# IVRL/NoiseDiff

Measured on AMD Instinct MI355X. Metric: sampled RAW patches/sec (256x256x4, 1000-step DDPM), higher is better.
Workload: dtype f32; 1 GPU; NoiseDiffNet dim=64, 256x256x4 patches, 1000-step DDPM (sigmoid2, pred_v), 16 patches per GPU; a step = one reverse-diffusion step (U-Net forward + fused posterior/noise update) over the per-GPU batch; patches/s = n_gpus*16/(1000*s_per_step); global_batch=16, launch=hipGraph replay, noise=device Philox4x32-10

## Files before the change

include/noisediff_hip.h:

```cpp
#ifndef NOISEDIFF_HIP_H
#define NOISEDIFF_HIP_H

#include <stdint.h>

#ifdef __cplusplus
extern "C" {
#endif

#define ND_E_BADARG   (-1)
#define ND_E_SHAPE    (-2)
#define ND_E_ALIGN    (-3)
#define ND_E_STATE    (-4)

int         nd_version(void);
const char* nd_last_error(void);
int         nd_device_arch(char* buf, int n);


enum nd_prologue {
    ND_PRO_NONE        = 0,
    ND_PRO_AFFINE_SILU = 1,
    ND_PRO_AFFINE_MAP_SILU = 2,
    ND_PRO_LAYERNORM   = 3,
    ND_PRO_SILU        = 4,
    ND_PRO_LEAKY       = 5,
    ND_PRO_LEAKY_SECOND = 6,
    ND_PRO_AFFINE_GENMAP_SILU = 7
};

typedef struct nd_src {
    const float* p0;
    const float* p1;
    int32_t c0, c1;
    int32_t ld0, ld1;
    int32_t mode;
    int32_t upsample;
    int32_t unshuffle;
    int32_t map_blocked;
    const float* mad;
    const float* map;
    const float* vec;
    const float* gamma;
    const float* beta;
    const float* rowstats;
} nd_src;

enum nd_act { ND_ACT_NONE = 0, ND_ACT_GELU = 1, ND_ACT_SILU = 2 };


typedef struct nd_conv3x3 {
    nd_src   src;
    const float* weight;
    const float* bias;
    float*   out;
    float*   stats;
    float*   slot_count;
    int32_t  B, H, W;
    int32_t  cin, cout, ldo;
} nd_conv3x3;

int nd_conv3x3_nhwc_f32(const nd_conv3x3* d, void* stream);
int nd_conv3x3_stat_slots(int H, int W, int cout, int B);
int nd_conv3x3_tiling_id(int B, int H, int W, int cout);
int64_t nd_pack_conv3x3_weight_floats(int cin, int cout);
int nd_pack_conv3x3_weight(const float* oihw, float* packed, int cin, int cout, void* stream);
int nd_pack_conv3x3_weight_dgrad(const float* oihw_fwd, float* packed, int cin, int cout, void* stream);

int nd_conv3x3_wino_nhwc_f32(const nd_conv3x3* d, void* stream);
int nd_conv3x3_wino2_nhwc_f32(const nd_conv3x3* d, void* stream);
int nd_conv3x3_wino_stat_slots(int H, int W);
int64_t nd_pack_conv3x3_wino_weight_floats(int cin, int cout);
int nd_pack_conv3x3_wino_weight(const float* oihw, float* packed, int cin, int cout, void* stream);
int nd_pack_conv3x3_wino_weight_dgrad(const float* oihw_fwd, float* packed, int cin, int cout, void* stream);

int nd_conv3x3_wino4_nhwc_f32(const nd_conv3x3* d, void* stream);
int nd_conv3x3_wino4_16_nhwc_f32(const nd_conv3x3* d, void* stream);
int nd_conv3x3_wino4_stat_slots(int H, int W);
int64_t nd_pack_conv3x3_wino4_weight_floats(int cin, int cout);
int nd_pack_conv3x3_wino4_weight(const float* oihw, float* packed, int cin, int cout, void* stream);
int nd_pack_conv3x3_wino4_weight_dgrad(const float* oihw_fwd, float* packed, int cin, int cout, void* stream);
typedef struct nd_pack_item {
    const float* w;
    float*       packed;
    int32_t      cin, cout, transposed, reserved;
} nd_pack_item;
int nd_pack_conv3x3_wino4_weights_batch(const nd_pack_item* items_dev, int n_items, void* stream);
int nd_conv3x3_wino4_splitk_plan(int B, int H, int W, int cin, int cout);
int64_t nd_conv3x3_wino4_splitk_workspace_floats(int B, int H, int W, int cout, int splits);
int nd_conv3x3_wino4_splitk_nhwc_f32(const nd_conv3x3* d, float* workspace, int splits, void* stream);
int nd_conv3x3_wino4_16_splitk_plan(int H, int W, int cin, int cout);
int nd_conv3x3_wino4_16_splitk_nhwc_f32(const nd_conv3x3* d, float* workspace, int splits, void* stream);


int64_t nd_conv3x3_wgrad_workspace_floats(int B, int H, int W, int cin, int cout);
int nd_conv3x3_wgrad_cat_nhwc_f32(const float* x0, int ldx0, int c0, const float* x1, int ldx1, int c1, const float* dy, int ldy, float* dw_oihw,
                                  float* dbias, float* workspace, int B, int H, int W, int cout, void* stream);
int nd_conv3x3_wgrad_form(int form);
int nd_conv3x3_wgrad_nhwc_f32(const float* x, int ldx, const float* dy, int ldy, float* dw_oihw, float* dbias, float* workspace,
                              int B, int H, int W, int cin, int cout, void* stream);
int nd_conv3x3_wgrad_leaky_nhwc_f32(const float* x, int ldx, const float* dy, int ldy, float* dw_oihw, float* dbias, float* workspace,
                                    int B, int H, int W, int cin, int cout, void* stream);
int64_t nd_conv3x3_wgrad_cat_workspace_floats(int B, int H, int W, int c0, int c1, int cout);
int nd_conv3x3_wgrad_cat_leaky_second_nhwc_f32(const float* x0, int ldx0, int c0, const float* x1, int ldx1, int c1, const float* dy, int ldy,
                                               float* dw_oihw, float* dbias, float* workspace, int B, int H, int W, int cout, void* stream);
int nd_leaky_grad_join_f32(const float* z, float* dz, const float* d_direct, int ld_direct, const float* d_pool, int B, int H, int W, int C,
                           void* stream);

int64_t nd_groupnorm_train_workspace_floats(int B, int HW, int C);
int nd_groupnorm_train_forward_f32(const float* x, int ldx, const float* gamma, const float* beta, float* y, int ldy, float* mean_rstd,
                                   float* workspace, int B, int HW, int C, int groups, float eps, void* stream);
int nd_groupnorm_train_backward_f32(const float* dy, int lddy, const float* x, int ldx, const float* gamma, const float* mean_rstd,
                                    float* dx, int lddx, float* dgamma, float* dbeta, float* workspace, int B, int HW, int C, int groups,
                                    void* stream);

int64_t nd_groupnorm_silu_train_workspace_floats(int B, int HW, int C);
int nd_groupnorm_silu_train_forward_f32(const float* x, int ldx, const float* gamma, const float* beta, const float* scale_shift, const float* res, int ldr,
                                        float* y, int ldy, float* mean_rstd, float* mad, float* workspace, int B, int HW, int C, int groups, float eps,
                                        void* stream);
int nd_groupnorm_silu_train_backward_f32(const float* dy, int lddy, const float* x, int ldx, const float* gamma, const float* beta,
                                         const float* scale_shift, const float* mean_rstd, const float* mad, float* dx, int lddx,
                                         float* dgamma, float* dbeta, float* dscale_shift, float* workspace, int B, int HW, int C, int groups,
                                         void* stream);

int nd_modulate_silu_forward_f32(const float* n, int ldn, const float* map, int ldm, float* y, int ldy, int64_t N, int C, void* stream);
int nd_modulate_silu_backward_f32(const float* dy, int lddy, const float* n, int ldn, const float* map, int ldm, float* dn, int lddn, float* dmap, int lddm,
                                  int64_t N, int C, void* stream);

int64_t nd_token_sum_workspace_floats(int B, int HW, int C);
int nd_token_sum_f32(const float* x, int ldx, float* out, float* workspace, int B, int HW, int C, void* stream);

int64_t nd_layernorm_train_workspace_floats(int64_t N, int C);
int nd_layernorm_train_forward_f32(const float* x, int ldx, const float* gamma, const float* beta, float* y, int ldy, float* stats,
                                   int64_t N, int C, float eps, void* stream);
int nd_layernorm_train_backward_f32(const float* dy, int lddy, const float* x, int ldx, const float* gamma, const float* stats,
                                    float* dx, int lddx, float* dgamma, float* dbeta, float* workspace, int64_t N, int C, void* stream);

int64_t nd_linear_wgrad_workspace_floats(int64_t N, int cin, int cout);
int nd_linear_wgrad_f32(const float* x, int ldx, const float* dy, int ldy, float* dw, float* dbias, float* workspace,
                        int64_t N, int cin, int cout, void* stream);
int nd_linear_wgrad_leaky_f32(const float* x, int ldx, const float* dy, int ldy, float* dw, float* dbias, float* workspace,
                              int64_t N, int cin, int cout, void* stream);
int64_t nd_convt2x2_wgrad_workspace_floats(int B, int h, int w, int cin, int cout);
int nd_convt2x2_wgrad_leaky_f32(const float* x, int ldx, const float* d_up, int ld_up, float* dw, float* workspace, int B, int h, int w,
                                int cin, int cout, int up_h, int up_w, void* stream);


typedef struct nd_pointwise {
    nd_src   src;
    const float* weight;
    const float* bias;
    float*   out;
    const float* res0; const float* res1;
    const float* vec;
    const float* gn_t;
    const float* gn_mad;
    int32_t  B, HW, W;
    int32_t  cin, cout, ldo, ldr0, ldr1, ldt;
    int32_t  act;
    int32_t  shuffle_c;
    int32_t  shuffle_h, shuffle_w;
} nd_pointwise;

int nd_pointwise_gemm_nhwc_f32(const nd_pointwise* d, void* stream);
int nd_pointwise_gemm_unshuffle_crop_nhwc_f32(const nd_pointwise* d, int src_h, int src_w, void* stream);

int64_t nd_image_quality_workspace_bytes(int B, int C, int H, int W);
int nd_image_quality_f32(const float* est, const float* target, const float* scale, double data_range, double* psnr, double* ssim,
                         double* mse, void* workspace, int B, int C, int H, int W, void* stream);
int64_t nd_illum_scale_workspace_bytes(int B, int C, int H, int W);
int nd_illum_scale_f32(const float* pred, const float* source, int source_batch, float* k32, double* k64, void* workspace,
                       int B, int C, int H, int W, void* stream);
int nd_illum_apply_f32(const float* pred, const float* k32, float* out, int B, int C, int H, int W, void* stream);
int64_t nd_pack_pointwise_weight_floats(int cin, int cout);
int nd_pack_pointwise_weight(const float* w, float* packed, int cin, int cout, int unshuffle_c, void* stream);
int nd_pack_pointwise_weight_t(const float* w_t, float* packed, int cin, int cout, void* stream);
int nd_pack_pointwise_weights_batch(const nd_pack_item* items_dev, int n_items, void* stream);

int nd_pointwise_gemm_split_nhwc_f32(const nd_pointwise* d, void* stream);
int nd_pointwise_gemm_split_takes(const nd_pointwise* d);
int64_t nd_pack_pointwise_weight_split_floats(int cin, int cout);
int nd_pack_pointwise_weight_split(const float* w, float* packed, int cin, int cout, void* stream);

enum nd_chain_res { ND_CHAIN_RES_NONE = 0, ND_CHAIN_RES_INPUT = 1 , ND_CHAIN_RES_INPUT_RAW = 2  };
typedef struct nd_chain_stage {
    const float* weight;
    const float* bias;
    int32_t  cin, cout;
    int32_t  act;
    int32_t  res;
} nd_chain_stage;
typedef struct nd_chain {
    nd_src   src;
    nd_chain_stage st[3];
    float*   out;
    int32_t  n_stages, B, HW, ldo;
} nd_chain;
int nd_pointwise_chain_nhwc_f32(const nd_chain* d, void* stream);
int nd_pointwise_chain_supported(int cin, int n1, int n2, int n3);
int64_t nd_pack_chain_weight_floats(int cin, int cout, int first_stage);
int nd_pack_chain_weight(const float* w, float* packed, int cin, int cout, int first_stage, void* stream);
int nd_pointwise_chain_split_nhwc_f32(const nd_chain* d, void* stream);
int64_t nd_pack_chain_weight_split_floats(int cin, int cout, int first_stage);
int nd_pack_chain_weight_split(const float* w, float* packed, int cin, int cout, int first_stage, void* stream);


int nd_groupnorm_finalize_f32(const float* stats, const float* slot_count, int slots,
                              const float* gamma, const float* beta,
                              const float* scale_shift, int ld_ss,
                              float* mad, int B, int C, int groups, float eps, void* stream);
int nd_groupnorm_finalize_train_f32(const float* stats, const float* slot_count, int slots, const float* gamma, const float* beta,
                                    const float* scale_shift, int ld_ss, float* mad, float* mean_rstd, int B, int C, int groups, float eps,
                                    void* stream);

int nd_layernorm_stats_f32(const float* x, int ldx, const float* vec, float* stats,
                           int B, int HW, int C, float eps, void* stream);

int nd_affine_silu_add_f32(const float* t, int ldt, const float* mad,
                           const float* res0, int ldr0, const float* res1, int ldr1,
                           float* out, int ldo, int B, int HW, int C, void* stream);


int nd_linear_rows_f32(const float* in, int ld_in, const float* W, const float* bias,
                       float* out, int ld_out, int B, int K, int N,
                       int act_in, int act_out, void* stream);
int nd_sinusoidal_time_emb_f32(const int64_t* time, const float* freqs, float* emb, int B, int half, void* stream);
int64_t nd_cond_step_lds_bytes(int B, int dim);
int nd_cond_step_f32(const int64_t* time, const float* freqs, const float* W1, const float* b1, const float* W2, const float* b2,
                     const float* Wp, const float* bp, float* out, int ld_out, int B, int dim, int J, void* stream);
int nd_cond_table_build_f32(const float* freqs, const float* W1, const float* b1, const float* W2, const float* b2, float* table, int rows, int dim,
                            void* stream);
int nd_cond_step_table_f32(const int64_t* time, const float* freqs, const float* W1, const float* b1, const float* W2, const float* b2,
                           const float* Wp, const float* bp, float* out, int ld_out, int B, int dim, int J, const float* table, int table_rows,
                           void* stream);
int nd_cond_step_ptable_f32(const int64_t* time, const float* freqs, const float* W1, const float* b1, const float* W2, const float* b2,
                            const float* Wp, const float* bp, float* out, int ld_out, int B, int dim, int J, const float* table, int table_rows,
                            const float* ptable, void* stream);
int nd_embedding_rows_f32(const int64_t* idx, const float* table, float* out, int B, int rows, int dim, void* stream);


int nd_conv7x7_c4_f32(const float* x, const float* wpacked, const float* bias, float* out, int ldo,
                      int B, int H, int W, int cout, void* stream);
int64_t nd_conv7x7_c4_wgrad_workspace_floats(int B, int H, int W, int cout);
int nd_conv7x7_c4_wgrad_f32(const float* x, const float* dy, int ldy, float* dw_oihw, float* dbias, float* workspace, int B, int H, int W, int cout,
                            void* stream);
int nd_pack_conv7x7_weight(const float* oihw, float* packed, int cout, void* stream);
int nd_conv7x7_c4_split_f32(const float* x, const float* wsplit, const float* bias, float* out, int ldo,
                            int B, int H, int W, int cout, void* stream);
int64_t nd_pack_conv7x7_weight_split_floats(int cout);
int nd_pack_conv7x7_weight_split(const float* oihw, float* packed, int cout, void* stream);
int nd_pos_enc_f32(const float* position_nchw, const float* w , const float* bias,
                   float* out, int B, int H, int W, int hid, void* stream);
int nd_maxpool2x2_nhwc_f32(const float* in, float* out, int B, int H, int W, int C, void* stream);
int nd_nchw_to_nhwc_f32(const float* in, float* out, int B, int C, int H, int W, void* stream);
int nd_nhwc_to_nchw_f32(const float* in, float* out, int B, int C, int H, int W, void* stream);
int nd_nchw_to_nhwc_pad_f32(const float* in, float* out, int B, int C, int H, int W, int Cpad, void* stream);


typedef struct nd_sampler_state {
    int32_t* step;
    const int32_t* t_cur;
    const int32_t* t_next;
    const float* coef;
    int64_t* time_out;
    const int64_t* rng;
    int32_t n_steps, B;
} nd_sampler_state;

int nd_sampler_begin_step(const nd_sampler_state* s, void* stream);
int nd_sampler_advance(const nd_sampler_state* s, void* stream);

int nd_sampler_step_ddpm_f32(float* x, const float* model_out, const float* noise, int64_t noise_step_stride,
                             const nd_sampler_state* s, int objective,
                             uint64_t seed, int64_t first_sample,
                             int B, int HW, int C, void* stream);
int nd_sampler_step_ddim_f32(float* x, const float* model_out, const float* noise, int64_t noise_step_stride,
                             const nd_sampler_state* s, int objective,
                             uint64_t seed, int64_t first_sample,
                             int B, int HW, int C, void* stream);
int nd_philox_normal_f32(float* out, uint64_t seed, int64_t first_sample, int32_t step,
                         int B, int HW, int C, void* stream);


int nd_attention_mfma_f32(const float* qkv, int ld_qkv, float* out, int ld_out,
                          int B, int N, int heads, int dh, void* stream);
int64_t nd_linear_attention_workspace_floats(int B, int N, int heads);
int nd_linear_attention_f32(const float* qkv, int ld_qkv, float* out, int ld_out, float* workspace,
                            int B, int N, int heads, int dh, void* stream);
int nd_rmsnorm_nhwc_f32(const float* x, int ldx, const float* g, float* out, int ldo,
                        int B, int HW, int C, void* stream);
int nd_rmsnorm_add_nhwc_f32(const float* x, int ldx, const float* g, const float* res, int ldr, float* out, int ldo, int B, int HW, int C, void* stream);

typedef struct nd_adam_item {
    float*       p;
    const float* g;
    float*       m;
    float*       v;
    int64_t      n;
    float        step_size, bias2_sqrt;
    int32_t      vec4, reserved;
    float*       step;
} nd_adam_item;
int nd_adam_chunk_elements(void);
int nd_adam_step_f32(const nd_adam_item* items_dev, int n_items, const int32_t* chunks_dev, int n_chunks, float beta1, float beta2, float eps,
                     float weight_decay, void* stream);
int nd_adam_step_capturable_f32(const nd_adam_item* items_dev, int n_items, const int32_t* chunks_dev, int n_chunks, float lr, float beta1, float beta2,
                                float eps, float weight_decay, void* stream);

int nd_stream_create(void** stream);
int nd_stream_destroy(void* stream);
int nd_stream_sync(void* stream);
int nd_graph_begin(void* stream);
int nd_graph_end(void* stream, void** graph_exec);
int nd_graph_launch(void* graph_exec, void* stream);
int nd_graph_destroy(void* graph_exec);
int nd_stream_device(void* stream);
int nd_event_create(void** ev);
int nd_event_record(void* ev, void* stream);
int nd_event_elapsed_ms(void* start, void* stop, float* ms);
int nd_event_destroy(void* ev);
int nd_event_create_untimed(void** ev);
int nd_stream_wait_event(void* stream, void* ev);

#ifdef __cplusplus
}
#endif
#endif
```

noisediff_amd/_lib.py:

```python
from __future__ import annotations

import ctypes as C
import os
from typing import Optional

HERE = os.path.dirname(os.path.abspath(__file__))
LIB_PATH = os.path.join(HERE, "libnoisediff_hip.so")

PRO_NONE, PRO_AFFINE_SILU, PRO_AFFINE_MAP_SILU, PRO_LAYERNORM, PRO_SILU, PRO_LEAKY, PRO_LEAKY_SECOND, PRO_AFFINE_GENMAP_SILU = 0, 1, 2, 3, 4, 5, 6, 7
ACT_NONE, ACT_GELU, ACT_SILU = 0, 1, 2
OBJECTIVES = {"pred_noise": 0, "pred_x0": 1, "pred_v": 2}

fptr = C.c_void_p


class HipError(RuntimeError):
    pass


class Src(C.Structure):
    _fields_ = [("p0", fptr), ("p1", fptr), ("c0", C.c_int32), ("c1", C.c_int32), ("ld0", C.c_int32), ("ld1", C.c_int32),
                ("mode", C.c_int32), ("upsample", C.c_int32), ("unshuffle", C.c_int32), ("map_blocked", C.c_int32),
                ("mad", fptr), ("map", fptr), ("vec", fptr), ("gamma", fptr), ("beta", fptr), ("rowstats", fptr)]


class AdamItem(C.Structure):
    _fields_ = [("p", fptr), ("g", fptr), ("m", fptr), ("v", fptr), ("n", C.c_int64), ("step_size", C.c_float), ("bias2_sqrt", C.c_float),
                ("vec4", C.c_int32), ("reserved", C.c_int32), ("step", fptr)]


class PackItem(C.Structure):
    _fields_ = [("w", fptr), ("packed", fptr), ("cin", C.c_int32), ("cout", C.c_int32), ("transposed", C.c_int32), ("reserved", C.c_int32)]


class Conv3x3(C.Structure):
    _fields_ = [("src", Src), ("weight", fptr), ("bias", fptr), ("out", fptr), ("stats", fptr), ("slot_count", fptr),
                ("B", C.c_int32), ("H", C.c_int32), ("W", C.c_int32), ("cin", C.c_int32), ("cout", C.c_int32), ("ldo", C.c_int32)]


class Pointwise(C.Structure):
    _fields_ = [("src", Src), ("weight", fptr), ("bias", fptr), ("out", fptr), ("res0", fptr), ("res1", fptr), ("vec", fptr),
                ("gn_t", fptr), ("gn_mad", fptr), ("B", C.c_int32), ("HW", C.c_int32), ("W", C.c_int32), ("cin", C.c_int32),
                ("cout", C.c_int32), ("ldo", C.c_int32), ("ldr0", C.c_int32), ("ldr1", C.c_int32), ("ldt", C.c_int32), ("act", C.c_int32),
                ("shuffle_c", C.c_int32), ("shuffle_h", C.c_int32), ("shuffle_w", C.c_int32)]


class ChainStage(C.Structure):
    _fields_ = [("weight", fptr), ("bias", fptr), ("cin", C.c_int32), ("cout", C.c_int32), ("act", C.c_int32), ("res", C.c_int32)]


class Chain(C.Structure):
    _fields_ = [("src", Src), ("st", ChainStage * 3), ("out", fptr), ("n_stages", C.c_int32), ("B", C.c_int32), ("HW", C.c_int32),
                ("ldo", C.c_int32)]


CHAIN_RES_NONE, CHAIN_RES_INPUT, CHAIN_RES_INPUT_RAW = 0, 1, 2


class SamplerState(C.Structure):
    _fields_ = [("step", fptr), ("t_cur", fptr), ("t_next", fptr), ("coef", fptr), ("time_out", fptr), ("rng", fptr),
                ("n_steps", C.c_int32), ("B", C.c_int32)]


i32, i64, u64, vp, f32, f64 = C.c_int, C.c_int64, C.c_uint64, C.c_void_p, C.c_float, C.c_double

SIGNATURES = {
    "nd_version": (i32, []),
    "nd_last_error": (C.c_char_p, []),
    "nd_device_arch": (i32, [C.c_char_p, i32]),
    "nd_conv3x3_nhwc_f32": (i32, [C.POINTER(Conv3x3), vp]),
    "nd_conv3x3_stat_slots": (i32, [i32, i32, i32, i32]),
    "nd_conv3x3_tiling_id": (i32, [i32, i32, i32, i32]),
    "nd_pack_conv3x3_weight_floats": (i64, [i32, i32]),
    "nd_pack_conv3x3_weight": (i32, [vp, vp, i32, i32, vp]),
    "nd_pack_conv3x3_weight_dgrad": (i32, [vp, vp, i32, i32, vp]),
    "nd_conv3x3_wino_nhwc_f32": (i32, [C.POINTER(Conv3x3), vp]),
    "nd_conv3x3_wino2_nhwc_f32": (i32, [C.POINTER(Conv3x3), vp]),
    "nd_conv3x3_wino_stat_slots": (i32, [i32, i32]),
    "nd_conv3x3_wino4_stat_slots": (i32, [i32, i32]),
    "nd_pack_conv3x3_wino_weight_floats": (i64, [i32, i32]),
    "nd_pack_conv3x3_wino_weight": (i32, [vp, vp, i32, i32, vp]),
    "nd_pack_conv3x3_wino_weight_dgrad": (i32, [vp, vp, i32, i32, vp]),
    "nd_conv3x3_wino4_nhwc_f32": (i32, [C.POINTER(Conv3x3), vp]),
    "nd_conv3x3_wino4_16_nhwc_f32": (i32, [C.POINTER(Conv3x3), vp]),
    "nd_pack_conv3x3_wino4_weight_floats": (i64, [i32, i32]),
    "nd_pack_conv3x3_wino4_weight": (i32, [vp, vp, i32, i32, vp]),
    "nd_pack_conv3x3_wino4_weight_dgrad": (i32, [vp, vp, i32, i32, vp]),
    "nd_conv3x3_wino4_splitk_plan": (i32, [i32, i32, i32, i32, i32]),
    "nd_conv3x3_wino4_splitk_workspace_floats": (i64, [i32, i32, i32, i32, i32]),
    "nd_conv3x3_wino4_splitk_nhwc_f32": (i32, [vp, vp, i32, vp]),
    "nd_conv3x3_wino4_16_splitk_plan": (i32, [i32, i32, i32, i32]),
    "nd_conv3x3_wino4_16_splitk_nhwc_f32": (i32, [vp, vp, i32, vp]),
    "nd_conv3x3_wgrad_workspace_floats": (i64, [i32, i32, i32, i32, i32]),
    "nd_conv3x3_wgrad_nhwc_f32": (i32, [vp, i32, vp, i32, vp, vp, vp, i32, i32, i32, i32, i32, vp]),
    "nd_groupnorm_train_workspace_floats": (i64, [i32, i32, i32]),
    "nd_linear_wgrad_workspace_floats": (i64, [i64, i32, i32]),
    "nd_groupnorm_silu_train_workspace_floats": (i64, [i32, i32, i32]),
    "nd_groupnorm_silu_train_forward_f32": (i32, [vp, i32, vp, vp, vp, vp, i32, vp, i32, vp, vp, vp, i32, i32, i32, i32, C.c_float, vp]),
    "nd_token_sum_workspace_floats": (i64, [i32, i32, i32]),
    "nd_token_sum_f32": (i32, [vp, i32, vp, vp, i32, i32, i32, vp]),
    "nd_modulate_silu_forward_f32": (i32, [vp, i32, vp, i32, vp, i32, i64, i32, vp]),
    "nd_modulate_silu_backward_f32": (i32, [vp, i32, vp, i32, vp, i32, vp, i32, vp, i32, i64, i32, vp]),
    "nd_groupnorm_silu_train_backward_f32": (i32, [vp, i32, vp, i32, vp, vp, vp, vp, vp, vp, i32, vp, vp, vp, vp, i32, i32, i32, i32, vp]),
    "nd_layernorm_train_workspace_floats": (i64, [i64, i32]),
    "nd_layernorm_train_forward_f32": (i32, [vp, i32, vp, vp, vp, i32, vp, i64, i32, C.c_float, vp]),
    "nd_layernorm_train_backward_f32": (i32, [vp, i32, vp, i32, vp, vp, vp, i32, vp, vp, vp, i64, i32, vp]),
    "nd_linear_wgrad_f32": (i32, [vp, i32, vp, i32, vp, vp, vp, i64, i32, i32, vp]),
    "nd_groupnorm_train_forward_f32": (i32, [vp, i32, vp, vp, vp, i32, vp, vp, i32, i32, i32, i32, C.c_float, vp]),
    "nd_groupnorm_train_backward_f32": (i32, [vp, i32, vp, i32, vp, vp, vp, i32, vp, vp, vp, i32, i32, i32, i32, vp]),
    "nd_pointwise_gemm_nhwc_f32": (i32, [C.POINTER(Pointwise), vp]),
    "nd_pointwise_chain_nhwc_f32": (i32, [C.POINTER(Chain), vp]),
    "nd_pointwise_chain_supported": (i32, [i32, i32, i32, i32]),
    "nd_pack_chain_weight_floats": (i64, [i32, i32, i32]),
    "nd_pack_chain_weight": (i32, [vp, vp, i32, i32, i32, vp]),
    "nd_pointwise_chain_split_nhwc_f32": (i32, [C.POINTER(Chain), vp]),
    "nd_pack_chain_weight_split_floats": (i64, [i32, i32, i32]),
    "nd_pack_chain_weight_split": (i32, [vp, vp, i32, i32, i32, vp]),
    "nd_pointwise_gemm_split_nhwc_f32": (i32, [C.POINTER(Pointwise), vp]),
    "nd_pointwise_gemm_split_takes": (i32, [C.POINTER(Pointwise)]),
    "nd_pack_pointwise_weight_split_floats": (i64, [i32, i32]),
    "nd_pack_pointwise_weight_split": (i32, [vp, vp, i32, i32, vp]),
    "nd_pack_pointwise_weight_floats": (i64, [i32, i32]),
    "nd_pack_pointwise_weight": (i32, [vp, vp, i32, i32, i32, vp]),
    "nd_pack_pointwise_weight_t": (i32, [vp, vp, i32, i32, vp]),
    "nd_pack_pointwise_weights_batch": (i32, [vp, i32, vp]),
    "nd_pack_conv3x3_wino4_weights_batch": (i32, [vp, i32, vp]),
    "nd_conv3x3_wgrad_cat_nhwc_f32": (i32, [vp, i32, i32, vp, i32, i32, vp, i32, vp, vp, vp, i32, i32, i32, i32, vp]),
    "nd_conv3x3_wgrad_form": (i32, [i32]),
    "nd_conv7x7_c4_wgrad_workspace_floats": (i64, [i32, i32, i32, i32]),
    "nd_conv7x7_c4_wgrad_f32": (i32, [vp, vp, i32, vp, vp, vp, i32, i32, i32, i32, vp]),
    "nd_adam_chunk_elements": (i32, []),
    "nd_adam_step_f32": (i32, [vp, i32, vp, i32, f32, f32, f32, f32, vp]),
    "nd_adam_step_capturable_f32": (i32, [vp, i32, vp, i32, f32, f32, f32, f32, f32, vp]),
    "nd_groupnorm_finalize_f32": (i32, [vp, vp, i32, vp, vp, vp, i32, vp, i32, i32, i32, f32, vp]),
    "nd_groupnorm_finalize_train_f32": (i32, [vp, vp, i32, vp, vp, vp, i32, vp, vp, i32, i32, i32, f32, vp]),
    "nd_layernorm_stats_f32": (i32, [vp, i32, vp, vp, i32, i32, i32, f32, vp]),
    "nd_affine_silu_add_f32": (i32, [vp, i32, vp, vp, i32, vp, i32, vp, i32, i32, i32, i32, vp]),
    "nd_linear_rows_f32": (i32, [vp, i32, vp, vp, vp, i32, i32, i32, i32, i32, i32, vp]),
    "nd_sinusoidal_time_emb_f32": (i32, [vp, vp, vp, i32, i32, vp]),
    "nd_cond_step_lds_bytes": (i64, [i32, i32]),
    "nd_cond_step_f32": (i32, [vp, vp, vp, vp, vp, vp, vp, vp, vp, i32, i32, i32, i32, vp]),
    "nd_cond_table_build_f32": (i32, [vp, vp, vp, vp, vp, vp, i32, i32, vp]),
    "nd_cond_step_table_f32": (i32, [vp, vp, vp, vp, vp, vp, vp, vp, vp, i32, i32, i32, i32, vp, i32, vp]),
    "nd_cond_step_ptable_f32": (i32, [vp, vp, vp, vp, vp, vp, vp, vp, vp, i32, i32, i32, i32, vp, i32, vp, vp]),
    "nd_embedding_rows_f32": (i32, [vp, vp, vp, i32, i32, i32, vp]),
    "nd_conv7x7_c4_f32": (i32, [vp, vp, vp, vp, i32, i32, i32, i32, i32, vp]),
    "nd_pack_conv7x7_weight": (i32, [vp, vp, i32, vp]),
    "nd_conv7x7_c4_split_f32": (i32, [vp, vp, vp, vp, i32, i32, i32, i32, i32, vp]),
    "nd_pack_conv7x7_weight_split_floats": (i64, [i32]),
    "nd_pack_conv7x7_weight_split": (i32, [vp, vp, i32, vp]),
    "nd_pos_enc_f32": (i32, [vp, vp, vp, vp, i32, i32, i32, i32, vp]),
    "nd_maxpool2x2_nhwc_f32": (i32, [vp, vp, i32, i32, i32, i32, vp]),
    "nd_nchw_to_nhwc_pad_f32": (i32, [vp, vp, i32, i32, i32, i32, i32, vp]),
    "nd_nchw_to_nhwc_f32": (i32, [vp, vp, i32, i32, i32, i32, vp]),
    "nd_nhwc_to_nchw_f32": (i32, [vp, vp, i32, i32, i32, i32, vp]),
    "nd_sampler_begin_step": (i32, [C.POINTER(SamplerState), vp]),
    "nd_sampler_advance": (i32, [C.POINTER(SamplerState), vp]),
    "nd_sampler_step_ddpm_f32": (i32, [vp, vp, vp, i64, C.POINTER(SamplerState), i32, u64, i64, i32, i32, i32, vp]),
    "nd_sampler_step_ddim_f32": (i32, [vp, vp, vp, i64, C.POINTER(SamplerState), i32, u64, i64, i32, i32, i32, vp]),
    "nd_philox_normal_f32": (i32, [vp, u64, i64, i32, i32, i32, i32, vp]),
    "nd_attention_mfma_f32": (i32, [vp, i32, vp, i32, i32, i32, i32, i32, vp]),
    "nd_linear_attention_workspace_floats": (i64, [i32, i32, i32]),
    "nd_linear_attention_f32": (i32, [vp, i32, vp, i32, vp, i32, i32, i32, i32, vp]),
    "nd_rmsnorm_nhwc_f32": (i32, [vp, i32, vp, vp, i32, i32, i32, i32, vp]),
    "nd_rmsnorm_add_nhwc_f32": (i32, [vp, i32, vp, vp, i32, vp, i32, i32, i32, i32, vp]),
    "nd_stream_create": (i32, [C.POINTER(vp)]),
    "nd_stream_destroy": (i32, [vp]),
    "nd_stream_sync": (i32, [vp]),
    "nd_graph_begin": (i32, [vp]),
    "nd_graph_end": (i32, [vp, C.POINTER(vp)]),
    "nd_graph_launch": (i32, [vp, vp]),
    "nd_graph_destroy": (i32, [vp]),
    "nd_event_create": (i32, [C.POINTER(vp)]),
    "nd_event_record": (i32, [vp, vp]),
    "nd_event_elapsed_ms": (i32, [vp, vp, C.POINTER(f32)]),
    "nd_event_destroy": (i32, [vp]),
    "nd_event_create_untimed": (i32, [C.POINTER(vp)]),
    "nd_stream_wait_event": (i32, [vp, vp]),
    "nd_stream_device": (i32, [vp]),
    "nd_conv3x3_wgrad_leaky_nhwc_f32": (i32, [vp, i32, vp, i32, vp, vp, vp, i32, i32, i32, i32, i32, vp]),
    "nd_conv3x3_wgrad_cat_workspace_floats": (i64, [i32, i32, i32, i32, i32, i32]),
    "nd_conv3x3_wgrad_cat_leaky_second_nhwc_f32": (i32, [vp, i32, i32, vp, i32, i32, vp, i32, vp, vp, vp, i32, i32, i32, i32, vp]),
    "nd_leaky_grad_join_f32": (i32, [vp, vp, vp, i32, vp, i32, i32, i32, i32, vp]),
    "nd_linear_wgrad_leaky_f32": (i32, [vp, i32, vp, i32, vp, vp, vp, i64, i32, i32, vp]),
    "nd_convt2x2_wgrad_workspace_floats": (i64, [i32, i32, i32, i32, i32]),
    "nd_convt2x2_wgrad_leaky_f32": (i32, [vp, i32, vp, i32, vp, vp, i32, i32, i32, i32, i32, i32, i32, vp]),
    "nd_pointwise_gemm_unshuffle_crop_nhwc_f32": (i32, [C.POINTER(Pointwise), i32, i32, vp]),
    "nd_image_quality_workspace_bytes": (i64, [i32, i32, i32, i32]),
    "nd_image_quality_f32": (i32, [vp, vp, vp, f64, vp, vp, vp, vp, i32, i32, i32, i32, vp]),
    "nd_illum_scale_workspace_bytes": (i64, [i32, i32, i32, i32]),
    "nd_illum_scale_f32": (i32, [vp, vp, i32, vp, vp, vp, i32, i32, i32, i32, vp]),
    "nd_illum_apply_f32": (i32, [vp, vp, vp, i32, i32, i32, i32, vp]),
}

_UNCHECKED = {"nd_version", "nd_last_error", "nd_stream_device", "nd_conv3x3_wgrad_form", "nd_adam_chunk_elements", "nd_conv7x7_c4_wgrad_workspace_floats", "nd_conv3x3_stat_slots", "nd_conv3x3_tiling_id", "nd_pack_conv3x3_weight_floats",
              "nd_pack_pointwise_weight_floats", "nd_linear_attention_workspace_floats", "nd_conv3x3_wino_stat_slots", "nd_conv3x3_wino4_stat_slots",
              "nd_pack_conv3x3_wino_weight_floats", "nd_pack_conv3x3_wino4_weight_floats", "nd_conv3x3_wino4_splitk_plan", "nd_conv3x3_wino4_16_splitk_plan", "nd_conv3x3_wino4_splitk_workspace_floats", "nd_token_sum_workspace_floats", "nd_cond_step_lds_bytes", "nd_conv3x3_wgrad_workspace_floats",
              "nd_groupnorm_train_workspace_floats", "nd_linear_wgrad_workspace_floats",
              "nd_layernorm_train_workspace_floats", "nd_groupnorm_silu_train_workspace_floats", "nd_conv3x3_wgrad_cat_workspace_floats",
              "nd_convt2x2_wgrad_workspace_floats", "nd_image_quality_workspace_bytes", "nd_illum_scale_workspace_bytes"}

_lib: Optional[C.CDLL] = None


def load(path: str = LIB_PATH) -> C.CDLL:
    global _lib
    if _lib is not None:
        return _lib
    import torch
    if not os.path.exists(path):
        raise HipError(f"{path} is missing: the HIP library is the product and there is no fallback. "
                       "Build it with `python -m noisediff_amd.build`.")
    lib = C.CDLL(path)
    for name, (res, args) in SIGNATURES.items():
        fn = getattr(lib, name)
        fn.restype, fn.argtypes = res, args
    _lib = lib
    return lib


def check(code: int, what: str = "") -> None:
    if code != 0:
        msg = load().nd_last_error().decode(errors="replace")
        raise HipError(f"{what or 'libnoisediff_hip'} failed with code {code}: {msg}")


def call(name: str, *args):
    r = getattr(load(), name)(*args)
    if name not in _UNCHECKED:
        check(r, name)
    return r


def ptr(t) -> Optional[int]:
    return None if t is None else t.data_ptr()
```

noisediff_amd/csrc/conv3x3_wino4.hip:

```cpp
#include <stdlib.h>
#include <type_traits>
#include "nd_common.h"

namespace {

typedef float f32x2 __attribute__((ext_vector_type(2)));
typedef unsigned u32x4_t __attribute__((ext_vector_type(4)));
typedef __attribute__((address_space(3))) void* lds_ptr;
typedef __attribute__((address_space(3))) short* lds_short_ptr;
typedef __attribute__((address_space(3))) unsigned* lds_u32_ptr;
typedef __attribute__((address_space(3))) unsigned short* lds_u16_ptr;
typedef __attribute__((address_space(3))) f32x4* lds_f32x4_ptr;

constexpr int KC4 = 16;
constexpr int NPOS = 36;
constexpr int VD_FLOATS = NPOS * 256;

constexpr int MAX_COUT = 2048;
template <int NTG, int NW = 4>
struct W4Geo {
    static constexpr int NT = 64 * NW;
    static constexpr int TGW = NTG * 4 / NW;
    static constexpr int REG_W = 16 * NTG, HALO_W = REG_W + 2;
    static constexpr int RAW_ROWP = NTG == 2 ? 40 : 24;
    static constexpr int RAW_ITEMS = 18 * HALO_W * 4, RAW_IT = (RAW_ITEMS + NT - 1) / NT;
    static constexpr int RAW_FLOATS = 18 * RAW_ROWP * 16;
    static constexpr bool RTAB = TGW == 2;
    static constexpr bool BIAS_LDS = TGW == 2;
    static constexpr int TAB_BYTES = (RAW_IT + (RTAB ? RAW_IT : 0)) * NT * 4 + (RAW_IT + 12) * NT * 2;
    static constexpr int BIAS_OFF_BYTES = RAW_FLOATS * 4 + NTG * VD_FLOATS * 4 + TAB_BYTES;
    static constexpr int LDS_BYTES = BIAS_OFF_BYTES + (BIAS_LDS ? MAX_COUT * 4 : 0);
    static constexpr int WG_PER_CU = NTG == 2 ? 1 : 2;
    static constexpr int ACC_AGPR = TGW == 2 ? 64 : 32;
    static_assert(NW == 4 || (NW == 8 && NTG == 2), "four waves, or eight on the 16 x 32 region");
    static_assert(LDS_BYTES * WG_PER_CU <= 160 * 1024, "LDS map");
};

#ifndef W4_UR
#define W4_UR 18
#endif
#ifndef W4_UR_AFF
#define W4_UR_AFF 18
#endif
#ifndef W4_UR_MAP
#define W4_UR_MAP 6
#endif
#ifndef W4_UR_GEN
#define W4_UR_GEN 6
#endif
#ifndef W4_UR_EPI
#define W4_UR_EPI 6
#endif
#ifndef W4_VR
#define W4_VR 3
#endif
#ifndef W4_COMMIT_AT
#define W4_COMMIT_AT 8
#endif
#ifndef W4_XF_AT
#define W4_XF_AT 10
#endif
#ifndef W4_U_AUX
#define W4_U_AUX 0
#endif
#ifndef W4_STORE_AUX
#define W4_STORE_AUX 19
#endif
#ifndef W4_STAGGER
#define W4_STAGGER 12
#endif
#ifndef W4_XF_SPLIT
#define W4_XF_SPLIT 1
#endif
#ifndef W4_UR1
#define W4_UR1 9
#endif
#ifndef W4_UR1_AFF
#define W4_UR1_AFF 6
#endif
#ifndef W4_UR1_EPI
#define W4_UR1_EPI 0
#endif
#ifndef W4_UR1_XF
#define W4_UR1_XF 6
#endif
#ifndef W4_PAIR_SKEW
#define W4_PAIR_SKEW 2
#endif
#ifndef W4_PRIO
#define W4_PRIO 0
#endif
#ifndef W4_ABLATE
#define W4_ABLATE 0
#endif

struct Wino4Args {
    nd_conv3x3 d;
    int tiles_x, tiles_y, regions_x, n_tiles, n_cg, n_c8, slots, total_wg;
    int splits, chunks_per_split;
};

#ifndef W4_NOP
#define W4_NOP ""
#endif
#define W4_MFMA_A(acc, uv, vv)  asm volatile(W4_NOP "v_mfma_f32_16x16x4_f32 %0, %2, %1, %0" : "+a"(acc) : "v"(uv), "v"(vv))
#define W4_MFMA_V(acc, uv, vv)  asm volatile(W4_NOP "v_mfma_f32_16x16x4_f32 %0, %2, %1, %0" : "+v"(acc) : "v"(uv), "v"(vv))
#define W4_MFMA_AZ(acc, uv, vv) asm volatile(W4_NOP "v_mfma_f32_16x16x4_f32 %0, %2, %1, 0" : "=&a"(acc) : "v"(uv), "v"(vv))
#define W4_MFMA_VZ(acc, uv, vv) asm volatile(W4_NOP "v_mfma_f32_16x16x4_f32 %0, %2, %1, 0" : "=&v"(acc) : "v"(uv), "v"(vv))
#define W4_MFMA_DRAIN() asm volatile("s_nop 15\n\ts_nop 15" ::: "memory")

__device__ __forceinline__ void w4_bt(const f32x2 (&d)[6], f32x2 (&t)[6]) {
    const f32x2 c4 = {4.0f, 4.0f}, cm4 = {-4.0f, -4.0f}, cm5 = {-5.0f, -5.0f}, c2 = {2.0f, 2.0f}, cm2 = {-2.0f, -2.0f};
    const f32x2 p = __builtin_elementwise_fma(cm4, d[2], d[4]), q = __builtin_elementwise_fma(cm4, d[1], d[3]);
    const f32x2 r = d[4] - d[2], s = d[3] - d[1];
    t[0] = __builtin_elementwise_fma(c4, d[0], __builtin_elementwise_fma(cm5, d[2], d[4]));
    t[1] = p + q;
    t[2] = p - q;
    t[3] = __builtin_elementwise_fma(c2, s, r);
    t[4] = __builtin_elementwise_fma(cm2, s, r);
    t[5] = __builtin_elementwise_fma(c4, d[1], __builtin_elementwise_fma(cm5, d[3], d[5]));
}

template <int HALF>
__device__ __forceinline__ void w4_bt_half(const f32x2 (&d)[6], f32x2 (&t)[3]) {
    const f32x2 c4 = {4.0f, 4.0f}, cm4 = {-4.0f, -4.0f}, cm5 = {-5.0f, -5.0f}, c2 = {2.0f, 2.0f}, cm2 = {-2.0f, -2.0f};
    if (HALF == 0) {
        const f32x2 p = __builtin_elementwise_fma(cm4, d[2], d[4]), q = __builtin_elementwise_fma(cm4, d[1], d[3]);
        t[0] = __builtin_elementwise_fma(c4, d[0], __builtin_elementwise_fma(cm5, d[2], d[4]));
        t[1] = p + q;
        t[2] = p - q;
    } else {
        const f32x2 r = d[4] - d[2], s = d[3] - d[1];
        t[0] = __builtin_elementwise_fma(c2, s, r);
        t[1] = __builtin_elementwise_fma(cm2, s, r);
        t[2] = __builtin_elementwise_fma(c4, d[1], __builtin_elementwise_fma(cm5, d[3], d[5]));
    }
}

template <int MODE, bool STREAM, bool SPLIT = false, int NTG = 2, int NW = 4>
__global__ __launch_bounds__((64 * NW), (W4Geo<NTG, NW>::WG_PER_CU)) void wino4_kernel(const Wino4Args a) {
    using Geo = W4Geo<NTG, NW>;
    constexpr int NT = Geo::NT, TGW = Geo::TGW;
    constexpr int RAW_FLOATS = Geo::RAW_FLOATS, BIAS_OFF_BYTES = Geo::BIAS_OFF_BYTES, ACC_AGPR = Geo::ACC_AGPR, REG_W = Geo::REG_W, HALO_W = Geo::HALO_W;
    constexpr bool MAP = MODE == ND_PRO_AFFINE_MAP_SILU;
    constexpr bool GEN = MODE == ND_PRO_AFFINE_GENMAP_SILU;
    constexpr bool MAPX = MAP || GEN;
    constexpr bool AFF = MODE == ND_PRO_AFFINE_SILU || MAPX;
    constexpr bool LEAKY = MODE == ND_PRO_LEAKY || MODE == ND_PRO_LEAKY_SECOND;
    constexpr int UR = TGW == 1 ? (AFF ? W4_UR1_AFF : W4_UR1) : MAP ? W4_UR_MAP : GEN ? W4_UR_GEN : AFF ? W4_UR_AFF : W4_UR, UR_EPI = TGW == 1 ? W4_UR1_EPI : W4_UR_EPI;
    static_assert(TGW == 2 || !MAPX, "the map prologues (20 more staging registers per halo item in flight) stay on the 512-register form");
    extern __shared__ __attribute__((aligned(16))) float lds_[];
    float* const Vd = lds_ + RAW_FLOATS;

    const int tid = threadIdx.x, lane = tid & 63;
    const int wave = __builtin_amdgcn_readfirstlane(tid >> 6);
    const int mtg = NW == 8 ? wave >> 2 : 0;
    const int tg = TGW == 2 ? wave >> 1 : mtg, rh = (wave >> 1) & 1, ch2 = wave & 1;
    const int tile = lane & 15, kq = lane >> 4;

    const int wgid = nd_xcd_remap(blockIdx.x, gridDim.x);
    const int t_begin = (int)((long)wgid * a.total_wg / gridDim.x), t_end = (int)((long)(wgid + 1) * a.total_wg / gridDim.x);
    if (t_begin >= t_end) return;

#ifdef W4_STAMP
    const unsigned long long stamp_c0 = __builtin_amdgcn_s_memtime(), stamp_r0 = __builtin_amdgcn_s_memrealtime();
    unsigned long long stamp_epi = 0, stamp_xf = 0, stamp_wait = 0, stamp_t = 0, stamp_drain = 0, stamp_first = 0, stamp_last = 0, stamp_second = 0, stamp_third = 0, stamp_pro = 0, stamp_top = 0, stamp_tile = 0;
#define W4_T0() (stamp_t = __builtin_amdgcn_s_memtime())
#define W4_ACC(x) (x += __builtin_amdgcn_s_memtime() - stamp_t)
#else
#define W4_T0()
#define W4_ACC(x)
#endif
#if W4_STAGGER
    if (a.total_wg >= 4 * (int)gridDim.x)
        for (int k = (int)(blockIdx.x >> 3) & 15; k > 0; --k) __builtin_amdgcn_s_sleep(W4_STAGGER);
#endif
#if W4_PAIR_SKEW
    if (NTG == 1 && 2 * blockIdx.x >= gridDim.x)
        for (int k = 0; k < W4_PAIR_SKEW; ++k) __builtin_amdgcn_s_sleep(32);
#endif
    const nd_src& s = a.d.src;
    const int H = a.d.H, W = a.d.W, Cin = a.d.cin, Cout = a.d.cout;
    const int up = s.upsample ? 1 : 0;
    const int sH = H >> up, sW = W >> up;
    const int Ctot = s.c0 + s.c1;
    const int n_chunks = SPLIT ? a.chunks_per_split : (Cin + KC4 - 1) / KC4;

    auto decode = [&](int t, int& b_, int& ty_, int& rx_, int& nt_, int& sp_) {
        int lid = t;
        nt_ = lid % a.n_tiles;  lid /= a.n_tiles;
        rx_ = lid % a.regions_x;  lid /= a.regions_x;
        ty_ = lid % a.tiles_y;
        b_ = lid / a.tiles_y;
        sp_ = 0;
        if (SPLIT) { sp_ = b_ / a.d.B;  b_ -= sp_ * a.d.B; }
    };

    constexpr int RAW_ROWP = Geo::RAW_ROWP, RAW_IT = Geo::RAW_IT;
    const long npx = (long)a.d.B * sH * sW;
    const unsigned PX_MARK = (unsigned)(npx + sW + 2);
    auto src_rsrc = [&](const float* p, long px_stride_floats) {
        return __builtin_amdgcn_make_buffer_rsrc(const_cast<float*>(p) - (long)(sW + 1) * px_stride_floats, 0,
                                                 (int)((npx + sW + 1) * px_stride_floats * 4), 0x00020000);
    };
    const __amdgpu_buffer_rsrc_t rsrc0 = src_rsrc(s.p0, s.ld0);
    const __amdgpu_buffer_rsrc_t rsrc1 = s.p1 ? src_rsrc(s.p1, s.ld1) : rsrc0;
    const __amdgpu_buffer_rsrc_t rsrcm = MAP ? src_rsrc(s.map, 2 * Ctot) : GEN ? src_rsrc(s.map, 8) : rsrc0;
    const int map_shift = s.map_blocked ? 64 : Ctot * 4;
    float* const vd_tg = Vd + tg * VD_FLOATS;
    char* const rawbuf = reinterpret_cast<char*>(lds_);
    lds_u32_ptr const ptab = (lds_u32_ptr)(Vd + NTG * VD_FLOATS) + tid;
    auto cperm = [](int c) { return ((c >> 2) & 3) | ((c & 3) << 2) | (c & 48); };
    auto swz = [](int r, int c) { return (2 * ((r >> 2) & 3)) ^ (4 * ((c >> 3) & 1)); };
    auto pixl_of = [](int t) { return GEN ? 16 * (t >> 6) + (t & 15) : t >> 2; };
    const int sq = GEN ? (tid >> 4) & 3 : tid & 3;
    lds_u32_ptr const rtab = ptab + RAW_IT * NT;
    lds_u16_ptr const dtab = (lds_u16_ptr)(ptab - tid + (Geo::RTAB ? 2 : 1) * RAW_IT * NT) + tid;
    lds_u16_ptr const ttab = dtab + RAW_IT * NT;
    float* const bias_lds = reinterpret_cast<float*>(reinterpret_cast<char*>(lds_) + BIAS_OFF_BYTES);
    auto item_rc = [&](int k, int tid_) {
        const int pix = pixl_of(tid_) + (NT / 4) * k, r = pix / HALO_W, c = pix - HALO_W * r;
        const int dy = up ? (r + 1) >> 1 : r, dx = up ? (c + 1) >> 1 : c;
        return (unsigned)(dy * sW + dx) | ((unsigned)r << 16) | ((unsigned)c << 24);
    };
#pragma unroll
    for (int k = 0; k < RAW_IT; ++k) {
        const int pix = pixl_of(tid) + (NT / 4) * k, r = pix / HALO_W, c = pix - HALO_W * r;
        dtab[k * NT] = (unsigned short)((r * RAW_ROWP + cperm(c)) * 64 + (((2 * sq) ^ swz(r, c)) * 8));
        if (Geo::RTAB) rtab[k * NT] = item_rc(k, tid);
    }
    const int t_tile = ((lane >> 1) & 7) | ((lane >> 4) & 1) << 3, t_kq = (lane & 1) | ((lane >> 5) << 1);
#pragma unroll
    for (int h = 0; h < 2; ++h)
#pragma unroll
        for (int bx = 0; bx < 6; ++bx) {
            const int r0 = 4 * (t_tile >> 2) + 4 * h, c = 16 * tg + 4 * (t_tile & 3) + bx;
            ttab[(h * 6 + bx) * NT] = (unsigned short)((4 * (t_tile >> 2) * RAW_ROWP + cperm(c)) * 64 + (((4 * ch2 + t_kq) ^ swz(r0, c)) * 8));
        }
    const unsigned t_lds = (unsigned)(ch2 * 1024 + (t_kq >> 1) * 512 + t_tile * 32 + (t_kq & 1) * 16);
    if (Geo::BIAS_LDS)
        for (int i = tid; i < a.n_tiles * 64; i += NT) bias_lds[i] = (a.d.bias && i < Cout) ? a.d.bias[i] : 0.0f;
    const __amdgpu_buffer_rsrc_t brsrc = __builtin_amdgcn_make_buffer_rsrc(const_cast<float*>(a.d.bias ? a.d.bias : a.d.weight), 0, a.d.bias ? Cout * 4 : 0, 0x00020000);
    float bias_r = 0.0f;

    const unsigned OOB = 0x7FFFFFF0u;
    int sb_ = 0;
    unsigned spx_ = 0;
    bool tab_clean = false;
    f32x4 tA4 = {1, 1, 1, 1}, tD4 = {0, 0, 0, 0};
    auto stage_tile = [&](int b_, int ty_, int rx_) {
        sb_ = b_;
        spx_ = (unsigned)((b_ * sH + ((ty_ * 16) >> up)) * sW + ((rx_ * REG_W) >> up));
        const int r_lo = ty_ == 0 ? 1 : 0, r_n = min(17, H - ty_ * 16) - r_lo;
        const int c_lo = rx_ == 0 ? 1 : 0, c_n = min(HALO_W - 1, W - rx_ * REG_W) - c_lo;
        const bool interior = r_lo == 0 && r_n == 17 && c_lo == 0 && c_n == HALO_W - 1;
        if (!(interior && tab_clean)) {
            int tid_ = tid;
            if (!Geo::RTAB) asm volatile("" : "+v"(tid_));
#pragma unroll
            for (int k = 0; k < RAW_IT; ++k) {
                const unsigned rc = Geo::RTAB ? rtab[k * NT] : item_rc(k, tid_);
                const unsigned r = (rc >> 16) & 255u, c = rc >> 24;
                const bool ok = r - (unsigned)r_lo <= (unsigned)r_n && c - (unsigned)c_lo <= (unsigned)c_n;
                ptab[k * NT] = ok ? (rc & 0xFFFFu) : PX_MARK;
            }
        }
        tab_clean = interior;
    };
    f32x4 raw[RAW_IT];
    constexpr int GEN_H = RAW_IT / 2;
    f32x4 msc[MAP ? RAW_IT : GEN ? GEN_H : 1], msh[MAP ? RAW_IT : GEN ? GEN_H : 1];
    float ev0[GEN ? RAW_IT : 1], ev1[GEN ? RAW_IT : 1];
    float gw_sc0 = 0, gw_sc1 = 0, gw_sh0 = 0, gw_sh1 = 0;
    f32x4 gb_sc = {0, 0, 0, 0}, gb_sh = {0, 0, 0, 0};
    int i_eoff = 0;
    bool i_second = false;
    __amdgpu_buffer_rsrc_t i_rs = rsrc0;
    int i_soff = 0, i_mapoff = 0;
    unsigned i_ld4 = 0, i_bias = 0;
    auto stage_issue_begin = [&](int cb_) {
        const bool sec = cb_ >= s.c0;
        i_second = sec;
        i_mapoff = (int)(cb_ * (s.map_blocked ? 8u : 4u) + spx_ * (unsigned)(2 * Ctot * 4));
        i_rs = sec ? rsrc1 : rsrc0;
        i_ld4 = (unsigned)(sec ? s.ld1 : s.ld0) * 4u;
        i_soff = (int)((sec ? cb_ - s.c0 : cb_) * 4u + spx_ * i_ld4);
        i_bias = cb_ + 4 * sq < Cin ? 16u * sq : OOB;
        if (GEN) {
            i_eoff = (int)(spx_ * 32u);
            const float* wr = s.gamma + (size_t)(cb_ + (lane & 15)) * 8 + sq;
            gw_sc0 = wr[0];  gw_sc1 = wr[4];  gw_sh0 = wr[(size_t)Ctot * 8];  gw_sh1 = wr[(size_t)Ctot * 8 + 4];
            gb_sc = nd_ld4(s.beta + cb_ + 4 * sq);  gb_sh = nd_ld4(s.beta + Ctot + cb_ + 4 * sq);
        }
        if (AFF) {
            const int c = cb_ + 4 * sq;
            const float* m = s.mad + (size_t)sb_ * 3 * Ctot + (c < Cin ? c : 0);
            const f32x4 M = nd_ld4(m), A = nd_ld4(m + Ctot), D = nd_ld4(m + 2 * Ctot);
            tA4 = A;
            tD4 = D - M * A;
        }
    };
    auto stage_issue_one = [&](int k, unsigned px, auto tile_first_c) {
#if !(W4_ABLATE & 1)
        const unsigned voff = __umul24(px, i_ld4) + i_bias;
        raw[k] = __builtin_bit_cast(f32x4, __builtin_amdgcn_raw_buffer_load_b128(i_rs, voff, i_soff, 0));
        if (GEN && decltype(tile_first_c)::value) {
            const unsigned eo = __umul24(px, 32u) + 4u * sq;
            ev0[k] = __builtin_bit_cast(float, __builtin_amdgcn_raw_buffer_load_b32(rsrcm, eo, i_eoff, 0));
            ev1[k] = __builtin_bit_cast(float, __builtin_amdgcn_raw_buffer_load_b32(rsrcm, eo, i_eoff + 16, 0));
        }
        if (MAP) {
            const unsigned mo = __umul24(px, (unsigned)(2 * Ctot * 4)) + i_bias;
            msc[k] = __builtin_bit_cast(f32x4, __builtin_amdgcn_raw_buffer_load_b128(rsrcm, mo, i_mapoff, 0));
            msh[k] = __builtin_bit_cast(f32x4, __builtin_amdgcn_raw_buffer_load_b128(rsrcm, mo, i_mapoff + map_shift, 0));
        }
#else
        raw[k] = f32x4{(float)k, 1.0f, 0.5f, 0.25f};
#endif
    };
    auto gen_maps = [&](int k0) {
#pragma unroll
        for (int k = 0; k < GEN_H; ++k) asm volatile("v_mfma_f32_16x16x4_f32 %0, %1, %2, %3" : "=&v"(msc[GEN ? k : 0]) : "v"(gw_sc0), "v"(ev0[GEN ? k0 + k : 0]), "v"(gb_sc));
#pragma unroll
        for (int k = 0; k < GEN_H; ++k) asm volatile("v_mfma_f32_16x16x4_f32 %0, %1, %2, %3" : "=&v"(msh[GEN ? k : 0]) : "v"(gw_sh0), "v"(ev0[GEN ? k0 + k : 0]), "v"(gb_sh));
#pragma unroll
        for (int k = 0; k < GEN_H; ++k) asm volatile("v_mfma_f32_16x16x4_f32 %0, %1, %2, %0" : "+v"(msc[GEN ? k : 0]) : "v"(gw_sc1), "v"(ev1[GEN ? k0 + k : 0]));
#pragma unroll
        for (int k = 0; k < GEN_H; ++k) asm volatile("v_mfma_f32_16x16x4_f32 %0, %1, %2, %0" : "+v"(msh[GEN ? k : 0]) : "v"(gw_sh1), "v"(ev1[GEN ? k0 + k : 0]));
        W4_MFMA_DRAIN();
    };
    auto stage_commit_one = [&](int k, unsigned daddr, unsigned pxk) {
        if (k == RAW_IT - 1 && pixl_of(tid) + (NT / 4) * k >= 18 * HALO_W) return;
        f32x4 v = raw[k];
        if (AFF) {
            f32x4 x = v * tA4 + tD4;
            if (MAPX) x = x * (msc[MAP ? k : GEN ? k % GEN_H : 0] + 1.0f) + msh[MAP ? k : GEN ? k % GEN_H : 0];
            const f32x4 t = x * -1.44269504088896340736f;
            f32x4 e;
            e.x = __builtin_amdgcn_exp2f(t.x); e.y = __builtin_amdgcn_exp2f(t.y); e.z = __builtin_amdgcn_exp2f(t.z); e.w = __builtin_amdgcn_exp2f(t.w);
            e = e + 1.0f;
            f32x4 r;
            r.x = __builtin_amdgcn_rcpf(e.x); r.y = __builtin_amdgcn_rcpf(e.y); r.z = __builtin_amdgcn_rcpf(e.z); r.w = __builtin_amdgcn_rcpf(e.w);
            const bool inside = pxk != PX_MARK && i_bias != OOB;
            const f32x4 zero = {0, 0, 0, 0};
            v = inside ? x * r : zero;
        }
        if (MODE == ND_PRO_LEAKY || (MODE == ND_PRO_LEAKY_SECOND && i_second)) v = nd_leaky4(v);
        *reinterpret_cast<lds_f32x4_ptr>(daddr) = v;
    };

    const unsigned d_lds = (unsigned)((kq >> 1) * 512 + tile * 32 + (kq & 1) * 16);

    auto xf_addr = [&](unsigned (&t_addr)[12]) {
#pragma unroll
        for (int i = 0; i < 12; ++i) t_addr[i] = ttab[i * NT];
    };
    auto xf_read = [&](f32x2 (&T)[6][6], const unsigned (&t_addr)[12], int ay) {
#if !(W4_ABLATE & 4)
#pragma unroll
        for (int bx = 0; bx < 6; ++bx)
            T[ay][bx] = *reinterpret_cast<const f32x2*>(rawbuf + t_addr[(ay >> 2) * 6 + bx] + ay * (RAW_ROWP * 64));
#endif
    };
    auto xf_finish = [&](f32x2 (&T)[6][6], float* buf, auto&& before_write) {
#if !(W4_ABLATE & 4)
        char* base = reinterpret_cast<char*>(buf) + t_lds;
#pragma unroll
        for (int bx = 0; bx < 6; ++bx) {
            f32x2 col[6], t[6];
#pragma unroll
            for (int ay = 0; ay < 6; ++ay) col[ay] = T[ay][bx];
            w4_bt(col, t);
#pragma unroll
            for (int xi = 0; xi < 6; ++xi) T[xi][bx] = t[xi];
        }
#if W4_XF_SPLIT
        before_write();
#endif
#pragma unroll
        for (int xi = 0; xi < 6; ++xi) {
            f32x2 v[6];
            w4_bt(T[xi], v);
#if W4_XF_SPLIT
#pragma unroll
            for (int h = 0; h < 3; ++h)
                *reinterpret_cast<f32x4*>(base + (xi * 3 + h) * 2048) = f32x4{v[2 * h].x, v[2 * h].y, v[2 * h + 1].x, v[2 * h + 1].y};
            __builtin_amdgcn_sched_barrier(0);
#else
#pragma unroll
            for (int bx = 0; bx < 6; ++bx) T[xi][bx] = v[bx];
#endif
        }
#if !W4_XF_SPLIT
        before_write();
#pragma unroll
        for (int xi = 0; xi < 6; ++xi)
#pragma unroll
            for (int h = 0; h < 3; ++h)
                *reinterpret_cast<f32x4*>(base + (xi * 3 + h) * 2048) = f32x4{T[xi][2 * h].x, T[xi][2 * h].y, T[xi][2 * h + 1].x, T[xi][2 * h + 1].y};
#endif
#else
        before_write();
#endif
    };

    auto xf_half = [&](float* buf) {
#if !(W4_ABLATE & 4)
        unsigned t_addr[12];
        xf_addr(t_addr);
        f32x2 T[3][6];
        auto pass1 = [&](auto half_c) {
#pragma unroll
            for (int bx = 0; bx < 6; ++bx) {
                f32x2 col[6], t[3];
#pragma unroll
                for (int ay = 0; ay < 6; ++ay) col[ay] = *reinterpret_cast<const f32x2*>(rawbuf + t_addr[(ay >> 2) * 6 + bx] + ay * (RAW_ROWP * 64));
                w4_bt_half<decltype(half_c)::value>(col, t);
#pragma unroll
                for (int i = 0; i < 3; ++i) T[i][bx] = t[i];
            }
        };
        if (rh == 0) pass1(std::integral_constant<int, 0>{}); else pass1(std::integral_constant<int, 1>{});
        char* base = reinterpret_cast<char*>(buf) + t_lds + rh * (9 * 2048);
#pragma unroll
        for (int i = 0; i < 3; ++i) {
            f32x2 v[6];
            w4_bt(T[i], v);
#pragma unroll
            for (int h = 0; h < 3; ++h)
                *reinterpret_cast<f32x4*>(base + (i * 3 + h) * 2048) = f32x4{v[2 * h].x, v[2 * h].y, v[2 * h + 1].x, v[2 * h + 1].y};
        }
#endif
    };

    const __amdgpu_buffer_rsrc_t wrsrc = __builtin_amdgcn_make_buffer_rsrc(
        const_cast<float*>(a.d.weight), 0, (int)((long)a.n_c8 * a.n_cg * 18 * 256 * 4), 0x00020000);
    const unsigned wvoff = (unsigned)(lane * 16);
    auto wblock = [&](int c8_, int cg_) { return __builtin_amdgcn_readfirstlane(((c8_ * a.n_cg + cg_) * 18) * 1024); };

    f32x4 acc[TGW * NPOS];
    f32x4 U[UR];
    f32x4 Vr[W4_VR][TGW];
    static_assert(36 % UR == 0, "the ring must close over a chunk's two stages of 18 fragments");
    auto load_u = [&](int slot, int q, int wb) {
#if !(W4_ABLATE & 2)
        U[slot % UR] = __builtin_bit_cast(f32x4, __builtin_amdgcn_raw_buffer_load_b128(wrsrc, wvoff, wb + q * 1024, W4_U_AUX));
#endif
    };
    auto read_v = [&](const char* v0base, const char* v1base, int pp) {
        Vr[pp % W4_VR][0] = *reinterpret_cast<const f32x4*>(v0base + pp * 2048);
        if (TGW == 2) Vr[pp % W4_VR][TGW - 1] = *reinterpret_cast<const f32x4*>(v1base + pp * 2048);
    };
    auto mfma = [&](auto first_c, int idx, float av, float bv) {
        constexpr bool FIRST = decltype(first_c)::value;
        if (idx < ACC_AGPR) { if (FIRST) W4_MFMA_AZ(acc[idx], av, bv); else W4_MFMA_A(acc[idx], av, bv); }
        else                { if (FIRST) W4_MFMA_VZ(acc[idx], av, bv); else W4_MFMA_V(acc[idx], av, bv); }
    };
    auto stage = [&](auto first_c, auto off_c, auto din_c, auto dout_c, const char* v0base, const char* v1base, int wb, int nb, auto&& pre, auto&& mid) {
        constexpr int OFF = decltype(off_c)::value, DIN = decltype(din_c)::value, DOUT = decltype(dout_c)::value;
        auto hi = [](int pp) { const int h = pp + UR; return h < 18 + DOUT ? h : 18 + DOUT; };
#pragma unroll
        for (int pp = 0; pp < W4_VR - 1; ++pp) read_v(v0base, v1base, pp);
#pragma unroll
        for (int q = DIN; q < hi(0); ++q) {
            if (q < 18) load_u(OFF + q, q, wb);
            else load_u(OFF + q, q - 18, nb);
        }
        __builtin_amdgcn_sched_barrier(0);
#pragma unroll
        for (int pp = 0; pp < 18; ++pp) {
            if (pp + W4_VR - 1 < 18) read_v(v0base, v1base, pp + W4_VR - 1);
            pre(pp);
            const f32x4 u = U[(OFF + pp) % UR];
            const f32x4 va = Vr[pp % W4_VR][0], vb = Vr[pp % W4_VR][TGW - 1];
            __builtin_amdgcn_sched_barrier(0);
            if (TGW == 2) {
                mfma(first_c, 4 * pp + 0, u.x, va.x);
                mfma(first_c, 4 * pp + 1, u.x, vb.x);
                mfma(first_c, 4 * pp + 2, u.z, va.z);
                mfma(first_c, 4 * pp + 3, u.z, vb.z);
                mfma(std::false_type{}, 4 * pp + 0, u.y, va.y);
                mfma(std::false_type{}, 4 * pp + 1, u.y, vb.y);
                mfma(std::false_type{}, 4 * pp + 2, u.w, va.w);
                mfma(std::false_type{}, 4 * pp + 3, u.w, vb.w);
            } else {
                mfma(first_c, 2 * pp + 0, u.x, va.x);
                mfma(first_c, 2 * pp + 1, u.z, va.z);
                mfma(std::false_type{}, 2 * pp + 0, u.y, va.y);
                mfma(std::false_type{}, 2 * pp + 1, u.w, va.w);
            }
            __builtin_amdgcn_sched_barrier(0);
#pragma unroll
            for (int q = (hi(pp) > DIN ? hi(pp) : DIN); q < hi(pp + 1); ++q) {
                if (q < 18) load_u(OFF + q, q, wb);
                else load_u(OFF + q, q - 18, nb);
            }
            mid(pp);
            __builtin_amdgcn_sched_barrier(0);
        }
    };

    auto read_acc2 = [&](int idx, int h) -> f32x2 {
        if (idx >= ACC_AGPR) {
            asm volatile("" : "+v"(acc[idx]));
            return h ? f32x2{acc[idx].z, acc[idx].w} : f32x2{acc[idx].x, acc[idx].y};
        }
        f32x2 r;
        if (h == 0) {
            asm volatile("v_accvgpr_read_b32 %0, %1" : "=v"(r.x) : "a"(acc[idx].x));
            asm volatile("v_accvgpr_read_b32 %0, %1" : "=v"(r.y) : "a"(acc[idx].y));
        } else {
            asm volatile("v_accvgpr_read_b32 %0, %1" : "=v"(r.x) : "a"(acc[idx].z));
            asm volatile("v_accvgpr_read_b32 %0, %1" : "=v"(r.y) : "a"(acc[idx].w));
        }
        return r;
    };

    int b, ty, rx, nt, sp;
    decode(t_begin, b, ty, rx, nt, sp);
    int b1 = b, ty1 = ty, rx1 = rx, nt1 = nt, sp1 = sp;
    stage_tile(b, ty, rx);
    stage_issue_begin(SPLIT ? sp * n_chunks * KC4 : 0);
#pragma unroll
    for (int k = 0; k < RAW_IT; ++k) stage_issue_one(k, ptab[k * NT], std::true_type{});
    {
        const int wb = wblock(SPLIT ? 2 * sp * n_chunks : 0, nt * 4 + (wave & 3));
#pragma unroll
        for (int q = 0; q < UR_EPI; ++q) load_u(q, q, wb);
    }
#pragma unroll
    for (int k = 0; k < RAW_IT; ++k) {
        if (GEN && k % GEN_H == 0) gen_maps(k);
        stage_commit_one(k, dtab[k * NT], AFF ? ptab[k * NT] : 0u);
    }
    asm volatile("s_waitcnt lgkmcnt(0)" ::: "memory");
    __builtin_amdgcn_s_barrier();
    if constexpr (TGW == 2) {
        f32x2 T[6][6];
        unsigned t_addr[12];
        xf_addr(t_addr);
#pragma unroll
        for (int ay = 0; ay < 6; ++ay) xf_read(T, t_addr, ay);
        xf_finish(T, vd_tg, [] {});
    } else xf_half(vd_tg);
    asm volatile("s_waitcnt lgkmcnt(0)" ::: "memory");
    __builtin_amdgcn_s_barrier();

#ifdef W4_STAMP
    stamp_pro = __builtin_amdgcn_s_memtime() - stamp_c0;
#endif
    for (int t = t_begin; t < t_end; ++t) {
        const bool more = t + 1 < t_end;
        W4_T0();
        if (more) {
            nt1 = nt + 1;  rx1 = rx;  ty1 = ty;  b1 = b;  sp1 = sp;
            if (nt1 == a.n_tiles) { nt1 = 0;  if (++rx1 == a.regions_x) { rx1 = 0;  if (++ty1 == a.tiles_y) { ty1 = 0;  ++b1;  if (SPLIT && b1 == a.d.B) { b1 = 0;  ++sp1; } } } }
        }
        const int ch0 = SPLIT ? sp * n_chunks : 0, ch0n = SPLIT ? sp1 * n_chunks : 0;
        const int cg = nt * 4 + (wave & 3), cg_next = (more ? nt1 : nt) * 4 + (wave & 3);

        auto chunk = [&](int ch, auto first_c, auto last_c) {
            const char* v0cur = reinterpret_cast<const char*>(Vd + mtg * VD_FLOATS) + d_lds;
            const char* v1cur = reinterpret_cast<const char*>(Vd + (NTG - 1) * VD_FLOATS) + d_lds;
            constexpr bool last = decltype(last_c)::value;
            const int c8 = 2 * (ch0 + ch);
            const int w0 = wblock(c8, cg), w1 = wblock(c8 + 1, cg), wn = last ? wblock(2 * ch0n, cg_next) : wblock(c8 + 2, cg);
#ifdef W4_STAMP
            if (decltype(first_c)::value) W4_ACC(stamp_top);
            W4_T0();
#endif
            if (last && more) stage_tile(b1, ty1, rx1);
#ifdef W4_STAMP
            if (last) W4_ACC(stamp_tile);
#endif
            using I0 = std::integral_constant<int, 0>;
            using IOFF1 = std::integral_constant<int, 18 % UR>;
            using IUR = std::integral_constant<int, UR>;
            using IEPI = std::integral_constant<int, UR_EPI>;
            using IXF = std::integral_constant<int, TGW == 1 ? (W4_UR1_XF < UR ? W4_UR1_XF : UR) : UR>;
            constexpr bool FIRST = decltype(first_c)::value;
            unsigned tab1 = 0;
            constexpr bool PRE_P = AFF && !MAPX;
            unsigned tabd[(AFF || LEAKY) ? RAW_IT : 1], tabp[PRE_P ? RAW_IT : 1];
            auto issue_pre = [&](int pp) { if (pp < RAW_IT) tab1 = ptab[pp * NT]; };
            auto issue = [&](int pp) {
                if (pp == 0) stage_issue_begin(last ? ch0n * KC4 : (ch0 + ch + 1) * KC4);
                if (pp < RAW_IT) stage_issue_one(pp, tab1, last_c);
            };
            auto commit_pre = [&](int pp) {
                if (AFF || LEAKY) {
                    if (pp == W4_COMMIT_AT) {
#pragma unroll
                        for (int k = 0; k < RAW_IT; ++k) {
                            tabd[k] = dtab[k * NT];
                            if (PRE_P) tabp[k] = ptab[k * NT];
                        }
                    }
                } else if (pp < RAW_IT) tab1 = dtab[pp * NT];
            };
            f32x2 T[TGW == 2 ? 6 : 1][6];
            unsigned t_addr[12];
            auto commit = [&](int pp) {
                if (AFF || LEAKY) {
                    if (pp == W4_COMMIT_AT) {
#pragma unroll
                        for (int k = 0; k < RAW_IT; ++k) {
                            if (GEN && k % GEN_H == 0) gen_maps(k);
                            stage_commit_one(k, tabd[(AFF || LEAKY) ? k : 0], PRE_P ? tabp[PRE_P ? k : 0] : MAPX ? ptab[k * NT] : 0u);
                        }
                    }
                } else if (pp < RAW_IT) stage_commit_one(pp, tab1, 0u);
                if constexpr (TGW == 2) {
                    if (pp == W4_XF_AT) {
                        asm volatile("s_waitcnt lgkmcnt(0)" ::: "memory");
                        __builtin_amdgcn_s_barrier();
                        xf_addr(t_addr);
                    }
                    if (pp > W4_XF_AT && pp <= W4_XF_AT + 6) xf_read(T, t_addr, pp - W4_XF_AT - 1);
                }
            };
            W4_T0();
            if (TGW == 1 && FIRST)
                bias_r = __builtin_bit_cast(float, __builtin_amdgcn_raw_buffer_load_b32(brsrc, (unsigned)(cg * 16 + (lane & 15)) * 4u, 0, 0));
            stage(first_c, I0{}, std::conditional_t<FIRST, IEPI, IXF>{}, IUR{}, v0cur, v1cur, w0, w1, issue_pre, issue);
            if (TGW == 1 && FIRST) asm volatile("" : "+v"(bias_r));
            stage(std::false_type{}, IOFF1{}, IUR{}, std::conditional_t<last, IEPI, IXF>{}, v0cur + 1024, v1cur + 1024, w1, wn, commit_pre, commit);
#ifdef W4_STAMP
            if (FIRST) W4_ACC(stamp_first);
            if (last) W4_ACC(stamp_last);
            if (!FIRST && !last && ch == 1) W4_ACC(stamp_second);
            if (!FIRST && !last && ch == 2) W4_ACC(stamp_third);
#endif
            W4_T0();
            if constexpr (TGW == 2) {
                xf_finish(T, vd_tg, [&] {
                    W4_ACC(stamp_xf);
                    W4_T0();
                    __builtin_amdgcn_s_barrier();
                    W4_ACC(stamp_wait);
                    W4_T0();
                });
            } else {
                asm volatile("s_waitcnt lgkmcnt(0)" ::: "memory");
                __builtin_amdgcn_s_barrier();
                W4_ACC(stamp_wait);
                W4_T0();
                if (W4_PRIO) __builtin_amdgcn_s_setprio(W4_PRIO);
                xf_half(vd_tg);
                if (W4_PRIO) __builtin_amdgcn_s_setprio(0);
            }
            asm volatile("s_waitcnt lgkmcnt(0)" ::: "memory");
            __builtin_amdgcn_s_barrier();
            W4_ACC(stamp_xf);
        };
        chunk(0, std::true_type{}, std::false_type{});
        for (int ch = 1; ch + 1 < n_chunks; ++ch) chunk(ch, std::false_type{}, std::false_type{});
        chunk(n_chunks - 1, std::false_type{}, std::true_type{});

        W4_T0();
        W4_MFMA_DRAIN();
        if (TGW == 1 && W4_PRIO) __builtin_amdgcn_s_setprio(W4_PRIO);

        const __amdgpu_buffer_rsrc_t orsrc = __builtin_amdgcn_make_buffer_rsrc(a.d.out, 0, (int)((unsigned)(SPLIT ? a.splits : 1) * a.d.B * H * W * a.d.ldo * 4u), 0x00020000);
        int Wt = __builtin_amdgcn_readfirstlane(W), ldot = __builtin_amdgcn_readfirstlane(a.d.ldo);
        asm volatile("" : "+s"(Wt), "+s"(ldot));
#pragma unroll
        for (int j = 0; j < TGW; ++j) {
            const int tx = NTG * rx + (TGW == 2 ? j : mtg);
            if (tx < a.tiles_x) {
                int l15 = lane;
                asm volatile("" : "+v"(l15));
                l15 &= 15;
                const int co = cg * 16 + l15;
                const bool cok = co < Cout;
                float z0 = 0.0f;
                asm volatile("" : "+v"(z0));
                const float* const bias_p = bias_lds + co;
                const int py0 = ty * 16 + 4 * kq, px0 = tx * 16;
                f32x2 sum2 = {z0, z0}, sq2 = {z0, z0}, cnt2 = {z0, z0};
                float pivot = z0;
                const bool full = ty * 16 + 16 <= H && tx * 16 + 16 <= W && cg * 16 + 16 <= Cout;
                const bool want_stats = a.d.stats != nullptr;
                const unsigned lane_off = (unsigned)((((unsigned)(SPLIT ? sp * a.d.B + b : b) * H + py0) * Wt + px0) * ldot + co) * 4u;
                auto emit = [&](auto full_c, auto stats_c) {
                    constexpr bool FULL = decltype(full_c)::value, STATS = decltype(stats_c)::value;
                    int step4 = ldot * 16, back3 = ldot * -12, rowadv = (Wt - 7) * ldot * 4;
                    asm volatile("" : "+s"(step4), "+s"(back3), "+s"(rowadv));
                    const f32x2 c2 = {2.0f, 2.0f}, c4 = {4.0f, 4.0f}, c8 = {8.0f, 8.0f};
                    const int rowlim = FULL ? 4 : H - py0, collim = FULL ? 16 : W - px0;
#pragma unroll
                    for (int h = 0; h < 2; ++h) {
                        int soff = h * 32 * ldot;
                        asm volatile("" : "+s"(soff));
                        f32x2 Z[4][6];
#pragma unroll
                        for (int nu = 0; nu < 6; ++nu) {
                            auto M = [&](int xi) { return read_acc2(TGW * (xi * 6 + nu) + j, h); };
                            f32x2 m1 = M(1);
                            const f32x2 m2 = M(2);
                            if (nu == 1) m1 += Geo::BIAS_LDS ? *bias_p : bias_r;
                            const f32x2 p = m1 + m2, q = m1 - m2;
                            const f32x2 m3 = M(3), m4 = M(4);
                            const f32x2 r = m3 + m4, u = m3 - m4;
                            Z[0][nu] = M(0) + p + r;
                            Z[1][nu] = __builtin_elementwise_fma(c2, u, q);
                            Z[2][nu] = __builtin_elementwise_fma(c4, r, p);
                            Z[3][nu] = __builtin_elementwise_fma(c8, u, q) + M(5);
                            __builtin_amdgcn_sched_barrier(0);
                        }
#pragma unroll
                        for (int i = 0; i < 4; ++i) {
                            const f32x2 (&z)[6] = Z[i];
                            const f32x2 ta = z[1] + z[2], tb = z[1] - z[2], tc = z[3] + z[4], te = z[3] - z[4];
                            f32x2 y[4];
                            y[0] = z[0] + ta + tc;
                            y[1] = __builtin_elementwise_fma(c2, te, tb);
                            y[2] = __builtin_elementwise_fma(c4, tc, ta);
                            y[3] = __builtin_elementwise_fma(c8, te, tb) + z[5];
#pragma unroll
                            for (int jj = 0; jj < 4; ++jj) {
                                const f32x2 v = y[jj];
                                if (STATS && h == 0 && i == 0 && jj == 0)
                                    pivot = __shfl(v.x, l15);
                                f32x2 in2 = {1.0f, 1.0f};
                                if (!FULL) {
                                    int rl = rowlim;
                                    asm volatile("" : "+v"(rl));
                                    const bool row_in = i < rl;
                                    in2.x = (row_in && 8 * h + jj < collim) ? 1.0f : 0.0f;
                                    in2.y = (row_in && 8 * h + 4 + jj < collim) ? 1.0f : 0.0f;
                                }
                                if (STATS) {
                                    f32x2 dv = v - f32x2{pivot, pivot};
                                    if (!FULL) { dv *= in2;  cnt2 += in2; }
                                    sum2 += dv;
                                    sq2 += dv * dv;
                                }
#if !(W4_ABLATE & 8)
#pragma unroll
                                for (int e = 0; e < 2; ++e) {
                                    const float vr = e ? v.y : v.x;
                                    unsigned off = lane_off;
                                    if (!FULL) off = ((e ? in2.y : in2.x) != 0.0f && cok) ? off : 0xFFFFFFF0u;
                                    __builtin_amdgcn_raw_buffer_store_b32(__builtin_bit_cast(unsigned, vr), orsrc, off, soff, STREAM ? W4_STORE_AUX : 0);
                                    asm volatile("s_add_i32 %0, %0, %1" : "+s"(soff) : "s"(e == 0 ? step4 : jj < 3 ? back3 : rowadv) : "scc");
                                }
#else
                                asm volatile("" :: "v"(v));
#endif
                            }
                        }
                    }
                };
                if (full) { if (want_stats) emit(std::true_type{}, std::true_type{}); else emit(std::true_type{}, std::false_type{}); }
                else { if (want_stats) emit(std::false_type{}, std::true_type{}); else emit(std::false_type{}, std::false_type{}); }
                if (a.d.stats) {
                    float fc = full ? 64.0f : cnt2.x + cnt2.y;
                    float S = sum2.x + sum2.y, Q = sq2.x + sq2.y;
                    fc += __shfl_xor(fc, 16);  S += __shfl_xor(S, 16);  Q += __shfl_xor(Q, 16);
                    fc += __shfl_xor(fc, 32);  S += __shfl_xor(S, 32);  Q += __shfl_xor(Q, 32);
                    const int slot = ty * a.tiles_x + tx;
                    if (kq == 0 && cok) {
                        fc = fmaxf(fc, 1.0f);
                        float* o = a.d.stats + (((size_t)b * a.slots + slot) * Cout + co) * 2;
                        *reinterpret_cast<f32x2*>(o) = f32x2{S + fc * pivot, fmaxf(Q - S * S / fc, 0.0f)};
                    }
#ifndef W4_STAMP
                    if (b == 0 && nt == 0 && (wave & 3) == 0 && lane == 0) {
                        a.d.slot_count[slot] = (float)(min(16, H - ty * 16) * min(16, W - tx * 16));
                    }
#endif
                }
            }
        }
        if (TGW == 1 && W4_PRIO) __builtin_amdgcn_s_setprio(0);
        W4_ACC(stamp_epi);
#ifdef W4_STAMP_DRAIN
        W4_T0();
        asm volatile("s_waitcnt vmcnt(0)" ::: "memory");
        W4_ACC(stamp_drain);
#endif
        b = b1; ty = ty1; rx = rx1; nt = nt1; sp = sp1;
    }
#ifdef W4_STAMP
    if (tid == 0) {
        unsigned long long* dbg = reinterpret_cast<unsigned long long*>(a.d.slot_count) + 16 * blockIdx.x;
        dbg[0] = __builtin_amdgcn_s_memtime() - stamp_c0;
        dbg[1] = __builtin_amdgcn_s_memrealtime() - stamp_r0;
        dbg[2] = (unsigned long long)(t_end - t_begin) * n_chunks;
        dbg[3] = stamp_epi;
        dbg[4] = stamp_xf;
        dbg[5] = stamp_second;
        dbg[6] = stamp_first;
        dbg[7] = stamp_last;
        dbg[8] = stamp_third;
        dbg[9] = stamp_wait;
        dbg[10] = stamp_pro;
        dbg[11] = stamp_top;
        dbg[12] = stamp_tile;
    }
#endif
}

__global__ __launch_bounds__(256) void w4_splitk_reduce_kernel(const float* __restrict__ part, const float* __restrict__ bias, float* __restrict__ out,
                                                               int splits, long npix, int cout, int ldo) {
    const int cq = cout >> 2;
    const long total = npix * cq;
    for (long i = blockIdx.x * (long)blockDim.x + threadIdx.x; i < total; i += (long)gridDim.x * blockDim.x) {
        const long n = i / cq;
        const int c = (int)(i - n * cq) * 4;
        f32x4 acc = nd_ld4(part + n * cout + c);
        for (int s = 1; s < splits; ++s) acc += nd_ld4(part + ((long)s * npix + n) * cout + c);
        if (bias) acc += nd_ld4(bias + c);
        nd_st4(out + n * ldo + c, acc);
    }
}

__global__ __launch_bounds__(256) void w4_splitk_reduce_stats_kernel(const float* __restrict__ part, const float* __restrict__ bias, float* __restrict__ out,
                                                                     float* __restrict__ stats, float* __restrict__ slot_count, int splits, int B, int H, int W,
                                                                     int cout, int ldo, int tiles_x, int tiles_y, int n_cgrp) {
    __shared__ __attribute__((aligned(16))) float red[2][256][4];
    int bid = blockIdx.x;
    const int cgrp = bid % n_cgrp;  bid /= n_cgrp;
    const int slot = bid % (tiles_x * tiles_y), b = bid / (tiles_x * tiles_y);
    const int ty = slot / tiles_x, tx = slot % tiles_x;
    const int y0 = ty * 16, x0 = tx * 16, th = min(16, H - y0), tw = min(16, W - x0), npx = th * tw;
    const long npix = (long)B * H * W;
    const int q = cgrp * 16 + (threadIdx.x & 15), rg = threadIdx.x >> 4;
    const bool act = 4 * q < cout;
    f32x4 s1 = {0, 0, 0, 0}, s2 = {0, 0, 0, 0}, pv = {0, 0, 0, 0};
    if (act) {
        const f32x4 bq = bias ? nd_ld4(bias + 4 * q) : f32x4{0, 0, 0, 0};
        {
            const long n0 = ((long)b * H + y0) * W + x0;
            pv = nd_ld4(part + n0 * cout + 4 * q);
            for (int sp = 1; sp < splits; ++sp) pv += nd_ld4(part + ((long)sp * npix + n0) * cout + 4 * q);
            pv += bq;
        }
        for (int p = rg; p < npx; p += 16) {
            const int py = p / tw, px = p - py * tw;
            const long n = ((long)b * H + y0 + py) * W + x0 + px;
            f32x4 v = nd_ld4(part + n * cout + 4 * q);
            for (int sp = 1; sp < splits; ++sp) v += nd_ld4(part + ((long)sp * npix + n) * cout + 4 * q);
            v += bq;
            nd_st4(out + n * ldo + 4 * q, v);
            const f32x4 dv = v - pv;
            s1 += dv;  s2 += dv * dv;
        }
    }
    *reinterpret_cast<f32x4*>(red[0][threadIdx.x]) = s1;
    *reinterpret_cast<f32x4*>(red[1][threadIdx.x]) = s2;
    __syncthreads();
    if (act && rg == 0) {
        for (int r = 1; r < 16; ++r) {
            s1 += *reinterpret_cast<const f32x4*>(red[0][r * 16 + (threadIdx.x & 15)]);
            s2 += *reinterpret_cast<const f32x4*>(red[1][r * 16 + (threadIdx.x & 15)]);
        }
        const float fn = (float)npx;
        float* o = stats + (((size_t)b * tiles_x * tiles_y + slot) * cout + 4 * q) * 2;
#pragma unroll
        for (int i = 0; i < 4; ++i) {
            o[2 * i] = s1[i] + fn * pv[i];
            o[2 * i + 1] = fmaxf(s2[i] - s1[i] * s1[i] / fn, 0.0f);
        }
    }
    if (b == 0 && cgrp == 0 && threadIdx.x == 0) slot_count[slot] = (float)npx;
}

template <int MODE, int NTG = 2>
int launch4_split(const Wino4Args& a, hipStream_t st) {
    static nd_device_once configured;
    constexpr int LDS_BYTES = W4Geo<NTG>::LDS_BYTES;
    if (int e = nd_reserve_lds(configured, reinterpret_cast<const void*>(wino4_kernel<MODE, false, true, NTG>), LDS_BYTES, "nd_conv3x3_wino4_splitk")) return e;
    const long resident = (long)nd_device_cus() * W4Geo<NTG>::WG_PER_CU;
    hipLaunchKernelGGL((wino4_kernel<MODE, false, true, NTG>), dim3((unsigned)(a.total_wg < resident ? a.total_wg : resident)), dim3(256), LDS_BYTES, st, a);
    return 0;
}

template <bool DGRAD>
__device__ __forceinline__ void pack_wino4_body(const float* __restrict__ w, float* __restrict__ out, int cin, int cout, int n_c8, int n_cg) {
    constexpr float G[6][3] = {{0.25f, 0.f, 0.f}, {-1.f / 6, -1.f / 6, -1.f / 6}, {-1.f / 6, 1.f / 6, -1.f / 6},
                               {1.f / 24, 1.f / 12, 1.f / 6}, {1.f / 24, -1.f / 12, 1.f / 6}, {0.f, 0.f, 1.f}};
    const size_t total = (size_t)n_c8 * n_cg * 64;
    for (size_t i = blockIdx.x * (size_t)blockDim.x + threadIdx.x; i < total; i += (size_t)gridDim.x * blockDim.x) {
        const int l = (int)(i & 63);
        const size_t blk = i >> 6;
        const int cg = (int)(blk % n_cg), c8 = (int)(blk / n_cg);
        const int co = cg * 16 + (l & 15), ch0 = c8 * 8 + 2 * (l >> 4);
        float g[2][9];
        bool ok[2];
#pragma unroll
        for (int c = 0; c < 2; ++c) {
            const int ch = ch0 + c;
            ok[c] = ch < cin && co < cout;
            const float* gp = w + (ok[c] ? (DGRAD ? (size_t)ch * cout + co : (size_t)co * cin + ch) * 9 : 0);
#pragma unroll
            for (int j = 0; j < 9; ++j) g[c][j] = gp[DGRAD ? 8 - j : j];
        }
        float* o = out + blk * (18 * 256) + l * 4;
#pragma unroll
        for (int pp = 0; pp < 18; ++pp) {
            f32x4 v;
#pragma unroll
            for (int e = 0; e < 4; ++e) {
                const int pos = 2 * pp + (e >> 1), xi = pos / 6, nu = pos % 6, c = e & 1;
                double acc = 0.0;
#pragma unroll
                for (int rr = 0; rr < 3; ++rr)
#pragma unroll
                    for (int ss = 0; ss < 3; ++ss) acc += (double)G[xi][rr] * (double)g[c][rr * 3 + ss] * (double)G[nu][ss];
                v[e] = ok[c] ? (float)acc : 0.0f;
            }
            nd_st4(o + pp * 256, v);
        }
    }
}

template <bool DGRAD>
__global__ void pack_wino4_kernel(const float* __restrict__ w, float* __restrict__ out, int cin, int cout, int n_c8, int n_cg) {
    pack_wino4_body<DGRAD>(w, out, cin, cout, n_c8, n_cg);
}

__global__ void pack_wino4_batch_kernel(const nd_pack_item* __restrict__ items) {
    const nd_pack_item it = items[blockIdx.y];
    const int n_c8 = (((it.cin + 7) / 8) + 1) / 2 * 2, n_cg = (it.cout + 63) / 64 * 4;
    if (it.transposed) pack_wino4_body<true>(it.w, it.packed, it.cin, it.cout, n_c8, n_cg);
    else pack_wino4_body<false>(it.w, it.packed, it.cin, it.cout, n_c8, n_cg);
}

template <int MODE, bool STREAM, int NTG = 2, int NW = 4>
int launch4s(const Wino4Args& a, hipStream_t st) {
    static nd_device_once configured;
    constexpr int LDS_BYTES = W4Geo<NTG, NW>::LDS_BYTES;
    if (int e = nd_reserve_lds(configured, reinterpret_cast<const void*>(wino4_kernel<MODE, STREAM, false, NTG, NW>), LDS_BYTES, "nd_conv3x3_wino4")) return e;
    const long resident = (long)nd_device_cus() * W4Geo<NTG, NW>::WG_PER_CU;
    hipLaunchKernelGGL((wino4_kernel<MODE, STREAM, false, NTG, NW>), dim3((unsigned)(a.total_wg < resident ? a.total_wg : resident)), dim3(64 * NW), LDS_BYTES, st, a);
    return 0;
}

template <int MODE, int NTG = 2, int NW = 4>
int launch4(const Wino4Args& a, hipStream_t st) {
    static const long stream_min = (getenv("ND_W4_STREAM_MB") ? atol(getenv("ND_W4_STREAM_MB")) : 48) << 20;
    static const int stream_kinds = getenv("ND_W4_STREAM_KINDS") ? atoi(getenv("ND_W4_STREAM_KINDS")) : 7;
    const int kind = (MODE == ND_PRO_AFFINE_SILU || MODE == ND_PRO_AFFINE_MAP_SILU || MODE == ND_PRO_AFFINE_GENMAP_SILU) ? 2 : a.d.stats ? 1 : 4;
    const long out_bytes = (long)a.d.B * a.d.H * a.d.W * a.d.ldo * 4;
    return (out_bytes >= stream_min && (stream_kinds & kind)) ? launch4s<MODE, true, NTG, NW>(a, st) : launch4s<MODE, false, NTG, NW>(a, st);
}

}

extern "C" int64_t nd_pack_conv3x3_wino4_weight_floats(int cin, int cout) {
    return (int64_t)nd_round_up(nd_cdiv(cin, 8), 2) * nd_cdiv(nd_round_up(cout, 64), 16) * 18 * 256;
}

static int pack_wino4(const float* oihw, float* packed, int cin, int cout, int dgrad, void* stream) {
    ND_REQUIRE(oihw && packed, ND_E_BADARG, "nd_pack_conv3x3_wino4_weight: null pointer");
    ND_REQUIRE(cin > 0 && cout > 0, ND_E_BADARG, "nd_pack_conv3x3_wino4_weight: non-positive size");
    const int n_c8 = nd_round_up(nd_cdiv(cin, 8), 2), n_cg = nd_round_up(cout, 64) / 16;
    const size_t total = (size_t)n_c8 * n_cg * 64;
    const int blocks = (int)((total + 255) / 256 < 4096 ? (total + 255) / 256 : 4096);
    if (dgrad) hipLaunchKernelGGL(pack_wino4_kernel<true>, dim3(blocks), dim3(256), 0, (hipStream_t)stream, oihw, packed, cin, cout, n_c8, n_cg);
    else hipLaunchKernelGGL(pack_wino4_kernel<false>, dim3(blocks), dim3(256), 0, (hipStream_t)stream, oihw, packed, cin, cout, n_c8, n_cg);
    return nd_launch_status("nd_pack_conv3x3_wino4_weight");
}

extern "C" int nd_pack_conv3x3_wino4_weight(const float* oihw, float* packed, int cin, int cout, void* stream) {
    return pack_wino4(oihw, packed, cin, cout, 0, stream);
}

extern "C" int nd_pack_conv3x3_wino4_weight_dgrad(const float* oihw_fwd, float* packed, int cin, int cout, void* stream) {
    return pack_wino4(oihw_fwd, packed, cin, cout, 1, stream);
}

extern "C" int nd_pack_conv3x3_wino4_weights_batch(const nd_pack_item* items_dev, int n_items, void* stream) {
    ND_REQUIRE(items_dev && n_items > 0 && n_items <= 65535, ND_E_BADARG, "nd_pack_conv3x3_wino4_weights_batch: needs 1 .. 65535 items in device memory");
    hipLaunchKernelGGL(pack_wino4_batch_kernel, dim3(64, (unsigned)n_items), dim3(256), 0, (hipStream_t)stream, items_dev);
    return nd_launch_status("nd_pack_conv3x3_wino4_weights_batch");
}

extern "C" int nd_conv3x3_wino4_stat_slots(int H, int W) { return nd_cdiv(W, 16) * nd_cdiv(H, 16); }

static int w4_prepare(const nd_conv3x3* d, Wino4Args& a, int ntg = 2) {
    ND_REQUIRE(d, ND_E_BADARG, "nd_conv3x3_wino4: null descriptor");
    const nd_src& s = d->src;
    ND_REQUIRE(s.p0 && d->weight && d->out, ND_E_BADARG, "nd_conv3x3_wino4: null tensor pointer");
    ND_REQUIRE(d->B > 0 && d->H > 0 && d->W > 0 && d->cin > 0 && d->cout > 0, ND_E_BADARG, "nd_conv3x3_wino4: non-positive size");
    ND_REQUIRE(d->cin % 4 == 0 && d->cout % 4 == 0 && d->cin > KC4 && d->cout <= MAX_COUT, ND_E_SHAPE,
               "nd_conv3x3_wino4: cin=%d and cout=%d must be multiples of 4, cin > 16 (at least two K chunks), cout <= %d", d->cin, d->cout, MAX_COUT);
    ND_REQUIRE(s.c0 + s.c1 == d->cin && s.c0 % 4 == 0 && s.c1 % 4 == 0 && s.c0 > 0, ND_E_SHAPE,
               "nd_conv3x3_wino4: source channels %d+%d do not match cin=%d (multiples of 4)", s.c0, s.c1, d->cin);
    ND_REQUIRE((s.c1 == 0) == (s.p1 == nullptr), ND_E_BADARG, "nd_conv3x3_wino4: p1/c1 mismatch");
    ND_REQUIRE(s.ld0 >= s.c0 && s.ld0 % 4 == 0 && (s.c1 == 0 || (s.ld1 >= s.c1 && s.ld1 % 4 == 0)), ND_E_ALIGN,
               "nd_conv3x3_wino4: pixel strides must be >= channels and multiples of 4");
    ND_REQUIRE(nd_aligned16(s.p0) && nd_aligned16(s.p1) && nd_aligned16(d->weight) && nd_aligned16(s.mad) && nd_aligned16(d->out) &&
               nd_aligned16(d->bias), ND_E_ALIGN, "nd_conv3x3_wino4: pointers must be 16-byte aligned");
    ND_REQUIRE(d->ldo >= d->cout && d->ldo % 4 == 0, ND_E_SHAPE, "nd_conv3x3_wino4: ldo must be >= cout and a multiple of 4");
    const bool aff = s.mode == ND_PRO_AFFINE_SILU || s.mode == ND_PRO_AFFINE_MAP_SILU || s.mode == ND_PRO_AFFINE_GENMAP_SILU;
    ND_REQUIRE(s.mode == ND_PRO_NONE || aff || s.mode == ND_PRO_LEAKY || s.mode == ND_PRO_LEAKY_SECOND, ND_E_BADARG,
               "nd_conv3x3_wino4: unsupported prologue %d", s.mode);
    ND_REQUIRE(s.mode != ND_PRO_AFFINE_GENMAP_SILU || (ntg == 2 && s.map && s.gamma && s.beta && !s.upsample && !s.map_blocked && s.c1 == 0 && s.c0 % KC4 == 0 &&
                                                     nd_aligned16(s.map) && nd_aligned16(s.gamma) && nd_aligned16(s.beta)), ND_E_BADARG,
               "nd_conv3x3_wino4: the in-kernel map prologue needs silu(pos_emb) (map), mlp[1].weight (gamma) and mlp[1].bias (beta), 16-byte aligned, one source of whole "
               "16-channel chunks, no upsample addressing, the 16 x 32-region form");
    ND_REQUIRE(!aff || s.mad, ND_E_BADARG, "nd_conv3x3_wino4: affine prologue needs mad");
    ND_REQUIRE(s.mode != ND_PRO_AFFINE_MAP_SILU || (s.map && !s.upsample && nd_aligned16(s.map)), ND_E_BADARG,
               "nd_conv3x3_wino4: the map prologue needs a 16-byte aligned map and no upsample addressing");
    ND_REQUIRE(s.mode != ND_PRO_AFFINE_MAP_SILU || (long)(d->B * (long)d->H + 2) * d->W * 2 * (s.c0 + s.c1) * 4 < (1L << 30) - 65536, ND_E_SHAPE,
               "nd_conv3x3_wino4: a scale / shift map of 1 GiB or more");
    ND_REQUIRE(s.mode != ND_PRO_LEAKY_SECOND || s.p1, ND_E_BADARG, "nd_conv3x3_wino4: LEAKY_SECOND needs a second source");
    ND_REQUIRE(!s.map_blocked || (s.mode == ND_PRO_AFFINE_MAP_SILU && (s.c0 + s.c1) % 16 == 0), ND_E_BADARG,
               "nd_conv3x3_wino4: map_blocked needs the map prologue and a channel count that is a multiple of 16");
    ND_REQUIRE(!s.unshuffle, ND_E_BADARG, "nd_conv3x3_wino4: no unshuffle addressing");
    ND_REQUIRE(!s.upsample || (d->H % 2 == 0 && d->W % 2 == 0 && s.c1 == 0), ND_E_SHAPE,
               "nd_conv3x3_wino4: nearest-x2 upsample addressing needs even H, W and a single source");
    ND_REQUIRE((d->stats == nullptr) == (d->slot_count == nullptr), ND_E_BADARG, "nd_conv3x3_wino4: stats and slot_count go together");
    ND_REQUIRE(s.c1 == 0 || s.c0 % KC4 == 0, ND_E_SHAPE,
               "nd_conv3x3_wino4: first concat source has %d channels; a 16-channel K chunk must not straddle the sources", s.c0);
    ND_REQUIRE(d->W <= 2048 && d->H <= 32768, ND_E_SHAPE, "nd_conv3x3_wino4: image wider than 2048 (16-bit border table)");
    {
        const long px = (long)(d->B) * (d->H >> (s.upsample ? 1 : 0)) * (d->W >> (s.upsample ? 1 : 0));
        const long ext = px + (d->W >> (s.upsample ? 1 : 0)) + 2;
        ND_REQUIRE(ext * s.ld0 * 4 < (1L << 30) - 65536 && ext * s.ld1 * 4 < (1L << 30) - 65536 && ext < (1L << 24), ND_E_SHAPE,
                   "nd_conv3x3_wino4: a source tensor of 1 GiB or 16 M pixels or more");
    }

    ND_REQUIRE((long)d->B * d->H * d->W * d->ldo * 4 < (1L << 32) - 65536, ND_E_SHAPE, "nd_conv3x3_wino4: an output tensor of 4 GiB or more");

    a.d = *d;
    a.tiles_x = nd_cdiv(d->W, 16);
    a.tiles_y = nd_cdiv(d->H, 16);
    a.regions_x = nd_cdiv(d->W, 16 * ntg);
    a.n_tiles = nd_cdiv(d->cout, 64);
    a.n_cg = nd_round_up(d->cout, 64) / 16;
    a.n_c8 = nd_round_up(nd_cdiv(d->cin, 8), 2);
    a.slots = a.tiles_x * a.tiles_y;
    const long wg = (long)d->B * a.regions_x * a.tiles_y * a.n_tiles;
    ND_REQUIRE(wg < (1L << 31), ND_E_SHAPE, "nd_conv3x3_wino4: grid too large");
    a.total_wg = (int)wg;
    a.splits = 1;
    a.chunks_per_split = nd_cdiv(d->cin, KC4);
    return 0;
}

static int w4_splitk(const nd_conv3x3* d, float* workspace, int splits, void* stream, int ntg, const char* who) {
    Wino4Args a;
    if (int e = w4_prepare(d, a, ntg)) return e;
    ND_REQUIRE(workspace && nd_aligned16(workspace), ND_E_BADARG, "%s: the workspace must be a 16-byte aligned pointer", who);
    ND_REQUIRE(d->src.mode == ND_PRO_NONE || d->src.mode == ND_PRO_AFFINE_SILU, ND_E_BADARG,
               "%s: plain or GroupNorm-affine + SiLU sources (no map / LeakyReLU prologue)", who);
    const int n_chunks = nd_cdiv(d->cin, KC4);
    ND_REQUIRE((splits == 2 || splits == 4 || splits == 8) && d->cin % KC4 == 0 && n_chunks % splits == 0 && n_chunks / splits >= 2, ND_E_SHAPE,
               "%s: splits=%d must be 2, 4 or 8 and divide cin=%d into ranges of at least two whole 16-channel chunks", who, splits, d->cin);
    const long npix = (long)d->B * d->H * d->W;
    ND_REQUIRE((long)splits * npix * d->cout * 4 < (1L << 31), ND_E_SHAPE, "%s: partial sums of 2 GiB or more", who);
    ND_REQUIRE(d->cout % 4 == 0, ND_E_SHAPE, "%s: cout must be a multiple of 4", who);
    const float* bias = d->bias;
    float* out = d->out;
    const int ldo = d->ldo;
    a.d.out = workspace;  a.d.ldo = d->cout;  a.d.bias = nullptr;
    a.d.stats = nullptr;  a.d.slot_count = nullptr;
    a.splits = splits;
    a.chunks_per_split = n_chunks / splits;
    a.total_wg *= splits;
    hipStream_t st = (hipStream_t)stream;
    const bool aff = d->src.mode == ND_PRO_AFFINE_SILU;
    if (int rc = ntg == 1 ? (aff ? launch4_split<ND_PRO_AFFINE_SILU, 1>(a, st) : launch4_split<ND_PRO_NONE, 1>(a, st))
                          : (aff ? launch4_split<ND_PRO_AFFINE_SILU>(a, st) : launch4_split<ND_PRO_NONE>(a, st))) return rc;
    if (int e = nd_launch_status(who)) return e;
    if (d->stats) {
        const int n_cgrp = nd_cdiv(d->cout, 64);
        hipLaunchKernelGGL(w4_splitk_reduce_stats_kernel, dim3((unsigned)(d->B * a.tiles_x * a.tiles_y * n_cgrp)), dim3(256), 0, st, workspace, bias, out,
                           d->stats, d->slot_count, splits, d->B, d->H, d->W, d->cout, ldo, a.tiles_x, a.tiles_y, n_cgrp);
        return nd_launch_status(who);
    }
    const long total = npix * (d->cout / 4);
    const int blocks = (int)((total + 255) / 256 < 4096 ? (total + 255) / 256 : 4096);
    hipLaunchKernelGGL(w4_splitk_reduce_kernel, dim3(blocks), dim3(256), 0, st, workspace, bias, out, splits, npix, d->cout, ldo);
    return nd_launch_status(who);
}

extern "C" int nd_conv3x3_wino4_nhwc_f32(const nd_conv3x3* d, void* stream) {
    Wino4Args a;
    if (int e = w4_prepare(d, a)) return e;
    const nd_src& s = d->src;
    hipStream_t st = (hipStream_t)stream;
    int rc;
    switch (s.mode) {
        case ND_PRO_AFFINE_SILU: rc = launch4<ND_PRO_AFFINE_SILU>(a, st); break;
        case ND_PRO_AFFINE_MAP_SILU: rc = launch4<ND_PRO_AFFINE_MAP_SILU>(a, st); break;
        case ND_PRO_AFFINE_GENMAP_SILU: rc = launch4<ND_PRO_AFFINE_GENMAP_SILU>(a, st); break;
        case ND_PRO_LEAKY: rc = launch4<ND_PRO_LEAKY>(a, st); break;
        case ND_PRO_LEAKY_SECOND: rc = launch4<ND_PRO_LEAKY_SECOND>(a, st); break;
        default: rc = launch4<ND_PRO_NONE>(a, st); break;
    }
    if (rc) return rc;
    return nd_launch_status("nd_conv3x3_wino4_nhwc_f32");
}

extern "C" int nd_conv3x3_wino4_16_nhwc_f32(const nd_conv3x3* d, void* stream) {
    Wino4Args a;
    if (int e = w4_prepare(d, a, 1)) return e;
    ND_REQUIRE(d->src.mode == ND_PRO_NONE || d->src.mode == ND_PRO_AFFINE_SILU, ND_E_BADARG,
               "nd_conv3x3_wino4_16: plain or GroupNorm-affine + SiLU sources (no map / LeakyReLU prologue)");
    hipStream_t st = (hipStream_t)stream;
    if (int rc = d->src.mode == ND_PRO_AFFINE_SILU ? launch4<ND_PRO_AFFINE_SILU, 1>(a, st) : launch4<ND_PRO_NONE, 1>(a, st)) return rc;
    return nd_launch_status("nd_conv3x3_wino4_16_nhwc_f32");
}

static int w4_splits(long items, int cin) {
    const int n_chunks = nd_cdiv(cin, KC4);
    if (cin % KC4) return 1;
    static const long cap = getenv("ND_W4_SPLIT_ITEMS") ? atol(getenv("ND_W4_SPLIT_ITEMS")) : 256;
    static const int min_chunks = getenv("ND_W4_SPLIT_MIN_CHUNKS") ? atoi(getenv("ND_W4_SPLIT_MIN_CHUNKS")) : 4;
    int splits = 1;
    while (splits < 8 && items * splits * 2 <= cap && n_chunks % (splits * 2) == 0 && n_chunks / (splits * 2) >= min_chunks) splits *= 2;
    return splits;
}

extern "C" int nd_conv3x3_wino4_splitk_plan(int B, int H, int W, int cin, int cout) {
    if (B <= 0 || H <= 0 || W <= 0 || cin <= 0 || cout <= 0) return 1;
    return w4_splits((long)B * nd_cdiv(W, 32) * nd_cdiv(H, 16) * nd_cdiv(cout, 64), cin);
}

extern "C" int64_t nd_conv3x3_wino4_splitk_workspace_floats(int B, int H, int W, int cout, int splits) {
    if (B <= 0 || H <= 0 || W <= 0 || cout <= 0 || splits <= 0) return -1;
    return (int64_t)splits * B * H * W * cout;
}

extern "C" int nd_conv3x3_wino4_splitk_nhwc_f32(const nd_conv3x3* d, float* workspace, int splits, void* stream) {
    return w4_splitk(d, workspace, splits, stream, 2, "nd_conv3x3_wino4_splitk_nhwc_f32");
}

extern "C" int nd_conv3x3_wino4_16_splitk_plan(int H, int W, int cin, int cout) {
    if (H <= 0 || W <= 0 || cin <= 0 || cout <= 0 || cin % KC4) return 1;
    const long items = (long)nd_cdiv(W, 16) * nd_cdiv(H, 16) * nd_cdiv(cout, 64);
    const int n_chunks = cin / KC4;
    int splits = 1;
    while (splits < 8 && items * splits < 32 && n_chunks % (splits * 2) == 0 && n_chunks / (splits * 2) >= 4) splits *= 2;
    return splits;
}

extern "C" int nd_conv3x3_wino4_16_splitk_nhwc_f32(const nd_conv3x3* d, float* workspace, int splits, void* stream) {
    return w4_splitk(d, workspace, splits, stream, 1, "nd_conv3x3_wino4_16_splitk_nhwc_f32");
}
```

noisediff_amd/engine.py:

```python
from __future__ import annotations

import ctypes as C
import logging
import math
import os
import threading
from dataclasses import dataclass
from typing import Callable, Dict, List, Optional, Sequence, Tuple

import torch

from . import _lib as L
from .spec import (normalize_stage_attn, stage_attention_param_spec, ATTN_DIM_HEAD, ATTN_HEADS, ISO_DIM, ISO_TABLE_ROWS, POS_DIM, POS_GROUPS, RESNET_GROUPS, SHOT_GROUPS,
                   arch_param_spec, arch_traits, attention_param_spec, stage_dims)

GN_EPS = 1e-5
_log = logging.getLogger("noisediff_amd")
WINOGRAD = os.environ.get("ND_WINOGRAD", "1") != "0"
PREACT = True
PREACT_MIN = 256
CHAIN = True
_CHAIN_FIRST = (".ff.net.0.0.weight", ".fc1.weight")
_CHAIN_LATER = (".ff.net.2.weight", ".proj_out.weight", ".fc2.weight")
WINO2 = os.environ.get("ND_WINO2", "1") != "0"
MAP_BLOCKED = True
GENMAP = os.environ.get("ND_GENMAP", "1") != "0"
COND_STEP = True
WINO4 = os.environ.get("ND_WINO4", "1") != "0"
SPLIT_K = os.environ.get("ND_SPLIT_K", "0") != "0"
EIGHT_TILES_RULE = True
WINO4_16 = os.environ.get("ND_WINO4_16", "narrow")
WINO4_16_SPLIT = True
_ALIGN = 64
_SPLIT = os.environ.get("ND_SPLIT_GEMM", "1")
SPLIT_GEMM = _SPLIT != "0"
SPLIT_CHAIN, SPLIT_PW = _SPLIT in ("1", "chain"), _SPLIT in ("1", "pw")
TIME_TABLE = True
PROJ_TABLE = True
TIME_TABLE_ROWS = 1000


def _few_items(H: int, W: int, cout: int) -> bool:
    return ((H + 15) // 16) * ((W + 31) // 32) * ((cout + 63) // 64) <= 8


def _wino4_layer(cin: int, cout: int) -> bool:
    return cin > 16 and cin % 4 == 0 and cout % 4 == 0


_MAP_PRODUCERS = ("pos_block1.mlp.1.weight", "pos_block2.mlp.1.weight")


def _blocked_map_rows(C_: int) -> torch.Tensor:
    i = torch.arange(2 * C_)
    c, j = i // 32, i % 32
    return torch.where(j < 16, 16 * c + j, C_ + 16 * c + j - 16)


_CHAIN_SPLIT_LIMIT = (1 << 32) - (1 << 17)


def _split_layer(cin: int, cout: int) -> bool:
    return SPLIT_PW and cin % 32 == 0 and cin >= 64 and cout % 128 == 0


def _classify(name: str, shape: Sequence[int]) -> str:
    if ".attn.to_q." in name or ".attn.to_k." in name or ".norm1." in name:
        return "skip"
    if len(shape) == 4:
        k = shape[-1]
        if name == "pos_enc.weights.weight" or name.endswith(".g"):
            return "raw"
        if k == 7:
            return "conv7"
        if k == 3:
            return "conv3"
        if name.startswith("downs.") and name.endswith((".3.1.weight", ".2.1.weight")):
            return "pw_unshuffle"
        return "pw"
    if len(shape) == 2 and (".ff.net." in name):
        return "pw"
    return "raw"


@dataclass
class Slot:
    offset: int
    numel: int
    kind: str
    shape: Tuple[int, ...]


class Engine:

    def __init__(self, dim: int, device: torch.device, mid_attn: bool = False, inp_dim: int = 4, arch: str = "NoiseDiffNet", stage_attn=None):
        if device.type != "cuda":
            raise L.HipError("noisediff_amd runs on MI355X only: got device %r (there is no CPU path)" % (device,))
        self.lib = L.load()
        self.dim, self.device, self.mid_attn, self.inp_dim = dim, device, mid_attn, inp_dim
        self.arch, self.traits = arch, arch_traits(arch)
        self.spec = list(arch_param_spec(arch, dim, inp_dim))
        if mid_attn:
            self.spec += attention_param_spec("mid_attn", 8 * dim)
        self.stage_attn = normalize_stage_attn(stage_attn)
        if self.stage_attn:
            self.spec += stage_attention_param_spec(dim, self.stage_attn)
        self.resnet_names = [p.name[:-len(".mlp.1.weight")] for p in self.spec
                             if p.name.endswith(".mlp.1.weight") and len(p.shape) == 2]
        self.tproj_off: Dict[str, int] = {}
        self._layout()
        with torch.inference_mode(False):
            self.arena = torch.empty(self.arena_floats, dtype=torch.float32, device=device)
        with torch.cuda.device(device):
            s = C.c_void_p()
            L.call("nd_stream_create", C.byref(s))
        self.stream = s
        self.plans: Dict[Tuple[int, int, int], "Plan"] = {}
        self.loaded = False
        self.used: set = set()
        self.valid: Optional[set] = None

    def __del__(self):
        s, self.stream = getattr(self, "stream", None), None
        for q in (s,):
            if q:
                try:
                    L.call("nd_stream_sync", q)
                    L.call("nd_stream_destroy", q)
                except Exception:
                    pass

    def _layout(self) -> None:
        self.slots: Dict[str, Slot] = {}
        off = 0

        def add(name, numel, kind, shape):
            nonlocal off
            self.slots[name] = Slot(off, int(numel), kind, tuple(shape))
            off += (int(numel) + _ALIGN - 1) // _ALIGN * _ALIGN

        for p in self.spec:
            kind = _classify(p.name, p.shape)
            if kind == "skip":
                continue
            if kind == "conv3":
                n = self.lib.nd_pack_conv3x3_weight_floats(p.shape[1], p.shape[0])
                add(p.name + ".wino", self.lib.nd_pack_conv3x3_wino_weight_floats(p.shape[1], p.shape[0]), "derived", p.shape)
                if WINO4 and _wino4_layer(p.shape[1], p.shape[0]):
                    add(p.name + ".wino4", self.lib.nd_pack_conv3x3_wino4_weight_floats(p.shape[1], p.shape[0]), "derived", p.shape)
            elif kind in ("pw", "pw_unshuffle"):
                n = self.lib.nd_pack_pointwise_weight_floats(p.shape[1], p.shape[0])
                if p.name in _MAP_PRODUCERS and p.shape[0] % 32 == 0:
                    add(p.name + ".blk16", n, "derived", p.shape)
                    add(p.name[:-len("weight")] + "bias.blk16", p.shape[0], "derived", (p.shape[0],))
                    if GENMAP and p.shape[1] == POS_DIM == 8 and p.shape[0] % 32 == 0:
                        add(p.name + ".gen", p.shape[0] * p.shape[1], "derived", p.shape)
                if kind == "pw" and p.name.endswith(_CHAIN_FIRST + _CHAIN_LATER):
                    first = int(p.name.endswith(_CHAIN_FIRST))
                    add(p.name + ".chain", self.lib.nd_pack_chain_weight_floats(p.shape[1], p.shape[0], first), "derived", p.shape)
                    if SPLIT_CHAIN:
                        add(p.name + ".chain_s", self.lib.nd_pack_chain_weight_split_floats(p.shape[1], p.shape[0], first), "derived", p.shape)
                if kind == "pw" and _split_layer(p.shape[1], p.shape[0]):
                    add(p.name + ".split", self.lib.nd_pack_pointwise_weight_split_floats(p.shape[1], p.shape[0]), "derived", p.shape)
            elif kind == "conv7":
                n = 196 * p.shape[0]
                if SPLIT_PW and p.name == "init_conv.weight":
                    add(p.name + ".split", self.lib.nd_pack_conv7x7_weight_split_floats(p.shape[0]), "derived", p.shape)
            else:
                n = math.prod(p.shape)
            add(p.name, n, kind, p.shape)
        j = 0
        for r in self.resnet_names:
            self.tproj_off[r] = j
            j += self.slots[r + ".mlp.1.weight"].shape[0]
        self.tproj_rows = j
        add("tproj.weight", j * 4 * self.dim, "derived", (j, 4 * self.dim))
        add("tproj.bias", j, "derived", (j,))
        add("time_freqs", self.dim // 2, "derived", (self.dim // 2,))
        self.time_table = TIME_TABLE and 4 * self.dim <= 2048 and self.lib.nd_cond_step_lds_bytes(16, self.dim) <= 160 * 1024
        if self.time_table:
            add("time_table", TIME_TABLE_ROWS * 4 * self.dim, "derived", (TIME_TABLE_ROWS, 4 * self.dim))
            if PROJ_TABLE and self.tproj_rows % 4 == 0 and TIME_TABLE_ROWS * self.tproj_rows * 4 <= (192 << 20):
                add("tproj_table", TIME_TABLE_ROWS * self.tproj_rows, "derived", (TIME_TABLE_ROWS, self.tproj_rows))
        self.arena_floats = off

    def view(self, name: str) -> torch.Tensor:
        s = self.slots[name]
        return self.arena[s.offset:s.offset + s.numel]

    def p(self, name: str) -> int:
        s = self.slots[name]
        if self.valid is not None and name not in self.valid:
            raise L.HipError(f"arena slice {name!r} was not part of this rank's weight broadcast (it carried the slices of the plans "
                             "recorded before it): record the plan before Engine.broadcast(only_used=True), or broadcast the whole arena")
        self.used.add(name)
        return self.arena.data_ptr() + 4 * s.offset

    def load_state_dict(self, sd: Dict[str, torch.Tensor]) -> None:
        st = self.stream
        self.valid = None
        keep = []
        used = set(self.used)
        with torch.cuda.device(self.device):
            for p in self.spec:
                if p.name not in self.slots:
                    continue
                t = sd[p.name].detach().to(device=self.device, dtype=torch.float32).contiguous()
                if tuple(t.shape) != tuple(p.shape):
                    raise ValueError(f"{p.name}: shape {tuple(t.shape)} != {tuple(p.shape)}")
                keep.append(t)
                kind = self.slots[p.name].kind
                if kind == "raw":
                    self.view(p.name).copy_(t.reshape(-1))
            torch.cuda.synchronize(self.device)
            for p, t in zip([q for q in self.spec if q.name in self.slots], keep):
                kind, dst = self.slots[p.name].kind, self.p(p.name)
                if kind == "conv3":
                    L.call("nd_pack_conv3x3_weight", t.data_ptr(), dst, p.shape[1], p.shape[0], st)
                    L.call("nd_pack_conv3x3_wino_weight", t.data_ptr(), self.p(p.name + ".wino"), p.shape[1], p.shape[0], st)
                    if p.name + ".wino4" in self.slots:
                        L.call("nd_pack_conv3x3_wino4_weight", t.data_ptr(), self.p(p.name + ".wino4"), p.shape[1], p.shape[0], st)
                elif kind == "pw":
                    L.call("nd_pack_pointwise_weight", t.data_ptr(), dst, p.shape[1], p.shape[0], 0, st)
                    if p.name + ".blk16" in self.slots:
                        perm = _blocked_map_rows(p.shape[0] // 2).to(self.device)
                        tp = t[perm].contiguous()
                        keep.append(tp)
                        L.call("nd_pack_pointwise_weight", tp.data_ptr(), self.p(p.name + ".blk16"), p.shape[1], p.shape[0], 0, st)
                        bname = p.name[:-len("weight")] + "bias"
                        self.view(bname + ".blk16").copy_(sd[bname].detach().to(device=self.device, dtype=torch.float32)[perm])
                    if p.name + ".gen" in self.slots:
                        self.view(p.name + ".gen").copy_(t.reshape(-1))
                    if p.name + ".chain" in self.slots:
                        L.call("nd_pack_chain_weight", t.data_ptr(), self.p(p.name + ".chain"), p.shape[1], p.shape[0],
                               int(p.name.endswith(_CHAIN_FIRST)), st)
                    if p.name + ".chain_s" in self.slots:
                        L.call("nd_pack_chain_weight_split", t.data_ptr(), self.p(p.name + ".chain_s"), p.shape[1], p.shape[0],
                               int(p.name.endswith(_CHAIN_FIRST)), st)
                    if p.name + ".split" in self.slots:
                        L.call("nd_pack_pointwise_weight_split", t.data_ptr(), self.p(p.name + ".split"), p.shape[1], p.shape[0], st)
                elif kind == "pw_unshuffle":
                    L.call("nd_pack_pointwise_weight", t.data_ptr(), dst, p.shape[1], p.shape[0], p.shape[1] // 4, st)
                elif kind == "conv7":
                    L.call("nd_pack_conv7x7_weight", t.data_ptr(), dst, p.shape[0], st)
                    if p.name + ".split" in self.slots:
                        L.call("nd_pack_conv7x7_weight_split", t.data_ptr(), self.p(p.name + ".split"), p.shape[0], st)
            L.call("nd_stream_sync", st)
            tw = torch.cat([self.view(r + ".mlp.1.weight") for r in self.resnet_names])
            tb = torch.cat([self.view(r + ".mlp.1.bias") for r in self.resnet_names])
            self.view("tproj.weight").copy_(tw)
            self.view("tproj.bias").copy_(tb)
            half = self.dim // 2
            e = math.log(10000) / (half - 1)
            self.view("time_freqs").copy_(torch.exp(torch.arange(half) * -e).to(torch.float32))
            torch.cuda.synchronize(self.device)
            self._build_time_tables()
        self.loaded, self.valid, self.used = True, None, used

    _DERIVED_TABLES = ("time_table", "tproj_table")

    def _build_time_tables(self) -> None:
        if not self.time_table:
            return
        st, used = self.stream, set(self.used)
        with torch.cuda.device(self.device):
            L.call("nd_cond_table_build_f32", self.p("time_freqs"), self.p("time_mlp.1.weight"), self.p("time_mlp.1.bias"), self.p("time_mlp.3.weight"),
                   self.p("time_mlp.3.bias"), self.p("time_table"), TIME_TABLE_ROWS, self.dim, st)
            L.call("nd_stream_sync", st)
            if "tproj_table" in self.slots:
                ts = torch.arange(TIME_TABLE_ROWS, dtype=torch.int64, device=self.device)
                torch.cuda.synchronize(self.device)
                J = self.tproj_rows
                for t0 in range(0, TIME_TABLE_ROWS, 16):
                    nb = min(16, TIME_TABLE_ROWS - t0)
                    L.call("nd_cond_step_table_f32", ts.data_ptr() + 8 * t0, self.p("time_freqs"), self.p("time_mlp.1.weight"), self.p("time_mlp.1.bias"),
                           self.p("time_mlp.3.weight"), self.p("time_mlp.3.bias"), self.p("tproj.weight"), self.p("tproj.bias"),
                           self.p("tproj_table") + 4 * t0 * J, J, nb, self.dim, J, self.p("time_table"), TIME_TABLE_ROWS, st)
                L.call("nd_stream_sync", st)
        self.used = used

    def broadcast_state_dict(self, sd: Optional[Dict[str, torch.Tensor]], src: int = 0, group=None) -> int:
        import torch.distributed as dist
        names = [p for p in self.spec if p.name in self.slots]
        total = sum(math.prod(p.shape) for p in names)
        with torch.cuda.device(self.device), torch.inference_mode(False):
            if dist.get_rank(group) == src:
                flat = torch.cat([sd[p.name].detach().reshape(-1).to(torch.float32) for p in names]).to(self.device)
                if flat.numel() != total:
                    raise ValueError("broadcast_state_dict: the state dict does not match the network's parameter spec")
            else:
                flat = torch.empty(total, dtype=torch.float32, device=self.device)
            torch.cuda.synchronize(self.device)
            dist.broadcast(flat, src=src, group=group)
            torch.cuda.synchronize(self.device)
            views, at = {}, 0
            for p in names:
                n = math.prod(p.shape)
                views[p.name] = flat[at:at + n].view(*p.shape)
                at += n
        self.load_state_dict(views)
        return total * 4

    def broadcast(self, src: int = 0, group=None, only_used: bool = False) -> int:
        import torch.distributed as dist
        with torch.cuda.device(self.device):
            torch.cuda.synchronize(self.device)
            if not only_used:
                dist.broadcast(self.arena, src=src, group=group)
                nbytes = self.arena.numel() * 4
            else:
                tables = [n for n in self._DERIVED_TABLES if n in self.used]
                if tables:
                    for dep in ("time_freqs", "time_mlp.1.weight", "time_mlp.1.bias", "time_mlp.3.weight", "time_mlp.3.bias", "tproj.weight", "tproj.bias"):
                        self.used.add(dep)
                names = sorted((n for n in self.used if n not in self._DERIVED_TABLES), key=lambda n: self.slots[n].offset)
                every = [None] * dist.get_world_size(group)
                dist.all_gather_object(every, names, group=group)
                if any(e != names for e in every):
                    raise L.HipError("Engine.broadcast(only_used=True): the ranks recorded different plans")
                ranges: List[List[int]] = []
                for n in names:
                    sl = self.slots[n]
                    lo, hi = sl.offset, sl.offset + (sl.numel + _ALIGN - 1) // _ALIGN * _ALIGN
                    if ranges and ranges[-1][1] == lo:
                        ranges[-1][1] = hi
                    else:
                        ranges.append([lo, hi])
                is_src = dist.get_rank(group) == src
                with torch.inference_mode(False):
                    stage = (torch.cat([self.arena[lo:hi] for lo, hi in ranges]) if is_src
                             else torch.empty(sum(hi - lo for lo, hi in ranges), dtype=torch.float32, device=self.device))
                dist.broadcast(stage, src=src, group=group)
                if not is_src:
                    at = 0
                    for lo, hi in ranges:
                        self.arena[lo:hi].copy_(stage[at:at + hi - lo])
                        at += hi - lo
                    self.valid = set(names) | set(tables)
                    if tables:
                        torch.cuda.synchronize(self.device)
                        self._build_time_tables()
                nbytes = stage.numel() * 4
            torch.cuda.synchronize(self.device)
        self.loaded = True
        return nbytes

    def copy_from(self, other: "Engine") -> None:
        if other.arena_floats != self.arena_floats or not other.loaded:
            raise L.HipError("Engine.copy_from: the source engine has no weights or another layout")
        other.sync()
        torch.cuda.synchronize(other.device)
        with torch.cuda.device(self.device):
            self.arena.copy_(other.arena)
            torch.cuda.synchronize(self.device)
        self.loaded, self.valid = True, other.valid

    def plan(self, B: int, H: int, W: int, debug: bool = False, tag: int = 0, allow_empty: bool = False) -> "Plan":
        if not self.loaded and not allow_empty:
            raise L.HipError("Engine has no weights: call load_state_dict() or broadcast() first")
        key = (B, H, W, debug, tag)
        if key not in self.plans:
            self.plans[key] = Plan(self, B, H, W, debug)
        return self.plans[key]

    def sync(self) -> None:
        L.call("nd_stream_sync", self.stream)


Op = Tuple[Callable, tuple]


class Plan:

    def __init__(self, eng: Engine, B: int, H: int, W: int, debug: bool = False):
        self.debug, self.taps = debug, {}
        self.lock = threading.Lock()
        if H % 8 or W % 8:
            raise AssertionError(f"your input dimensions {(H, W)} need to be divisible by 8, given the unet")
        self.e, self.B, self.H, self.W = eng, B, H, W
        self.dev = eng.device
        self._keep: List[object] = []
        self._free: Dict[int, List[torch.Tensor]] = {}
        self.workspace_floats = 0
        d = eng.dim
        with torch.cuda.device(self.dev), torch.inference_mode(False):
            f = lambda *s: torch.empty(*s, dtype=torch.float32, device=self.dev)
            self.x = f(B, H, W, eng.inp_dim)
            self.clean = f(B, H, W, eng.inp_dim)
            self.position = f(B, 2, H, W)
            self.iso_idx = torch.zeros(B, dtype=torch.int64, device=self.dev)
            self.time = torch.zeros(B, dtype=torch.int64, device=self.dev)
            self.model_out = f(B, H, W, eng.inp_dim)
            self.nchw_tmp = f(B, eng.inp_dim, H, W)
            self.pos_emb = f(B, H, W, POS_DIM)
            self.posgen = (GENMAP and eng.traits.position and all(b + ".mlp.1.weight.gen" in eng.slots for b in ("pos_block1", "pos_block2")) and d % 16 == 0 and
                           self._wino4_kind("pos_block1.block2.proj", L.PRO_AFFINE_GENMAP_SILU, False, d, 0, d, 0, d, d, H, W,
                                            self._conv_rows(H, W, 0, d, 0, d, d, L.PRO_AFFINE_GENMAP_SILU)) == "wino4")
            self.posmap1 = self.posmap2 = None
            if self.posgen:
                self.pos_e = f(B, H, W, POS_DIM)
                self.pos_e_mad = torch.tensor([0.0, 1.0, 0.0], device=self.dev).repeat_interleave(POS_DIM).repeat(B).view(B, 3, POS_DIM).contiguous()
            else:
                self.posmap1 = f(B, H, W, 2 * d)
                self.posmap2 = f(B, H, W, 2 * d)
            self.posmap_blocked = (not self.posgen and MAP_BLOCKED and "pos_block1.mlp.1.weight.blk16" in eng.slots and
                                   self._wino4_takes("pos_block1.block2.proj", L.PRO_AFFINE_MAP_SILU, False, d, 0, d, 0, d, d, H, W))
            self.iso_emb = f(B, ISO_DIM)
            self.attn_names = [p.name[:-len(".attn.to_v.weight")] for p in eng.spec if p.name.endswith(".attn.to_v.weight")]
            self.cb = {n: f(B, eng.slots[n + ".proj_out.bias"].shape[0]) for n in self.attn_names}
            self.emb = f(B, d)
            self.t1 = f(B, 4 * d)
            self.st = f(B, 4 * d)
            self.tproj = f(B, eng.tproj_rows)
        self.cond_ops: List[Op] = []
        self.step_ops: List[Op] = []
        self._ops = self.cond_ops
        self._record_condition()
        self._ops = self.step_ops
        self._record_time()
        self._record_net()
        self.condition_set = False

    def _alloc(self, *shape) -> torch.Tensor:
        n = math.prod(shape)
        lst = self._free.get(n)
        if lst:
            return lst.pop().view(*shape)
        self.workspace_floats += n
        with torch.cuda.device(self.dev), torch.inference_mode(False):
            t = torch.empty(n, dtype=torch.float32, device=self.dev)
        self._keep.append(t)
        return t.view(*shape)

    def _tap(self, name: str, t: torch.Tensor) -> torch.Tensor:
        if self.debug:
            self.taps[name] = t
        return t

    def _release(self, *ts: torch.Tensor) -> None:
        if self.debug:
            return
        for t in ts:
            self._free.setdefault(t.numel(), []).append(t.reshape(-1))

    def _add(self, name: str, *args, meta: Optional[dict] = None) -> None:
        fn = getattr(self.e.lib, name)
        self._keep.append(args)
        self._ops.append((fn, args, name, meta))

    def _src(self, t: torch.Tensor, t2: Optional[torch.Tensor] = None, mode=L.PRO_NONE, **kw) -> L.Src:
        s = L.Src()
        s.p0, s.c0, s.ld0 = t.data_ptr(), t.shape[-1], t.shape[-1]
        if t2 is not None:
            s.p1, s.c1, s.ld1 = t2.data_ptr(), t2.shape[-1], t2.shape[-1]
        s.mode = mode
        for k, v in kw.items():
            setattr(s, k, v.data_ptr() if isinstance(v, torch.Tensor) else v)
        return s

    def _conv_rows(self, H: int, W: int, up: int, ld0: int, ld1: int, cin: int, cout: int, mode: int, splits: int = 1) -> int:
        sh, sw, lim = H >> up, W >> up, (1 << 30) - (1 << 16)

        def fits(b: int) -> bool:
            px = b * sh * sw + sw + 2
            return (px * 4 * max(ld0, ld1) < lim and px < (1 << 24) and b * H * W < (1 << 24) and b * H * W * cout * 4 < (1 << 32) - (1 << 16)
                    and (mode != L.PRO_AFFINE_MAP_SILU or (b * H + 2) * W * 8 * cin < lim) and splits * b * H * W * cout * 4 < (1 << 31))
        if fits(self.B):
            return self.B
        lo, hi = 1, self.B
        while lo < hi:
            mid = (lo + hi + 1) // 2
            lo, hi = (mid, hi) if fits(mid) else (lo, mid - 1)
        if not fits(lo):
            raise L.HipError(f"conv3x3 at {H} x {W} x {max(ld0, ld1)}: one sample exceeds the kernels' 1 GiB source limit")
        pieces = -(-self.B // lo)
        return -(-self.B // pieces)

    def conv3(self, name: str, src: L.Src, cin: int, cout: int, H: int, W: int, stats: bool):
        e = self.e
        out = self._alloc(self.B, H, W, cout)
        wino = WINOGRAD and H >= 16 and W >= 16
        up = 1 if src.upsample else 0
        rows = self._conv_rows(H, W, up, src.ld0, src.ld1, cin, cout, src.mode) if wino else self.B
        wino2 = (wino and WINO2 and not (src.mode == L.PRO_AFFINE_MAP_SILU and src.upsample)
                 and (src.c1 == 0 or src.c0 % 32 == 0) and rows * H * W < (1 << 24)
                 and rows * H * W * 4 * max(src.ld0, src.ld1, 2 * cin if src.mode == L.PRO_AFFINE_MAP_SILU else 0) < (1 << 31))
        w4kind = self._wino4_kind(name, src.mode, bool(src.upsample), src.c0, src.c1, src.ld0, src.ld1, cin, cout, H, W, rows) if wino else ""
        wino4 = bool(w4kind)
        if src.mode == L.PRO_AFFINE_GENMAP_SILU and w4kind != "wino4":
            raise L.HipError(f"{name}: maps formed in the kernel need conv3x3_wino4's 16 x 32-region form (Plan.posgen decides by the same rule)")
        if wino and not wino4 and (name + ".weight.wino4") in e.slots and src.mode in (L.PRO_NONE, L.PRO_AFFINE_SILU, L.PRO_AFFINE_MAP_SILU) and not _few_items(H, W, cout):
            _log.warning("%s (%d -> %d at %d x %d, batch %d): not on the F(4x4) kernel", name, cin, cout, H, W, self.B)
        st = sc = None
        slots = 0
        if stats:
            slots = (e.lib.nd_conv3x3_wino4_stat_slots(H, W) if wino4 else e.lib.nd_conv3x3_wino_stat_slots(H, W) if wino
                     else e.lib.nd_conv3x3_stat_slots(H, W, cout, self.B))
            st = self._alloc(self.B, slots, cout, 2)
            sc = self._alloc(slots)
        if src.map_blocked and not wino4:
            raise L.HipError(f"{name}: the scale / shift map was produced in the blocked layout but the layer does not run on conv3x3_wino4")
        lowlat_split = SPLIT_K and w4kind == "wino4" and src.mode in (L.PRO_NONE, L.PRO_AFFINE_SILU) and int(e.lib.nd_conv3x3_wino4_splitk_plan(self.B, H, W, cin, cout)) > 1
        weight = e.p(name + (".weight.wino4" if wino4 else ".weight.wino" if wino else ".weight"))
        entry = (f"nd_conv3x3_{w4kind}_nhwc_f32" if wino4 else "nd_conv3x3_wino2_nhwc_f32" if wino2 else
                 "nd_conv3x3_wino_nhwc_f32" if wino else "nd_conv3x3_nhwc_f32")
        tiling = (9016 if w4kind == "wino4_16" else 9004) if wino4 else 9002 if wino2 else 9001 if wino else e.lib.nd_conv3x3_tiling_id(self.B, H, W, cout)
        splits = int(e.lib.nd_conv3x3_wino4_splitk_plan(self.B, H, W, cin, cout)) if lowlat_split else 1
        if w4kind == "wino4_16" and WINO4_16_SPLIT:
            splits = int(e.lib.nd_conv3x3_wino4_16_splitk_plan(H, W, cin, cout))
        if splits > 1:
            rows = self._conv_rows(H, W, up, src.ld0, src.ld1, cin, cout, src.mode, splits)
        ws = self._alloc(splits * rows * H * W * cout) if splits > 1 else None
        sh, sw, ctot = H >> up, W >> up, src.c0 + src.c1
        for b0 in range(0, self.B, rows):
            nb = min(rows, self.B - b0)
            d = L.Conv3x3()
            s = L.Src.from_buffer_copy(src)
            if b0:
                s.p0 = src.p0 + 4 * b0 * sh * sw * src.ld0
                if src.p1:
                    s.p1 = src.p1 + 4 * b0 * sh * sw * src.ld1
                if src.mad:
                    s.mad = src.mad + 4 * b0 * 3 * ctot
                if src.map:
                    s.map = src.map + 4 * b0 * H * W * (POS_DIM if src.mode == L.PRO_AFFINE_GENMAP_SILU else 2 * ctot)
            d.src, d.weight, d.bias, d.out = s, weight, e.p(name + ".bias"), out.data_ptr() + 4 * b0 * H * W * cout
            d.B, d.H, d.W, d.cin, d.cout, d.ldo = nb, H, W, cin, cout, cout
            if stats:
                d.stats, d.slot_count = st.data_ptr() + 4 * b0 * slots * cout * 2, sc.data_ptr()
            meta = {"layer": name, "B": nb, "H": H, "W": W, "cin": cin, "cout": cout, "mode": int(src.mode), "tiling": tiling}
            if splits > 1:
                meta["splits"] = splits
                entry_s = "nd_conv3x3_wino4_16_splitk_nhwc_f32" if w4kind == "wino4_16" else "nd_conv3x3_wino4_splitk_nhwc_f32"
                self._add(entry_s, C.byref(d), ws.data_ptr(), splits, e.stream, meta=meta)
            else:
                self._add(entry, C.byref(d), e.stream, meta=meta)
            self._keep.append(d)
        if ws is not None:
            self._release(ws)
        return out, st, sc, slots

    def _wino4_kind(self, name: str, mode: int, upsample: bool, c0: int, c1: int, ld0: int, ld1: int, cin: int, cout: int, H: int, W: int, rows: Optional[int] = None) -> str:
        up = 1 if upsample else 0
        rows = self.B if rows is None else rows
        src_px = rows * (H >> up) * (W >> up) + (W >> up) + 2
        src_bytes = src_px * 4 * max(ld0, ld1)
        common = (WINOGRAD and WINO4 and H >= 16 and W >= 16 and cout <= 2048 and (name + ".weight.wino4") in self.e.slots
                  and W <= 2048 and (c1 == 0 or (c0 % 16 == 0 and not up)) and src_bytes < (1 << 30) - (1 << 16) and src_px < (1 << 24)
                  and (not up or (H % 2 == 0 and W % 2 == 0)))
        if not common:
            return ""
        takes16 = WINO4_16 != "0" and mode in (L.PRO_NONE, L.PRO_AFFINE_SILU) and (W % 16 == 0 or W >= 48)
        few = _few_items(H, W, cout)
        if takes16 and (WINO4_16 == "all" or W < 32 or (few and EIGHT_TILES_RULE and not SPLIT_K)):
            return "wino4_16"
        return "wino4" if self._wino4_takes(name, mode, upsample, c0, c1, ld0, ld1, cin, cout, H, W, rows) else ""

    def _wino4_takes(self, name: str, mode: int, upsample: bool, c0: int, c1: int, ld0: int, ld1: int, cin: int, cout: int, H: int, W: int, rows: Optional[int] = None) -> bool:
        up = 1 if upsample else 0
        if (WINO2 and not SPLIT_K and EIGHT_TILES_RULE and ((H + 15) // 16) * ((W + 31) // 32) * ((cout + 63) // 64) <= 8 and (c1 == 0 or c0 % 32 == 0)
                and not (mode == L.PRO_AFFINE_MAP_SILU and up)):
            return False
        rows = self.B if rows is None else rows
        src_px = rows * (H >> up) * (W >> up) + (W >> up) + 2
        src_bytes = src_px * 4 * max(ld0, ld1)
        return (WINOGRAD and WINO4 and H >= 16 and W >= 16 and cout <= 2048 and (name + ".weight.wino4") in self.e.slots
                and mode in (L.PRO_NONE, L.PRO_AFFINE_SILU, L.PRO_AFFINE_MAP_SILU, L.PRO_AFFINE_GENMAP_SILU)
                and not (mode == L.PRO_AFFINE_MAP_SILU and (up or (rows * H + 2) * W * 8 * cin >= (1 << 30) - (1 << 16)))
                and not (mode == L.PRO_AFFINE_GENMAP_SILU and (up or c1 or cin % 16))
                and W >= 32 and (W % 32 == 0 or W >= 96) and W <= 2048 and (c1 == 0 or (c0 % 16 == 0 and not up))
                and src_bytes < (1 << 30) - (1 << 16) and src_px < (1 << 24)
                and (not up or (H % 2 == 0 and W % 2 == 0)))

    def pw(self, name: str, src: L.Src, cin: int, cout: int, HW: int, W: int, act=L.ACT_NONE, bias=True,
           res0=None, res1=None, vec=None, gn_t=None, gn_mad=None, out=None, variant: str = "") -> torch.Tensor:
        e = self.e
        if out is None:
            out = self._alloc(self.B, HW, cout)
        d = L.Pointwise()
        d.src, d.out = src, out.data_ptr()
        d.bias = e.p(name + ".bias" + variant) if bias else None
        d.B, d.HW, d.W, d.cin, d.cout, d.ldo, d.act = self.B, HW, W, cin, cout, cout, act
        split = not variant and (name + ".weight.split") in e.slots and bool(e.lib.nd_pointwise_gemm_split_takes(C.byref(d)))
        d.weight = e.p(name + (".weight.split" if split else ".weight" + variant))
        if res0 is not None:
            d.res0, d.ldr0 = res0.data_ptr(), res0.shape[-1]
        if res1 is not None:
            d.res1, d.ldr1 = res1.data_ptr(), res1.shape[-1]
        if vec is not None:
            d.vec = vec.data_ptr()
        if gn_t is not None:
            d.gn_t, d.ldt, d.gn_mad = gn_t.data_ptr(), gn_t.shape[-1], gn_mad.data_ptr()
        self._add("nd_pointwise_gemm_split_nhwc_f32" if split else "nd_pointwise_gemm_nhwc_f32", C.byref(d), e.stream,
                  meta={"layer": name, "B": self.B, "HW": HW, "cin": cin, "cout": cout, "split": int(split)})
        self._keep.append(d)
        return out

    def gn_finalize(self, st, sc, slots: int, norm: str, C_: int, groups: int, ss_off: Optional[int]) -> torch.Tensor:
        e = self.e
        mad = self._alloc(self.B, 3, C_)
        ss = (self.tproj.data_ptr() + 4 * ss_off) if ss_off is not None else None
        self._add("nd_groupnorm_finalize_f32", st.data_ptr(), sc.data_ptr(), slots, e.p(norm + ".weight"), e.p(norm + ".bias"),
                  ss, e.tproj_rows, mad.data_ptr(), self.B, C_, groups, GN_EPS, e.stream)
        return mad

    def linear_rows(self, x: torch.Tensor, w: int, b: Optional[int], out: torch.Tensor, K: int, N: int, act_in=0, act_out=0):
        self._add("nd_linear_rows_f32", x.data_ptr(), x.shape[-1], w, b, out.data_ptr(), out.shape[-1], self.B, K, N,
                  act_in, act_out, self.e.stream)

    def resnet(self, name: str, x: torch.Tensor, skip: Optional[torch.Tensor], cout: int, H: int, W: int, groups: int,
               posmap: Optional[torch.Tensor] = None, extra_res: Optional[torch.Tensor] = None) -> torch.Tensor:
        cin = x.shape[-1] + (skip.shape[-1] if skip is not None else 0)
        HW = H * W
        c1, st1, sc1, n1 = self.conv3(name + ".block1.proj", self._src(x, skip), cin, cout, H, W, stats=True)
        ss_off = None if posmap is not None else self.e.tproj_off.get(name)
        mad1 = self.gn_finalize(st1, sc1, n1, name + ".block1.norm", cout, groups, ss_off)
        a1 = None
        if PREACT and posmap is None and cout >= PREACT_MIN and H >= 16 and W >= 16:
            a1 = self._alloc(self.B, HW, cout)
            self._add("nd_affine_silu_add_f32", c1.data_ptr(), cout, mad1.data_ptr(), None, cout, None, cout, a1.data_ptr(), cout,
                      self.B, HW, cout, self.e.stream,
                      meta={"layer": name + ".block1.act", "stream_bytes": 4.0 * self.B * HW * cout * 2})
            src2 = self._src(a1)
        else:
            if posmap is not None and self.posgen:
                src2 = self._src(c1, None, L.PRO_AFFINE_GENMAP_SILU, mad=mad1, map=self.pos_e, gamma=self.e.p(name + ".mlp.1.weight.gen"),
                                 beta=self.e.p(name + ".mlp.1.bias"))
            else:
                mode = L.PRO_AFFINE_MAP_SILU if posmap is not None else L.PRO_AFFINE_SILU
                src2 = self._src(c1, None, mode, mad=mad1, **({"map": posmap, "map_blocked": int(self.posmap_blocked)} if posmap is not None else {}))
        c2, st2, sc2, n2 = self.conv3(name + ".block2.proj", src2, cout, cout, H, W, stats=True)
        if a1 is not None:
            self._release(a1)
        mad2 = self.gn_finalize(st2, sc2, n2, name + ".block2.norm", cout, groups, None)
        if cin != cout:
            assert extra_res is None
            out = self.pw(name + ".res_conv", self._src(x, skip), cin, cout, HW, W, gn_t=c2, gn_mad=mad2)
        else:
            assert skip is None
            out = self._alloc(self.B, HW, cout)
            self._add("nd_affine_silu_add_f32", c2.data_ptr(), cout, mad2.data_ptr(), x.data_ptr(), cout,
                      extra_res.data_ptr() if extra_res is not None else None, cout, out.data_ptr(), cout,
                      self.B, HW, cout, self.e.stream,
                      meta={"layer": name + ".tail", "stream_bytes": 4.0 * self.B * HW * cout * (4 if extra_res is not None else 3)})
        self._release(c1, st1, sc1, mad1, c2, st2, sc2, mad2)
        return out.view(self.B, H, W, cout)

    def chain(self, name: str, src: L.Src, stages, HW: int) -> torch.Tensor:
        e = self.e
        out = self._alloc(self.B, HW, stages[-1][2])
        split = all((layer + ".weight.chain_s") in e.slots for layer, *_ in stages) and (src.c1 == 0 or stages[0][1] <= 16)
        ldo = stages[-1][2]
        rows = self.B
        if split:
            per = 4 * HW * max(src.ld0, src.ld1, ldo)
            rows = max(1, min(self.B, _CHAIN_SPLIT_LIMIT // per))
            rows = -(-self.B // -(-self.B // rows))
        for b0 in range(0, self.B, rows):
            nb = min(rows, self.B - b0)
            d = L.Chain()
            sp = L.Src.from_buffer_copy(src)
            if b0:
                sp.p0 = src.p0 + 4 * b0 * HW * src.ld0
                if src.p1:
                    sp.p1 = src.p1 + 4 * b0 * HW * src.ld1
                if src.vec:
                    sp.vec = src.vec + 4 * b0 * (src.c0 + src.c1)
            d.src, d.out, d.n_stages, d.B, d.HW, d.ldo = sp, out.data_ptr() + 4 * b0 * HW * ldo, len(stages), nb, HW, ldo
            for i, (layer, cin, cout, act, res) in enumerate(stages):
                d.st[i].weight, d.st[i].bias = e.p(layer + (".weight.chain_s" if split else ".weight.chain")), e.p(layer + ".bias")
                d.st[i].cin, d.st[i].cout, d.st[i].act, d.st[i].res = cin, cout, act, res
            self._add("nd_pointwise_chain_split_nhwc_f32" if split else "nd_pointwise_chain_nhwc_f32", C.byref(d), e.stream,
                      meta={"layer": name, "B": nb, "HW": HW, "cin": stages[0][1], "cout": stages[-1][2], "split": int(split),
                            "flop_per_px": 2.0 * sum(c_in * c_out for _, c_in, c_out, _, _ in stages)})
            self._keep.append(d)
        return out

    def _chain_ok(self, HW: int, widths) -> bool:
        w = list(widths) + [0] * (4 - len(widths))
        return CHAIN and HW % 32 == 0 and bool(self.e.lib.nd_pointwise_chain_supported(*w))

    def attn_block(self, name: str, x: torch.Tensor, H: int, W: int) -> torch.Tensor:
        Cc, HW = x.shape[-1], H * W
        cb = self.cb[name]
        if self._chain_ok(HW, (Cc, 2 * Cc, Cc, Cc)):
            ln = self._src(x, None, L.PRO_LAYERNORM, vec=cb, gamma=self.e.p(name + ".norm2.weight"), beta=self.e.p(name + ".norm2.bias"))
            y = self.chain(name + ".ff+proj_out", ln,
                           [(name + ".ff.net.0.0", Cc, 2 * Cc, L.ACT_GELU, L.CHAIN_RES_NONE),
                            (name + ".ff.net.2", 2 * Cc, Cc, L.ACT_NONE, L.CHAIN_RES_INPUT),
                            (name + ".proj_out", Cc, Cc, L.ACT_NONE, L.CHAIN_RES_INPUT_RAW)], HW)
            return y.view(self.B, H, W, Cc)
        kw = {}
        rs = None
        if Cc > 64:
            rs = self._alloc(self.B, HW, 2)
            self._add("nd_layernorm_stats_f32", x.data_ptr(), Cc, cb.data_ptr(), rs.data_ptr(), self.B, HW, Cc, 1e-5, self.e.stream)
            kw["rowstats"] = rs
        ln = self._src(x, None, L.PRO_LAYERNORM, vec=cb, gamma=self.e.p(name + ".norm2.weight"), beta=self.e.p(name + ".norm2.bias"), **kw)
        h1 = self.pw(name + ".ff.net.0.0", ln, Cc, 2 * Cc, HW, W, act=L.ACT_GELU)
        x2 = self.pw(name + ".ff.net.2", self._src(h1), 2 * Cc, Cc, HW, W, res0=x, vec=cb)
        y = self.pw(name + ".proj_out", self._src(x2), Cc, Cc, HW, W, res0=x)
        self._release(h1, x2)
        if rs is not None:
            self._release(rs)
        return y.view(self.B, H, W, Cc)

    def mlp(self, name: str, src: L.Src, cin: int, hid: int, cout: int, H: int, W: int, res0=None) -> torch.Tensor:
        if res0 is None and src.mode == L.PRO_NONE and self._chain_ok(H * W, (cin, hid, cout)):
            o = self.chain(name, src, [(name + ".fc1", cin, hid, L.ACT_GELU, L.CHAIN_RES_NONE),
                                       (name + ".fc2", hid, cout, L.ACT_NONE, L.CHAIN_RES_NONE)], H * W)
            return o.view(self.B, H, W, cout)
        h = self.pw(name + ".fc1", src, cin, hid, H * W, W, act=L.ACT_GELU)
        o = self.pw(name + ".fc2", self._src(h), hid, cout, H * W, W, res0=res0)
        self._release(h)
        return o.view(self.B, H, W, cout)

    def _record_condition(self) -> None:
        e, B, H, W, st = self.e, self.B, self.H, self.W, self.e.stream
        tr = e.traits
        if tr.position:
            pe = self._alloc(B, H, W, 3 * POS_DIM)
            self._add("nd_pos_enc_f32", self.position.data_ptr(), e.p("pos_enc.weights.weight"), e.p("pos_enc.weights.bias"),
                      pe.data_ptr(), B, H, W, POS_DIM, st)
            h = self.pw("pos_mlp.fc1", self._src(pe), 3 * POS_DIM, 2 * POS_DIM, H * W, W, act=L.ACT_GELU)
            self.pw("pos_mlp.fc2", self._src(h), 2 * POS_DIM, POS_DIM, H * W, W, out=self.pos_emb)
            if self.posgen:
                self._add("nd_affine_silu_add_f32", self.pos_emb.data_ptr(), POS_DIM, self.pos_e_mad.data_ptr(), None, POS_DIM, None, POS_DIM,
                          self.pos_e.data_ptr(), POS_DIM, B, H * W, POS_DIM, st, meta={"layer": "pos_emb.silu", "stream_bytes": 8.0 * B * H * W * POS_DIM})
            for blk, dst in (() if self.posgen else (("pos_block1", self.posmap1), ("pos_block2", self.posmap2))):
                self.pw(blk + ".mlp.1", self._src(self.pos_emb, None, L.PRO_SILU), POS_DIM, 2 * e.dim, H * W, W, out=dst,
                        variant=".blk16" if self.posmap_blocked else "")
            self._release(pe, h)
        if tr.iso_attn:
            self._add("nd_embedding_rows_f32", self.iso_idx.data_ptr(), e.p("iso_embed.weight"), self.iso_emb.data_ptr(), B,
                      ISO_TABLE_ROWS, ISO_DIM, st)
            inner = ATTN_HEADS * ATTN_DIM_HEAD
            v = self._alloc(B, inner)
            for n in self.attn_names:
                Cc = self.cb[n].shape[-1]
                self.linear_rows(self.iso_emb, e.p(n + ".attn.to_v.weight"), None, v, ISO_DIM, inner)
                self.linear_rows(v, e.p(n + ".attn.to_out.0.weight"), e.p(n + ".attn.to_out.0.bias"), self.cb[n], inner, Cc)
            self._release(v)
        self.clean_emb = None
        if tr.cond_branch:
            ce = self._alloc(B, H, W, e.dim)
            self._add("nd_conv7x7_c4_f32", self.clean.data_ptr(), e.p("cond_init_conv.weight"), e.p("cond_init_conv.bias"),
                      ce.data_ptr(), e.dim, B, H, W, e.dim, st)
            self.clean_emb = self._tap("clean_emb", self.resnet("cond_res_block1", ce, None, e.dim, H, W, RESNET_GROUPS))
            self._release(ce)

    def _record_time(self) -> None:
        e, d = self.e, self.e.dim
        if COND_STEP and 4 * d <= 2048 and e.lib.nd_cond_step_lds_bytes(self.B, d) <= 160 * 1024:
            args = (self.time.data_ptr(), e.p("time_freqs"), e.p("time_mlp.1.weight"), e.p("time_mlp.1.bias"),
                    e.p("time_mlp.3.weight"), e.p("time_mlp.3.bias"), e.p("tproj.weight"), e.p("tproj.bias"), self.tproj.data_ptr(),
                    e.tproj_rows, self.B, d, e.tproj_rows)
            if e.time_table and "tproj_table" in e.slots and e.tproj_rows % 4 == 0:
                self._add("nd_cond_step_ptable_f32", *args, e.p("time_table"), TIME_TABLE_ROWS, e.p("tproj_table"), e.stream)
            elif e.time_table:
                self._add("nd_cond_step_table_f32", *args, e.p("time_table"), TIME_TABLE_ROWS, e.stream)
            else:
                self._add("nd_cond_step_f32", *args, e.stream)
            return
        self._add("nd_sinusoidal_time_emb_f32", self.time.data_ptr(), e.p("time_freqs"), self.emb.data_ptr(), self.B, d // 2, e.stream)
        self.linear_rows(self.emb, e.p("time_mlp.1.weight"), e.p("time_mlp.1.bias"), self.t1, d, 4 * d, act_out=L.ACT_GELU)
        self.linear_rows(self.t1, e.p("time_mlp.3.weight"), e.p("time_mlp.3.bias"), self.st, 4 * d, 4 * d, act_out=L.ACT_SILU)
        self.linear_rows(self.st, e.p("tproj.weight"), e.p("tproj.bias"), self.tproj, 4 * d, e.tproj_rows)

    def _record_net(self) -> None:
        e, B, H, W, d = self.e, self.B, self.H, self.W, self.e.dim
        G, tr = RESNET_GROUPS, self.e.traits
        shot_noise = None
        if tr.shot_branch:
            r_shot = self.mlp("shot_mlp1", self._src(self.clean, self.x), 2 * e.inp_dim, d, d, H, W)
            s = self.attn_block("shot_attn", r_shot, H, W)
            s2 = self.mlp("shot_mlp2", self._src(s), d, d, d, H, W)
            s3 = self.resnet("shot_time", s2, None, d, H, W, SHOT_GROUPS, extra_res=r_shot)
            shot_noise = self._tap("shot_noise", self.mlp("shot_mlp3", self._src(s3), d, d, e.inp_dim, H, W))
            for nm, tt in (("shot_mlp1", r_shot), ("shot_attn", s), ("shot_mlp2", s2), ("shot_time", s3)):
                self._tap(nm, tt)
            self._release(r_shot, s, s2, s3)
        x0 = self._alloc(B, H, W, d)
        stem_split = "init_conv.weight.split" in e.slots
        self._add("nd_conv7x7_c4_split_f32" if stem_split else "nd_conv7x7_c4_f32", self.x.data_ptr(),
                  e.p("init_conv.weight.split" if stem_split else "init_conv.weight"), e.p("init_conv.bias"), x0.data_ptr(), d, B, H, W, d, e.stream)
        self._tap("init_conv", x0)
        xin = x0
        if tr.cond_branch:
            xin, *_ = self.conv3("cond_concat_conv", self._src(x0, self.clean_emb), 2 * d, d, H, W, stats=False)
            self._tap("cond_concat", xin)
        pm1, pm2 = ((self.pos_e, self.pos_e) if self.posgen else (self.posmap1, self.posmap2)) if tr.position else (None, None)
        x = self._tap("pos_block1", self.resnet("pos_block1", xin, None, d, H, W, POS_GROUPS, posmap=pm1))
        if xin is not x0:
            self._release(xin)
        rs = 3 if tr.iso_attn else 2
        hs: List[torch.Tensor] = []
        h, w = H, W
        for i, (cin, cout) in enumerate(stage_dims(d)):
            p = f"downs.{i}"
            x1 = self.resnet(p + ".0", x, None, cin, h, w, G)
            self._release(x)
            x2 = self.resnet(p + ".1", x1, None, cin, h, w, G)
            if e.stage_attn and e.stage_attn[i]:
                x2 = self._stage_attention(f"down_attns.{i}", e.stage_attn[i], x2, h, w)
            hs += [x1, x2]
            xa = self.attn_block(p + ".2", x2, h, w) if tr.iso_attn else x2
            self._tap(p + ".0", x1); self._tap(p + ".1", x2); self._tap(p + ".2", xa)
            if i == 3:
                x, *_ = self.conv3(f"{p}.{rs}", self._src(xa), cin, cout, h, w, stats=False)
            else:
                h, w = h // 2, w // 2
                x = self.pw(f"{p}.{rs}.1", self._src(xa, None, L.PRO_NONE, unshuffle=1, c0=4 * cin, ld0=cin), 4 * cin, cout,
                            h * w, w).view(B, h, w, cout)
            if xa is not x2:
                self._release(xa)
            self._tap(f"down{i}", x)
        mid = x.shape[-1]
        xm = self.resnet("mid_block1", x, None, mid, h, w, G)
        self._release(x)
        if e.mid_attn:
            xm = self._mid_attention(xm, h, w)
        x = self._tap("mid", self.resnet("mid_block2", xm, None, mid, h, w, G))
        self._release(xm)
        for i, (cin, cout) in enumerate(reversed(stage_dims(d))):
            p = f"ups.{i}"
            sk = hs.pop()
            x1 = self.resnet(p + ".0", x, sk, cout, h, w, G)
            self._release(x, sk)
            sk = hs.pop()
            x2 = self.resnet(p + ".1", x1, sk, cout, h, w, G)
            self._release(x1, sk)
            if e.stage_attn and e.stage_attn[3 - i]:
                x2 = self._stage_attention(f"up_attns.{i}", e.stage_attn[3 - i], x2, h, w)
            xa = self.attn_block(p + ".2", x2, h, w) if tr.iso_attn else x2
            if xa is not x2:
                self._release(x2)
            if i == 3:
                x, *_ = self.conv3(f"{p}.{rs}", self._src(xa), cout, cin, h, w, stats=False)
            else:
                h, w = h * 2, w * 2
                x, *_ = self.conv3(f"{p}.{rs}.1", self._src(xa, None, L.PRO_NONE, upsample=1), cout, cin, h, w, stats=False)
            self._release(xa)
            self._tap(p + ".0", x1); self._tap(p + ".1", x2); self._tap(p + ".2", xa); self._tap(f"up{i}", x)
        xp = self._tap("pos_block2", self.resnet("pos_block2", x, None, d, H, W, POS_GROUPS, posmap=pm2))
        self._release(x)
        xf = self._tap("final_res_block", self.resnet("final_res_block", xp, x0, d, H, W, G))
        self._release(xp, x0)
        self.pw("final_conv", self._src(xf), d, e.inp_dim, H * W, W, res0=shot_noise, out=self.model_out)
        self._release(xf)
        if shot_noise is not None:
            self._release(shot_noise)

    def _mid_attention(self, x: torch.Tensor, h: int, w: int, prefix: str = "mid_attn") -> torch.Tensor:
        e, B, Cc, N = self.e, self.B, x.shape[-1], h * w
        hid = ATTN_HEADS * ATTN_DIM_HEAD
        xn = self._alloc(B, N, Cc)
        self._add("nd_rmsnorm_nhwc_f32", x.data_ptr(), Cc, e.p(prefix + ".norm.g"), xn.data_ptr(), Cc, B, N, Cc, e.stream)
        qkv = self.pw(prefix + ".to_qkv", self._src(xn), Cc, 3 * hid, N, w, bias=False)
        att = self._alloc(B, N, hid)
        self._add("nd_attention_mfma_f32", qkv.data_ptr(), 3 * hid, att.data_ptr(), hid, B, N, ATTN_HEADS, ATTN_DIM_HEAD, e.stream)
        y = self.pw(prefix + ".to_out", self._src(att), hid, Cc, N, w, res0=x)
        self._release(xn, qkv, att, x)
        return y.view(B, h, w, Cc)

    def _stage_attention(self, prefix: str, kind: str, x: torch.Tensor, h: int, w: int) -> torch.Tensor:
        if kind == "full":
            return self._mid_attention(x, h, w, prefix)
        e, B, Cc, N = self.e, self.B, x.shape[-1], h * w
        hid = ATTN_HEADS * ATTN_DIM_HEAD
        xn = self._alloc(B, N, Cc)
        self._add("nd_rmsnorm_nhwc_f32", x.data_ptr(), Cc, e.p(prefix + ".norm.g"), xn.data_ptr(), Cc, B, N, Cc, e.stream)
        qkv = self.pw(prefix + ".to_qkv", self._src(xn), Cc, 3 * hid, N, w, bias=False)
        att = self._alloc(B, N, hid)
        ws = self._alloc(int(e.lib.nd_linear_attention_workspace_floats(B, N, ATTN_HEADS)))
        self._add("nd_linear_attention_f32", qkv.data_ptr(), 3 * hid, att.data_ptr(), hid, ws.data_ptr(), B, N, ATTN_HEADS, ATTN_DIM_HEAD, e.stream)
        o = self.pw(prefix + ".to_out.0", self._src(att), hid, Cc, N, w)
        y = self._alloc(B, N, Cc)
        self._add("nd_rmsnorm_add_nhwc_f32", o.data_ptr(), Cc, e.p(prefix + ".to_out.1.g"), x.data_ptr(), Cc, y.data_ptr(), Cc, B, N, Cc, e.stream)
        self._release(xn, qkv, att, ws, o, x)
        return y.view(B, h, w, Cc)

    @staticmethod
    def run(ops: List[Op]) -> None:
        for fn, args, name, _meta in ops:
            r = fn(*args)
            if r != 0:
                L.check(r, name)

    def set_condition(self, condition) -> None:
        B, H, W, e = self.B, self.H, self.W, self.e
        tr = e.traits
        if torch.is_tensor(condition):
            if tr.position or tr.iso_attn:
                raise TypeError(f"{e.arch} needs the condition dict (clean_img, position, iso_ratio_idx), got a tensor")
            condition = {"clean_img": condition}
        clean = condition["clean_img"]
        if tuple(clean.shape) != (B, e.inp_dim, H, W):
            raise ValueError(f"condition shapes: clean_img {tuple(clean.shape)} do not match batch {(B, e.inp_dim, H, W)}")
        with torch.cuda.device(self.dev):
            self.nchw_tmp.copy_(clean.to(self.dev, torch.float32))
            if tr.position:
                pos = condition["position"]
                if tuple(pos.shape) != (B, 2, H, W):
                    raise ValueError(f"condition shapes: position {tuple(pos.shape)} do not match batch {(B, 2, H, W)}")
                self.position.copy_(pos.to(self.dev, torch.float32))
            if tr.iso_attn:
                iso = condition["iso_ratio_idx"]
                if tuple(iso.shape) != (B,):
                    raise ValueError(f"condition shapes: iso_ratio_idx {tuple(iso.shape)} do not match batch {(B,)}")
                iso = iso.to(torch.int64)
                if int(iso.min()) < 0 or int(iso.max()) >= ISO_TABLE_ROWS:
                    raise IndexError("iso_ratio_idx out of range for nn.Embedding(100, 16)")
                self.iso_idx.copy_(iso.to(self.dev))
            torch.cuda.synchronize(self.dev)
            L.call("nd_nchw_to_nhwc_f32", self.nchw_tmp.data_ptr(), self.clean.data_ptr(), B, e.inp_dim, H, W, e.stream)
            self.run(self.cond_ops)
            e.sync()
        self.condition_set = True

    def load_x(self, x_nchw: torch.Tensor) -> None:
        e = self.e
        with torch.cuda.device(self.dev):
            self.nchw_tmp.copy_(x_nchw.to(self.dev, torch.float32))
            torch.cuda.synchronize(self.dev)
            L.call("nd_nchw_to_nhwc_f32", self.nchw_tmp.data_ptr(), self.x.data_ptr(), self.B, e.inp_dim, self.H, self.W, e.stream)

    def read_nchw(self, nhwc: torch.Tensor) -> torch.Tensor:
        e = self.e
        with torch.cuda.device(self.dev), torch.inference_mode(False):
            out = torch.empty(self.B, e.inp_dim, self.H, self.W, dtype=torch.float32, device=self.dev)
            L.call("nd_nhwc_to_nchw_f32", nhwc.data_ptr(), out.data_ptr(), self.B, e.inp_dim, self.H, self.W, e.stream)
            e.sync()
        return out

    def forward(self, x_nchw: torch.Tensor, time: torch.Tensor) -> torch.Tensor:
        if not self.condition_set:
            raise L.HipError("Plan.forward: set_condition() first")
        with torch.cuda.device(self.dev):
            self.time.copy_(time.to(self.dev, torch.int64))
        self.load_x(x_nchw)
        self.run(self.step_ops)
        return self.read_nchw(self.model_out)
```

Measured before the change: 0.9404 patches/s.

## Add Winograd F(4x4) conv variant using 32x32x2 MFMA with restructured wave split

Adds a wino4x kernel path that computes the Winograd-domain GEMM with v_mfma_f32_32x32x2_f32 instead of 16x16x4. It reassigns waves so each covers 32 output channels for one tile half, and changes the LDS and weight addressing and the accumulator layout to match. The output transform and epilogue are rewritten to exchange halves through LDS, and the input transform for the next tile is deferred past the epilogue. The engine routes plain and affine-SiLU wino4 layers without split-K or upsample to it by default. It aims to raise MFMA throughput and cut operand traffic per FLOP, at the cost of one workgroup per CU, an extra LDS exchange and a less overlapped transform.

Result: no change. 0.9413 patches/s (median of 4 runs) (+0.1%).

```diff
diff --git a/include/noisediff_hip.h b/include/noisediff_hip.h
--- a/include/noisediff_hip.h
+++ b/include/noisediff_hip.h
@@ -75,6 +75,8 @@
 
 int nd_conv3x3_wino4_nhwc_f32(const nd_conv3x3* d, void* stream);
 int nd_conv3x3_wino4_16_nhwc_f32(const nd_conv3x3* d, void* stream);
+int nd_conv3x3_wino4x_nhwc_f32(const nd_conv3x3* d, void* stream);
+int nd_conv3x3_wino4x_supported(int H, int W, int cin, int cout, int mode, int upsample);
 int nd_conv3x3_wino4_stat_slots(int H, int W);
 int64_t nd_pack_conv3x3_wino4_weight_floats(int cin, int cout);
 int nd_pack_conv3x3_wino4_weight(const float* oihw, float* packed, int cin, int cout, void* stream);
diff --git a/noisediff_amd/_lib.py b/noisediff_amd/_lib.py
--- a/noisediff_amd/_lib.py
+++ b/noisediff_amd/_lib.py
@@ -83,6 +83,8 @@
     "nd_pack_conv3x3_wino_weight_dgrad": (i32, [vp, vp, i32, i32, vp]),
     "nd_conv3x3_wino4_nhwc_f32": (i32, [C.POINTER(Conv3x3), vp]),
     "nd_conv3x3_wino4_16_nhwc_f32": (i32, [C.POINTER(Conv3x3), vp]),
+    "nd_conv3x3_wino4x_nhwc_f32": (i32, [C.POINTER(Conv3x3), vp]),
+    "nd_conv3x3_wino4x_supported": (i32, [i32, i32, i32, i32, i32, i32]),
     "nd_pack_conv3x3_wino4_weight_floats": (i64, [i32, i32]),
     "nd_pack_conv3x3_wino4_weight": (i32, [vp, vp, i32, i32, vp]),
     "nd_pack_conv3x3_wino4_weight_dgrad": (i32, [vp, vp, i32, i32, vp]),
@@ -195,7 +197,7 @@
 
 _UNCHECKED = {"nd_version", "nd_last_error", "nd_stream_device", "nd_conv3x3_wgrad_form", "nd_adam_chunk_elements", "nd_conv7x7_c4_wgrad_workspace_floats", "nd_conv3x3_stat_slots", "nd_conv3x3_tiling_id", "nd_pack_conv3x3_weight_floats",
               "nd_pack_pointwise_weight_floats", "nd_linear_attention_workspace_floats", "nd_conv3x3_wino_stat_slots", "nd_conv3x3_wino4_stat_slots",
-              "nd_pack_conv3x3_wino_weight_floats", "nd_pack_conv3x3_wino4_weight_floats", "nd_conv3x3_wino4_splitk_plan", "nd_conv3x3_wino4_16_splitk_plan", "nd_conv3x3_wino4_splitk_workspace_floats", "nd_token_sum_workspace_floats", "nd_cond_step_lds_bytes", "nd_conv3x3_wgrad_workspace_floats",
+              "nd_pack_conv3x3_wino_weight_floats", "nd_pack_conv3x3_wino4_weight_floats", "nd_conv3x3_wino4_splitk_plan", "nd_conv3x3_wino4x_supported", "nd_conv3x3_wino4_16_splitk_plan", "nd_conv3x3_wino4_splitk_workspace_floats", "nd_token_sum_workspace_floats", "nd_cond_step_lds_bytes", "nd_conv3x3_wgrad_workspace_floats",
               "nd_groupnorm_train_workspace_floats", "nd_linear_wgrad_workspace_floats",
               "nd_layernorm_train_workspace_floats", "nd_groupnorm_silu_train_workspace_floats", "nd_conv3x3_wgrad_cat_workspace_floats",
               "nd_convt2x2_wgrad_workspace_floats", "nd_image_quality_workspace_bytes", "nd_illum_scale_workspace_bytes"}
diff --git a/noisediff_amd/csrc/conv3x3_wino4.hip b/noisediff_amd/csrc/conv3x3_wino4.hip
--- a/noisediff_amd/csrc/conv3x3_wino4.hip
+++ b/noisediff_amd/csrc/conv3x3_wino4.hip
@@ -108,6 +108,10 @@
 #define W4_MFMA_AZ(acc, uv, vv) asm volatile(W4_NOP "v_mfma_f32_16x16x4_f32 %0, %2, %1, 0" : "=&a"(acc) : "v"(uv), "v"(vv))
 #define W4_MFMA_VZ(acc, uv, vv) asm volatile(W4_NOP "v_mfma_f32_16x16x4_f32 %0, %2, %1, 0" : "=&v"(acc) : "v"(uv), "v"(vv))
 #define W4_MFMA_DRAIN() asm volatile("s_nop 15\n\ts_nop 15" ::: "memory")
+#define W4X_MFMA_A(acc, uv, vv)  asm volatile(W4_NOP "v_mfma_f32_32x32x2_f32 %0, %2, %1, %0" : "+a"(acc) : "v"(uv), "v"(vv))
+#define W4X_MFMA_V(acc, uv, vv)  asm volatile(W4_NOP "v_mfma_f32_32x32x2_f32 %0, %2, %1, %0" : "+v"(acc) : "v"(uv), "v"(vv))
+#define W4X_MFMA_AZ(acc, uv, vv) asm volatile(W4_NOP "v_mfma_f32_32x32x2_f32 %0, %2, %1, 0" : "=&a"(acc) : "v"(uv), "v"(vv))
+#define W4X_MFMA_VZ(acc, uv, vv) asm volatile(W4_NOP "v_mfma_f32_32x32x2_f32 %0, %2, %1, 0" : "=&v"(acc) : "v"(uv), "v"(vv))
 
 __device__ __forceinline__ void w4_bt(const f32x2 (&d)[6], f32x2 (&t)[6]) {
     const f32x2 c4 = {4.0f, 4.0f}, cm4 = {-4.0f, -4.0f}, cm5 = {-5.0f, -5.0f}, c2 = {2.0f, 2.0f}, cm2 = {-2.0f, -2.0f};
@@ -137,11 +141,13 @@
     }
 }
 
-template <int MODE, bool STREAM, bool SPLIT = false, int NTG = 2, int NW = 4>
-__global__ __launch_bounds__((64 * NW), (W4Geo<NTG, NW>::WG_PER_CU)) void wino4_kernel(const Wino4Args a) {
+template <int MODE, bool STREAM, bool SPLIT, int NTG, int NW, bool X>
+__device__ __forceinline__ void wino4_body(const Wino4Args& a) {
+    static_assert(!X || (NTG == 2 && NW == 4 && !SPLIT), "the 32x32x2 form: 16 x 32 regions, four waves, no split-K");
     using Geo = W4Geo<NTG, NW>;
     constexpr int NT = Geo::NT, TGW = Geo::TGW;
-    constexpr int RAW_FLOATS = Geo::RAW_FLOATS, BIAS_OFF_BYTES = Geo::BIAS_OFF_BYTES, ACC_AGPR = Geo::ACC_AGPR, REG_W = Geo::REG_W, HALO_W = Geo::HALO_W;
+    constexpr int RAW_FLOATS = Geo::RAW_FLOATS, BIAS_OFF_BYTES = Geo::BIAS_OFF_BYTES, REG_W = Geo::REG_W, HALO_W = Geo::HALO_W;
+    constexpr int ACC_AGPR = X ? 16 : Geo::ACC_AGPR;
     constexpr bool MAP = MODE == ND_PRO_AFFINE_MAP_SILU;
     constexpr bool GEN = MODE == ND_PRO_AFFINE_GENMAP_SILU;
     constexpr bool MAPX = MAP || GEN;
@@ -157,6 +163,7 @@
     const int mtg = NW == 8 ? wave >> 2 : 0;
     const int tg = TGW == 2 ? wave >> 1 : mtg, rh = (wave >> 1) & 1, ch2 = wave & 1;
     const int tile = lane & 15, kq = lane >> 4;
+    const int xh = wave >> 1, cw = wave & 1;
 
     const int wgid = nd_xcd_remap(blockIdx.x, gridDim.x);
     const int t_begin = (int)((long)wgid * a.total_wg / gridDim.x), t_end = (int)((long)(wgid + 1) * a.total_wg / gridDim.x);
@@ -349,7 +356,8 @@
         *reinterpret_cast<lds_f32x4_ptr>(daddr) = v;
     };
 
-    const unsigned d_lds = (unsigned)((kq >> 1) * 512 + tile * 32 + (kq & 1) * 16);
+    const unsigned d_lds = X ? (unsigned)(((lane >> 4) & 1) * (VD_FLOATS * 4) + tile * 32 + (lane >> 5) * 16 + xh * (9 * 2048))
+                             : (unsigned)((kq >> 1) * 512 + tile * 32 + (kq & 1) * 16);
 
     auto xf_addr = [&](unsigned (&t_addr)[12]) {
 #pragma unroll
@@ -435,26 +443,36 @@
 
     const __amdgpu_buffer_rsrc_t wrsrc = __builtin_amdgcn_make_buffer_rsrc(
         const_cast<float*>(a.d.weight), 0, (int)((long)a.n_c8 * a.n_cg * 18 * 256 * 4), 0x00020000);
-    const unsigned wvoff = (unsigned)(lane * 16);
-    auto wblock = [&](int c8_, int cg_) { return __builtin_amdgcn_readfirstlane(((c8_ * a.n_cg + cg_) * 18) * 1024); };
-
-    f32x4 acc[TGW * NPOS];
+    const unsigned wvoff = X ? (unsigned)(((lane >> 4) & 1) * (18 * 1024) + ((lane & 15) + 16 * (lane >> 5)) * 16) : (unsigned)(lane * 16);
+    auto wblock = [&](int c8_, int cg_) { return __builtin_amdgcn_readfirstlane(((c8_ * a.n_cg + cg_) * 18 + (X ? 9 * xh : 0)) * 1024); };
+    auto cg_of = [&](int nt_) { return nt_ * 4 + (X ? 2 * cw : (wave & 3)); };
+
+    using acc_t = std::conditional_t<X, f32x16, f32x4>;
+    acc_t acc[X ? NPOS / 2 : TGW * NPOS];
     f32x4 U[UR];
-    f32x4 Vr[W4_VR][TGW];
+    f32x4 Vr[W4_VR][X ? 1 : TGW];
     static_assert(36 % UR == 0, "the ring must close over a chunk's two stages of 18 fragments");
     auto load_u = [&](int slot, int q, int wb) {
 #if !(W4_ABLATE & 2)
-        U[slot % UR] = __builtin_bit_cast(f32x4, __builtin_amdgcn_raw_buffer_load_b128(wrsrc, wvoff, wb + q * 1024, W4_U_AUX));
+        U[slot % UR] = __builtin_bit_cast(f32x4, __builtin_amdgcn_raw_buffer_load_b128(wrsrc, wvoff, wb + q * (X ? 512 : 1024), W4_U_AUX));
 #endif
     };
     auto read_v = [&](const char* v0base, const char* v1base, int pp) {
-        Vr[pp % W4_VR][0] = *reinterpret_cast<const f32x4*>(v0base + pp * 2048);
-        if (TGW == 2) Vr[pp % W4_VR][TGW - 1] = *reinterpret_cast<const f32x4*>(v1base + pp * 2048);
+        if constexpr (X) Vr[pp % W4_VR][0] = *reinterpret_cast<const f32x4*>(v0base + (pp >> 1) * 2048 + (pp & 1) * 512);
+        else {
+            Vr[pp % W4_VR][0] = *reinterpret_cast<const f32x4*>(v0base + pp * 2048);
+            if (TGW == 2) Vr[pp % W4_VR][TGW - 1] = *reinterpret_cast<const f32x4*>(v1base + pp * 2048);
+        }
     };
     auto mfma = [&](auto first_c, int idx, float av, float bv) {
         constexpr bool FIRST = decltype(first_c)::value;
-        if (idx < ACC_AGPR) { if (FIRST) W4_MFMA_AZ(acc[idx], av, bv); else W4_MFMA_A(acc[idx], av, bv); }
-        else                { if (FIRST) W4_MFMA_VZ(acc[idx], av, bv); else W4_MFMA_V(acc[idx], av, bv); }
+        if constexpr (X) {
+            if (idx < ACC_AGPR) { if (FIRST) W4X_MFMA_AZ(acc[idx], av, bv); else W4X_MFMA_A(acc[idx], av, bv); }
+            else                { if (FIRST) W4X_MFMA_VZ(acc[idx], av, bv); else W4X_MFMA_V(acc[idx], av, bv); }
+        } else {
+            if (idx < ACC_AGPR) { if (FIRST) W4_MFMA_AZ(acc[idx], av, bv); else W4_MFMA_A(acc[idx], av, bv); }
+            else                { if (FIRST) W4_MFMA_VZ(acc[idx], av, bv); else W4_MFMA_V(acc[idx], av, bv); }
+        }
     };
     auto stage = [&](auto first_c, auto off_c, auto din_c, auto dout_c, const char* v0base, const char* v1base, int wb, int nb, auto&& pre, auto&& mid) {
         constexpr int OFF = decltype(off_c)::value, DIN = decltype(din_c)::value, DOUT = decltype(dout_c)::value;
@@ -472,9 +490,15 @@
             if (pp + W4_VR - 1 < 18) read_v(v0base, v1base, pp + W4_VR - 1);
             pre(pp);
             const f32x4 u = U[(OFF + pp) % UR];
-            const f32x4 va = Vr[pp % W4_VR][0], vb = Vr[pp % W4_VR][TGW - 1];
+            const f32x4 va = Vr[pp % W4_VR][0], vb = Vr[pp % W4_VR][X ? 0 : TGW - 1];
             __builtin_amdgcn_sched_barrier(0);
-            if (TGW == 2) {
+            if constexpr (X) {
+                const int p0 = 2 * (pp >> 1);
+                if ((pp & 1) == 0) { mfma(first_c, p0, u.x, va.x);  mfma(first_c, p0 + 1, u.z, va.z); }
+                else { mfma(std::false_type{}, p0, u.x, va.x);  mfma(std::false_type{}, p0 + 1, u.z, va.z); }
+                mfma(std::false_type{}, p0, u.y, va.y);
+                mfma(std::false_type{}, p0 + 1, u.w, va.w);
+            } else if (TGW == 2) {
                 mfma(first_c, 4 * pp + 0, u.x, va.x);
                 mfma(first_c, 4 * pp + 1, u.x, vb.x);
                 mfma(first_c, 4 * pp + 2, u.z, va.z);
@@ -500,7 +524,21 @@
         }
     };
 
+    auto read_accx = [&](int p, int r) -> f32x2 {
+        f32x2 v = {0.0f, 0.0f};
+        if constexpr (X) {
+            if (p >= ACC_AGPR) {
+                asm volatile("" : "+v"(acc[p]));
+                return f32x2{acc[p][r], acc[p][r + 1]};
+            }
+            asm volatile("v_accvgpr_read_b32 %0, %1" : "=v"(v.x) : "a"(acc[p][r]));
+            asm volatile("v_accvgpr_read_b32 %0, %1" : "=v"(v.y) : "a"(acc[p][r + 1]));
+        }
+        return v;
+    };
     auto read_acc2 = [&](int idx, int h) -> f32x2 {
+        if constexpr (X) return f32x2{0.0f, 0.0f};
+        else {
         if (idx >= ACC_AGPR) {
             asm volatile("" : "+v"(acc[idx]));
             return h ? f32x2{acc[idx].z, acc[idx].w} : f32x2{acc[idx].x, acc[idx].y};
@@ -514,6 +552,7 @@
             asm volatile("v_accvgpr_read_b32 %0, %1" : "=v"(r.y) : "a"(acc[idx].w));
         }
         return r;
+        }
     };
 
     int b, ty, rx, nt, sp;
@@ -524,7 +563,7 @@
 #pragma unroll
     for (int k = 0; k < RAW_IT; ++k) stage_issue_one(k, ptab[k * NT], std::true_type{});
     {
-        const int wb = wblock(SPLIT ? 2 * sp * n_chunks : 0, nt * 4 + (wave & 3));
+        const int wb = wblock(SPLIT ? 2 * sp * n_chunks : 0, cg_of(nt));
 #pragma unroll
         for (int q = 0; q < UR_EPI; ++q) load_u(q, q, wb);
     }
@@ -557,7 +596,7 @@
             if (nt1 == a.n_tiles) { nt1 = 0;  if (++rx1 == a.regions_x) { rx1 = 0;  if (++ty1 == a.tiles_y) { ty1 = 0;  ++b1;  if (SPLIT && b1 == a.d.B) { b1 = 0;  ++sp1; } } } }
         }
         const int ch0 = SPLIT ? sp * n_chunks : 0, ch0n = SPLIT ? sp1 * n_chunks : 0;
-        const int cg = nt * 4 + (wave & 3), cg_next = (more ? nt1 : nt) * 4 + (wave & 3);
+        const int cg = cg_of(nt), cg_next = cg_of(more ? nt1 : nt);
 
         auto chunk = [&](int ch, auto first_c, auto last_c) {
             const char* v0cur = reinterpret_cast<const char*>(Vd + mtg * VD_FLOATS) + d_lds;
@@ -611,12 +650,13 @@
                     }
                 } else if (pp < RAW_IT) stage_commit_one(pp, tab1, 0u);
                 if constexpr (TGW == 2) {
-                    if (pp == W4_XF_AT) {
+                    constexpr bool XF_HERE = !(X && last);
+                    if (XF_HERE && pp == W4_XF_AT) {
                         asm volatile("s_waitcnt lgkmcnt(0)" ::: "memory");
                         __builtin_amdgcn_s_barrier();
                         xf_addr(t_addr);
                     }
-                    if (pp > W4_XF_AT && pp <= W4_XF_AT + 6) xf_read(T, t_addr, pp - W4_XF_AT - 1);
+                    if (XF_HERE && pp > W4_XF_AT && pp <= W4_XF_AT + 6) xf_read(T, t_addr, pp - W4_XF_AT - 1);
                 }
             };
             W4_T0();
@@ -632,7 +672,12 @@
             if (!FIRST && !last && ch == 2) W4_ACC(stamp_third);
 #endif
             W4_T0();
-            if constexpr (TGW == 2) {
+            if constexpr (X && last) {
+                asm volatile("s_waitcnt lgkmcnt(0)" ::: "memory");
+                __builtin_amdgcn_s_barrier();
+                W4_ACC(stamp_wait);
+                return;
+            } else if constexpr (TGW == 2) {
                 xf_finish(T, vd_tg, [&] {
                     W4_ACC(stamp_xf);
                     W4_T0();
@@ -664,64 +709,102 @@
         const __amdgpu_buffer_rsrc_t orsrc = __builtin_amdgcn_make_buffer_rsrc(a.d.out, 0, (int)((unsigned)(SPLIT ? a.splits : 1) * a.d.B * H * W * a.d.ldo * 4u), 0x00020000);
         int Wt = __builtin_amdgcn_readfirstlane(W), ldot = __builtin_amdgcn_readfirstlane(a.d.ldo);
         asm volatile("" : "+s"(Wt), "+s"(ldot));
-#pragma unroll
-        for (int j = 0; j < TGW; ++j) {
-            const int tx = NTG * rx + (TGW == 2 ? j : mtg);
-            if (tx < a.tiles_x) {
-                int l15 = lane;
-                asm volatile("" : "+v"(l15));
-                l15 &= 15;
-                const int co = cg * 16 + l15;
-                const bool cok = co < Cout;
-                float z0 = 0.0f;
-                asm volatile("" : "+v"(z0));
-                const float* const bias_p = bias_lds + co;
-                const int py0 = ty * 16 + 4 * kq, px0 = tx * 16;
-                f32x2 sum2 = {z0, z0}, sq2 = {z0, z0}, cnt2 = {z0, z0};
-                float pivot = z0;
-                const bool full = ty * 16 + 16 <= H && tx * 16 + 16 <= W && cg * 16 + 16 <= Cout;
-                const bool want_stats = a.d.stats != nullptr;
-                const unsigned lane_off = (unsigned)((((unsigned)(SPLIT ? sp * a.d.B + b : b) * H + py0) * Wt + px0) * ldot + co) * 4u;
-                auto emit = [&](auto full_c, auto stats_c) {
-                    constexpr bool FULL = decltype(full_c)::value, STATS = decltype(stats_c)::value;
-                    int step4 = ldot * 16, back3 = ldot * -12, rowadv = (Wt - 7) * ldot * 4;
-                    asm volatile("" : "+s"(step4), "+s"(back3), "+s"(rowadv));
-                    const f32x2 c2 = {2.0f, 2.0f}, c4 = {4.0f, 4.0f}, c8 = {8.0f, 8.0f};
+        if constexpr (X) {
+            char* const xb_out = reinterpret_cast<char*>(Vd) + wave * 16384 + lane * 16;
+            const char* const xb_in = reinterpret_cast<const char*>(Vd) + (wave ^ 2) * 16384 + lane * 16;
+            int l31 = lane;
+            asm volatile("" : "+v"(l31));
+            const int kk = l31 >> 5;
+            l31 &= 31;
+            const int co = cg * 16 + l31;
+            const bool cok = co < Cout;
+            float z0 = 0.0f;
+            asm volatile("" : "+v"(z0));
+            const float* const bias_p = bias_lds + co;
+            const int tx = 2 * rx + xh, px0 = tx * 16;
+            const bool tin = tx < a.tiles_x;
+            f32x2 sum2 = {z0, z0}, sq2 = {z0, z0}, cnt2 = {z0, z0};
+            float pivot = z0;
+            const bool full = ty * 16 + 16 <= H && tx * 16 + 16 <= W && cg * 16 + 32 <= Cout;
+            const bool want_stats = a.d.stats != nullptr;
+            auto emit = [&](auto half_c, auto full_c, auto stats_c) {
+                constexpr int HALF = decltype(half_c)::value;
+                constexpr bool FULL = decltype(full_c)::value, STATS = decltype(stats_c)::value;
+                int step4 = ldot * 16, back3 = ldot * -12, rowadv = (Wt - 7) * ldot * 4;
+                asm volatile("" : "+s"(step4), "+s"(back3), "+s"(rowadv));
+                const f32x2 c2 = {2.0f, 2.0f}, c4 = {4.0f, 4.0f}, c8 = {8.0f, 8.0f};
+                auto zpart = [&](int g, int h, f32x2 (&Z)[4][6]) {
+#pragma unroll
+                    for (int nu = 0; nu < 6; ++nu) {
+                        auto M = [&](int xil) { return read_accx(xil * 6 + nu, 4 * g + 2 * h); };
+                        if (HALF == 0) {
+                            f32x2 m1 = M(1);
+                            const f32x2 m2 = M(2);
+                            if (nu == 1) m1 += *bias_p;
+                            const f32x2 p = m1 + m2, q = m1 - m2;
+                            Z[0][nu] = M(0) + p;
+                            Z[1][nu] = q;
+                            Z[2][nu] = p;
+                            Z[3][nu] = q;
+                        } else {
+                            const f32x2 m3 = M(0), m4 = M(1);
+                            const f32x2 r = m3 + m4, u = m3 - m4;
+                            Z[0][nu] = r;
+                            Z[1][nu] = c2 * u;
+                            Z[2][nu] = c4 * r;
+                            Z[3][nu] = __builtin_elementwise_fma(c8, u, M(2));
+                        }
+                        __builtin_amdgcn_sched_barrier(0);
+                    }
+                };
+                auto yrow = [&](const f32x2 (&z)[6], f32x2 (&y)[4]) {
+                    const f32x2 ta = z[1] + z[2], tb = z[1] - z[2], tc = z[3] + z[4], te = z[3] - z[4];
+                    y[0] = z[0] + ta + tc;
+                    y[1] = __builtin_elementwise_fma(c2, te, tb);
+                    y[2] = __builtin_elementwise_fma(c4, tc, ta);
+                    y[3] = __builtin_elementwise_fma(c8, te, tb) + z[5];
+                };
+#pragma unroll
+                for (int ro = 0; ro < 2; ++ro) {
+#pragma unroll
+                    for (int h = 0; h < 2; ++h) {
+                        f32x2 Z[4][6];
+                        zpart(2 * (1 - HALF) + ro, h, Z);
+#pragma unroll
+                        for (int i = 0; i < 4; ++i) {
+                            f32x2 y[4];
+                            yrow(Z[i], y);
+                            *reinterpret_cast<f32x4*>(xb_out + ((h * 4 + i) * 2) * 1024) = f32x4{y[0].x, y[0].y, y[1].x, y[1].y};
+                            *reinterpret_cast<f32x4*>(xb_out + ((h * 4 + i) * 2 + 1) * 1024) = f32x4{y[2].x, y[2].y, y[3].x, y[3].y};
+                        }
+                    }
+                    asm volatile("s_waitcnt lgkmcnt(0)" ::: "memory");
+                    __builtin_amdgcn_s_barrier();
+                    const int py0 = ty * 16 + 4 * (2 * ro + kk);
+                    const unsigned lane_off = (unsigned)((((unsigned)b * H + py0) * Wt + px0) * ldot + co) * 4u;
                     const int rowlim = FULL ? 4 : H - py0, collim = FULL ? 16 : W - px0;
 #pragma unroll
                     for (int h = 0; h < 2; ++h) {
                         int soff = h * 32 * ldot;
                         asm volatile("" : "+s"(soff));
+                        f32x4 rv[8];
+#pragma unroll
+                        for (int k = 0; k < 8; ++k) rv[k] = *reinterpret_cast<const f32x4*>(xb_in + (h * 8 + k) * 1024);
                         f32x2 Z[4][6];
-#pragma unroll
-                        for (int nu = 0; nu < 6; ++nu) {
-                            auto M = [&](int xi) { return read_acc2(TGW * (xi * 6 + nu) + j, h); };
-                            f32x2 m1 = M(1);
-                            const f32x2 m2 = M(2);
-                            if (nu == 1) m1 += Geo::BIAS_LDS ? *bias_p : bias_r;
-                            const f32x2 p = m1 + m2, q = m1 - m2;
-                            const f32x2 m3 = M(3), m4 = M(4);
-                            const f32x2 r = m3 + m4, u = m3 - m4;
-                            Z[0][nu] = M(0) + p + r;
-                            Z[1][nu] = __builtin_elementwise_fma(c2, u, q);
-                            Z[2][nu] = __builtin_elementwise_fma(c4, r, p);
-                            Z[3][nu] = __builtin_elementwise_fma(c8, u, q) + M(5);
-                            __builtin_amdgcn_sched_barrier(0);
-                        }
+                        zpart(2 * HALF + ro, h, Z);
 #pragma unroll
                         for (int i = 0; i < 4; ++i) {
-                            const f32x2 (&z)[6] = Z[i];
-                            const f32x2 ta = z[1] + z[2], tb = z[1] - z[2], tc = z[3] + z[4], te = z[3] - z[4];
                             f32x2 y[4];
-                            y[0] = z[0] + ta + tc;
-                            y[1] = __builtin_elementwise_fma(c2, te, tb);
-                            y[2] = __builtin_elementwise_fma(c4, tc, ta);
-                            y[3] = __builtin_elementwise_fma(c8, te, tb) + z[5];
+                            yrow(Z[i], y);
+                            y[0] += f32x2{rv[2 * i].x, rv[2 * i].y};
+                            y[1] += f32x2{rv[2 * i].z, rv[2 * i].w};
+                            y[2] += f32x2{rv[2 * i + 1].x, rv[2 * i + 1].y};
+                            y[3] += f32x2{rv[2 * i + 1].z, rv[2 * i + 1].w};
 #pragma unroll
                             for (int jj = 0; jj < 4; ++jj) {
                                 const f32x2 v = y[jj];
-                                if (STATS && h == 0 && i == 0 && jj == 0)
-                                    pivot = __shfl(v.x, l15);
+                                if (STATS && ro == 0 && h == 0 && i == 0 && jj == 0)
+                                    pivot = __shfl(v.x, l31);
                                 f32x2 in2 = {1.0f, 1.0f};
                                 if (!FULL) {
                                     int rl = rowlim;
@@ -751,30 +834,155 @@
                             }
                         }
                     }
-                };
-                if (full) { if (want_stats) emit(std::true_type{}, std::true_type{}); else emit(std::true_type{}, std::false_type{}); }
-                else { if (want_stats) emit(std::false_type{}, std::true_type{}); else emit(std::false_type{}, std::false_type{}); }
-                if (a.d.stats) {
-                    float fc = full ? 64.0f : cnt2.x + cnt2.y;
-                    float S = sum2.x + sum2.y, Q = sq2.x + sq2.y;
-                    fc += __shfl_xor(fc, 16);  S += __shfl_xor(S, 16);  Q += __shfl_xor(Q, 16);
-                    fc += __shfl_xor(fc, 32);  S += __shfl_xor(S, 32);  Q += __shfl_xor(Q, 32);
-                    const int slot = ty * a.tiles_x + tx;
-                    if (kq == 0 && cok) {
-                        fc = fmaxf(fc, 1.0f);
-                        float* o = a.d.stats + (((size_t)b * a.slots + slot) * Cout + co) * 2;
-                        *reinterpret_cast<f32x2*>(o) = f32x2{S + fc * pivot, fmaxf(Q - S * S / fc, 0.0f)};
+                    if (ro == 0) __builtin_amdgcn_s_barrier();
+                }
+            };
+            auto emit_half = [&](auto half_c) {
+                if (full) { if (want_stats) emit(half_c, std::true_type{}, std::true_type{}); else emit(half_c, std::true_type{}, std::false_type{}); }
+                else { if (want_stats) emit(half_c, std::false_type{}, std::true_type{}); else emit(half_c, std::false_type{}, std::false_type{}); }
+            };
+            if (xh == 0) emit_half(std::integral_constant<int, 0>{}); else emit_half(std::integral_constant<int, 1>{});
+            if (a.d.stats && tin) {
+                float fc = full ? 128.0f : cnt2.x + cnt2.y;
+                float S = sum2.x + sum2.y, Q = sq2.x + sq2.y;
+                fc += __shfl_xor(fc, 32);  S += __shfl_xor(S, 32);  Q += __shfl_xor(Q, 32);
+                const int slot = ty * a.tiles_x + tx;
+                if (kk == 0 && cok) {
+                    fc = fmaxf(fc, 1.0f);
+                    float* o = a.d.stats + (((size_t)b * a.slots + slot) * Cout + co) * 2;
+                    *reinterpret_cast<f32x2*>(o) = f32x2{S + fc * pivot, fmaxf(Q - S * S / fc, 0.0f)};
+                }
+#ifndef W4_STAMP
+                if (b == 0 && nt == 0 && cw == 0 && lane == 0) a.d.slot_count[slot] = (float)(min(16, H - ty * 16) * min(16, W - tx * 16));
+#endif
+            }
+        } else {
+#pragma unroll
+            for (int j = 0; j < TGW; ++j) {
+                const int tx = NTG * rx + (TGW == 2 ? j : mtg);
+                if (tx < a.tiles_x) {
+                    int l15 = lane;
+                    asm volatile("" : "+v"(l15));
+                    l15 &= 15;
+                    const int co = cg * 16 + l15;
+                    const bool cok = co < Cout;
+                    float z0 = 0.0f;
+                    asm volatile("" : "+v"(z0));
+                    const float* const bias_p = bias_lds + co;
+                    const int py0 = ty * 16 + 4 * kq, px0 = tx * 16;
+                    f32x2 sum2 = {z0, z0}, sq2 = {z0, z0}, cnt2 = {z0, z0};
+                    float pivot = z0;
+                    const bool full = ty * 16 + 16 <= H && tx * 16 + 16 <= W && cg * 16 + 16 <= Cout;
+                    const bool want_stats = a.d.stats != nullptr;
+                    const unsigned lane_off = (unsigned)((((unsigned)(SPLIT ? sp * a.d.B + b : b) * H + py0) * Wt + px0) * ldot + co) * 4u;
+                    auto emit = [&](auto full_c, auto stats_c) {
+                        constexpr bool FULL = decltype(full_c)::value, STATS = decltype(stats_c)::value;
+                        int step4 = ldot * 16, back3 = ldot * -12, rowadv = (Wt - 7) * ldot * 4;
+                        asm volatile("" : "+s"(step4), "+s"(back3), "+s"(rowadv));
+                        const f32x2 c2 = {2.0f, 2.0f}, c4 = {4.0f, 4.0f}, c8 = {8.0f, 8.0f};
+                        const int rowlim = FULL ? 4 : H - py0, collim = FULL ? 16 : W - px0;
+#pragma unroll
+                        for (int h = 0; h < 2; ++h) {
+                            int soff = h * 32 * ldot;
+                            asm volatile("" : "+s"(soff));
+                            f32x2 Z[4][6];
+#pragma unroll
+                            for (int nu = 0; nu < 6; ++nu) {
+                                auto M = [&](int xi) { return read_acc2(TGW * (xi * 6 + nu) + j, h); };
+                                f32x2 m1 = M(1);
+                                const f32x2 m2 = M(2);
+                                if (nu == 1) m1 += Geo::BIAS_LDS ? *bias_p : bias_r;
+                                const f32x2 p = m1 + m2, q = m1 - m2;
+                                const f32x2 m3 = M(3), m4 = M(4);
+                                const f32x2 r = m3 + m4, u = m3 - m4;
+                                Z[0][nu] = M(0) + p + r;
+                                Z[1][nu] = __builtin_elementwise_fma(c2, u, q);
+                                Z[2][nu] = __builtin_elementwise_fma(c4, r, p);
+                                Z[3][nu] = __builtin_elementwise_fma(c8, u, q) + M(5);
+                                __builtin_amdgcn_sched_barrier(0);
+                            }
+#pragma unroll
+                            for (int i = 0; i < 4; ++i) {
+                                const f32x2 (&z)[6] = Z[i];
+                                const f32x2 ta = z[1] + z[2], tb = z[1] - z[2], tc = z[3] + z[4], te = z[3] - z[4];
+                                f32x2 y[4];
+                                y[0] = z[0] + ta + tc;
+                                y[1] = __builtin_elementwise_fma(c2, te, tb);
+                                y[2] = __builtin_elementwise_fma(c4, tc, ta);
+                                y[3] = __builtin_elementwise_fma(c8, te, tb) + z[5];
+#pragma unroll
+                                for (int jj = 0; jj < 4; ++jj) {
+                                    const f32x2 v = y[jj];
+                                    if (STATS && h == 0 && i == 0 && jj == 0)
+                                        pivot = __shfl(v.x, l15);
+                                    f32x2 in2 = {1.0f, 1.0f};
+                                    if (!FULL) {
+                                        int rl = rowlim;
+                                        asm volatile("" : "+v"(rl));
+                                        const bool row_in = i < rl;
+                                        in2.x = (row_in && 8 * h + jj < collim) ? 1.0f : 0.0f;
+                                        in2.y = (row_in && 8 * h + 4 + jj < collim) ? 1.0f : 0.0f;
+                                    }
+                                    if (STATS) {
+                                        f32x2 dv = v - f32x2{pivot, pivot};
+                                        if (!FULL) { dv *= in2;  cnt2 += in2; }
+                                        sum2 += dv;
+                                        sq2 += dv * dv;
+                                    }
+#if !(W4_ABLATE & 8)
+#pragma unroll
+                                    for (int e = 0; e < 2; ++e) {
+                                        const float vr = e ? v.y : v.x;
+                                        unsigned off = lane_off;
+                                        if (!FULL) off = ((e ? in2.y : in2.x) != 0.0f && cok) ? off : 0xFFFFFFF0u;
+                                        __builtin_amdgcn_raw_buffer_store_b32(__builtin_bit_cast(unsigned, vr), orsrc, off, soff, STREAM ? W4_STORE_AUX : 0);
+                                        asm volatile("s_add_i32 %0, %0, %1" : "+s"(soff) : "s"(e == 0 ? step4 : jj < 3 ? back3 : rowadv) : "scc");
+                                    }
+#else
+                                    asm volatile("" :: "v"(v));
+#endif
+                                }
+                            }
+                        }
+                    };
+                    if (full) { if (want_stats) emit(std::true_type{}, std::true_type{}); else emit(std::true_type{}, std::false_type{}); }
+                    else { if (want_stats) emit(std::false_type{}, std::true_type{}); else emit(std::false_type{}, std::false_type{}); }
+                    if (a.d.stats) {
+                        float fc = full ? 64.0f : cnt2.x + cnt2.y;
+                        float S = sum2.x + sum2.y, Q = sq2.x + sq2.y;
+                        fc += __shfl_xor(fc, 16);  S += __shfl_xor(S, 16);  Q += __shfl_xor(Q, 16);
+                        fc += __shfl_xor(fc, 32);  S += __shfl_xor(S, 32);  Q += __shfl_xor(Q, 32);
+                        const int slot = ty * a.tiles_x + tx;
+                        if (kq == 0 && cok) {
+                            fc = fmaxf(fc, 1.0f);
+                            float* o = a.d.stats + (((size_t)b * a.slots + slot) * Cout + co) * 2;
+                            *reinterpret_cast<f32x2*>(o) = f32x2{S + fc * pivot, fmaxf(Q - S * S / fc, 0.0f)};
+                        }
+#ifndef W4_STAMP
+                        if (b == 0 && nt == 0 && (wave & 3) == 0 && lane == 0) {
+                            a.d.slot_count[slot] = (float)(min(16, H - ty * 16) * min(16, W - tx * 16));
+                        }
+#endif
                     }
-#ifndef W4_STAMP
-                    if (b == 0 && nt == 0 && (wave & 3) == 0 && lane == 0) {
-                        a.d.slot_count[slot] = (float)(min(16, H - ty * 16) * min(16, W - tx * 16));
-                    }
-#endif
                 }
             }
         }
         if (TGW == 1 && W4_PRIO) __builtin_amdgcn_s_setprio(0);
         W4_ACC(stamp_epi);
+        if constexpr (X) {
+            if (more) {
+                W4_T0();
+                f32x2 T[6][6];
+                unsigned t_addr[12];
+                xf_addr(t_addr);
+#pragma unroll
+                for (int ay = 0; ay < 6; ++ay) xf_read(T, t_addr, ay);
+                xf_finish(T, vd_tg, [&] { __builtin_amdgcn_s_barrier(); });
+                asm volatile("s_waitcnt lgkmcnt(0)" ::: "memory");
+                __builtin_amdgcn_s_barrier();
+                W4_ACC(stamp_xf);
+            }
+        }
 #ifdef W4_STAMP_DRAIN
         W4_T0();
         asm volatile("s_waitcnt vmcnt(0)" ::: "memory");
@@ -800,6 +1008,16 @@
         dbg[12] = stamp_tile;
     }
 #endif
+}
+
+template <int MODE, bool STREAM, bool SPLIT = false, int NTG = 2, int NW = 4>
+__global__ __launch_bounds__((64 * NW), (W4Geo<NTG, NW>::WG_PER_CU)) void wino4_kernel(const Wino4Args a) {
+    wino4_body<MODE, STREAM, SPLIT, NTG, NW, false>(a);
+}
+
+template <int MODE, bool STREAM>
+__global__ __launch_bounds__(256, 1) void wino4x_kernel(const Wino4Args a) {
+    wino4_body<MODE, STREAM, false, 2, 4, true>(a);
 }
 
 __global__ __launch_bounds__(256) void w4_splitk_reduce_kernel(const float* __restrict__ part, const float* __restrict__ bias, float* __restrict__ out,
@@ -945,6 +1163,22 @@
     const int kind = (MODE == ND_PRO_AFFINE_SILU || MODE == ND_PRO_AFFINE_MAP_SILU || MODE == ND_PRO_AFFINE_GENMAP_SILU) ? 2 : a.d.stats ? 1 : 4;
     const long out_bytes = (long)a.d.B * a.d.H * a.d.W * a.d.ldo * 4;
     return (out_bytes >= stream_min && (stream_kinds & kind)) ? launch4s<MODE, true, NTG, NW>(a, st) : launch4s<MODE, false, NTG, NW>(a, st);
+}
+
+template <int MODE, bool STREAM>
+int launch4xs(const Wino4Args& a, hipStream_t st) {
+    static nd_device_once configured;
+    constexpr int LDS_BYTES = W4Geo<2>::LDS_BYTES;
+    if (int e = nd_reserve_lds(configured, reinterpret_cast<const void*>(wino4x_kernel<MODE, STREAM>), LDS_BYTES, "nd_conv3x3_wino4x")) return e;
+    const long resident = nd_device_cus();
+    hipLaunchKernelGGL((wino4x_kernel<MODE, STREAM>), dim3((unsigned)(a.total_wg < resident ? a.total_wg : resident)), dim3(256), LDS_BYTES, st, a);
+    return 0;
+}
+
+template <int MODE>
+int launch4x(const Wino4Args& a, hipStream_t st) {
+    const long out_bytes = (long)a.d.B * a.d.H * a.d.W * a.d.ldo * 4;
+    return out_bytes >= (48L << 20) ? launch4xs<MODE, true>(a, st) : launch4xs<MODE, false>(a, st);
 }
 
 }
@@ -1107,6 +1341,21 @@
     return nd_launch_status("nd_conv3x3_wino4_16_nhwc_f32");
 }
 
+extern "C" int nd_conv3x3_wino4x_supported(int H, int W, int cin, int cout, int mode, int upsample) {
+    return (mode == ND_PRO_NONE || mode == ND_PRO_AFFINE_SILU) && !upsample && H >= 16 && W >= 32 && W <= 2048 && H <= 32768 &&
+           cin > KC4 && cin % 4 == 0 && cout > 0 && cout % 4 == 0 && cout <= MAX_COUT;
+}
+
+extern "C" int nd_conv3x3_wino4x_nhwc_f32(const nd_conv3x3* d, void* stream) {
+    Wino4Args a;
+    if (int e = w4_prepare(d, a)) return e;
+    ND_REQUIRE(nd_conv3x3_wino4x_supported(d->H, d->W, d->cin, d->cout, d->src.mode, d->src.upsample), ND_E_SHAPE,
+               "nd_conv3x3_wino4x: plain or GroupNorm-affine + SiLU sources without upsample addressing, H >= 16, W >= 32 (nd_conv3x3_wino4x_supported)");
+    hipStream_t st = (hipStream_t)stream;
+    if (int rc = d->src.mode == ND_PRO_AFFINE_SILU ? launch4x<ND_PRO_AFFINE_SILU>(a, st) : launch4x<ND_PRO_NONE>(a, st)) return rc;
+    return nd_launch_status("nd_conv3x3_wino4x_nhwc_f32");
+}
+
 static int w4_splits(long items, int cin) {
     const int n_chunks = nd_cdiv(cin, KC4);
     if (cin % KC4) return 1;
diff --git a/noisediff_amd/engine.py b/noisediff_amd/engine.py
--- a/noisediff_amd/engine.py
+++ b/noisediff_amd/engine.py
@@ -27,6 +27,7 @@
 GENMAP = os.environ.get("ND_GENMAP", "1") != "0"
 COND_STEP = True
 WINO4 = os.environ.get("ND_WINO4", "1") != "0"
+WINO4X = os.environ.get("ND_WINO4X", "1") != "0"
 SPLIT_K = os.environ.get("ND_SPLIT_K", "0") != "0"
 EIGHT_TILES_RULE = True
 WINO4_16 = os.environ.get("ND_WINO4_16", "narrow")
@@ -506,6 +507,10 @@
                  "nd_conv3x3_wino_nhwc_f32" if wino else "nd_conv3x3_nhwc_f32")
         tiling = (9016 if w4kind == "wino4_16" else 9004) if wino4 else 9002 if wino2 else 9001 if wino else e.lib.nd_conv3x3_tiling_id(self.B, H, W, cout)
         splits = int(e.lib.nd_conv3x3_wino4_splitk_plan(self.B, H, W, cin, cout)) if lowlat_split else 1
+        wino4x = (WINO4X and w4kind == "wino4" and splits == 1
+                  and bool(e.lib.nd_conv3x3_wino4x_supported(H, W, cin, cout, int(src.mode), up)))
+        if wino4x:
+            entry = "nd_conv3x3_wino4x_nhwc_f32"
         if w4kind == "wino4_16" and WINO4_16_SPLIT:
             splits = int(e.lib.nd_conv3x3_wino4_16_splitk_plan(H, W, cin, cout))
         if splits > 1:
```
